# marict/nnue-vision

Hardware: AMD Instinct MI355X
Metric: NNUE training images/sec (full step: fwd+bwd+clip+SGD) (higher is better)
Workload: dtype f32; 1 GPU; c2: NNUE 32x32 grid 10x10x8 F=800 -> 1024/128/32 -> 10, batch 512/GPU, SGD m0.9 wd2e-4 clip1.0; global_batch=512, parallelism=dp1, launch=hipGraph, steps_per_graph=26, max_active_features=453

## Files before the change

### include/nnue_hip.h

```cpp
#ifndef NNUE_HIP_H
#define NNUE_HIP_H

#include <stdint.h>

#ifdef __cplusplus
extern "C" {
#endif

#define NNUE_HIP_ABI_VERSION 39

#define NNUE_OK 0
#define NNUE_E_ARG (-1)
#define NNUE_E_SHAPE (-2)
#define NNUE_E_LAUNCH (-3)
#define NNUE_E_SCRATCH (-4)

typedef void* nnue_stream_t;
typedef struct nnue_cls_rider { unsigned char opaque[256]; } nnue_cls_rider;

int nnue_hip_abi_version(void);
const char* nnue_hip_last_error(void);


int nnue_conv3x3_forward(const float* images, const float* weight, float* conv_out,
// ... 37 lines not shown
int nnue_ft_backward_weight(const float* d_out, const float* coefT, int ldb,
                            int B, int F, int L1, float* d_weight, float* d_bias,
                            nnue_stream_t stream);

int nnue_ft_backward_values(const float* d_out, const float* weight,
                            const int32_t* rows, const int32_t* pos, const int32_t* n, int cap,
                            int B, int F, int L1, float* dst, int dst_ld, nnue_stream_t stream);

int nnue_ftb_supported(int L1);
int nnue_ftb_list_tiles(int B, int F, int P, int* tiles_fwd, int* tiles_bwd);
int64_t nnue_ftb_scratch(int B, int F, int P, int L1);

int nnue_binarize_bits(const float* conv_out, const float* thr, int B, int fps, int Gh, int Gw, int F,
                       uint64_t* maskW, int pw64, uint64_t* maskT, int bw64, float* sink, int32_t* n,
                       uint8_t* tlW, uint8_t* tcW, uint8_t* tlT, uint8_t* tcT, int stages, nnue_stream_t stream);

int nnue_ftb_forward(const float* weight, const float* bias, const uint8_t* tlW, const uint8_t* tcW,
                     const float* sink, int B, int F, int P, int L1, float* out,
                     void* scratch, int64_t scratch_bytes, nnue_stream_t stream);

int nnue_ftb_backward_weight(const float* d_out, const uint8_t* tlT, const uint8_t* tcT, const float* sink,
                             int B, int F, int P, int L1, float* d_weight, float* d_bias,
                             void* scratch, int64_t scratch_bytes, nnue_stream_t stream);

int nnue_ftb_backward_values(const float* d_out, const float* weight, const uint64_t* maskW, int pw64,
                             int B, int F, int P, int L1, float* d_conv_out, nnue_stream_t stream);

int nnue_ftm_supported(int F, int P, int L1);
int64_t nnue_ftm_scratch(int B, int F, int P, int L1);

int nnue_ftm_binarize(const float* conv_out, const float* thr, int B, int fps, int Gh, int Gw, int F,
                      uint8_t* bits, int32_t* n, float* sink, nnue_stream_t stream);

int nnue_ftm_conv_binarize(const float* images, const float* weight, const float* thr, int B, int H, int W,
                           int fps, int stride, int F, float* conv_out, uint8_t* bits, int32_t* n, float* sink,
                           nnue_stream_t stream);
int nnue_ftm_conv_binarize_patches(const float* images, const float* weight, const float* thr, int B, int H, int W,
                                   int fps, int stride, int F, float* patches, float* conv_out, uint8_t* bits,
                                   int32_t* n, float* sink, nnue_stream_t stream);

int nnue_ftm_forward(const uint8_t* bits, const float* sink, const float* weight, const float* bias,
                     int B, int F, int P, int L1, float* out,
                     void* scratch, int64_t scratch_bytes, nnue_stream_t stream);

int nnue_ftm_forward_l1_supported(int B, int F, int P, int L1, int L2);

int nnue_ftm_forward_l1(const uint8_t* bits, const float* sink, const float* weight, const float* bias,
                        const float* w1, int B, int F, int P, int L1, int L2, float* out, float* part,
                        nnue_stream_t stream);

int nnue_ftm_forward_l1_planes_supported(int B, int F, int P, int L1, int L2);
int64_t nnue_ftm_forward_planes_bytes(int B, int F, int P, int L1);

int nnue_ftm_conv_binarize_planes(const float* images, const float* weight, const float* thr, int B, int H, int W,
                                  int fps, int stride, int F, const float* table, int L1, int L2, void* planes,
                                  int64_t planes_bytes, float* conv_out, uint8_t* bits, int32_t* n, float* sink,
                                  nnue_stream_t stream);

int nnue_ftm_forward_l1_planes(const uint8_t* bits, const float* sink, const void* planes, int64_t planes_bytes,
                               const float* weight, const float* bias, const float* w1, int B, int F, int P, int L1,
                               int L2, float* out, float* part, nnue_stream_t stream);

int nnue_ftm_backward_weight(const uint8_t* bits, const float* sink, const float* d_out,
                             int B, int F, int P, int L1, float* d_weight, float* d_bias,
                             nnue_stream_t stream);

int nnue_ftm_backward_values(const uint8_t* bits, const float* d_out, const float* weight,
                             int B, int F, int P, int L1, float* d_conv_out, nnue_stream_t stream);
int64_t nnue_ftm_backward_values_scratch(int B, int F, int P, int L1);
int nnue_ftm_backward_values_ws(const uint8_t* bits, const float* d_out, const float* weight, int B, int F, int P, int L1,
                                float* d_conv_out, void* scratch, int64_t scratch_bytes, nnue_stream_t stream);

int nnue_ftm_backward_cw_supported(int B, int F, int P, int L1, int L2);
int64_t nnue_ftm_backward_sq_count(int B, int F, int P, int L1);
int64_t nnue_ftm_backward_ste_chunks(int B, int F, int P, int L1, int H, int W, int stride);
int nnue_ftm_backward_ste_supported(int B, int F, int P, int L1, int H, int W, int stride);

int nnue_ftm_backward(const uint8_t* bits, const float* sink, const float* d_out, const float* weight,
                      int B, int F, int P, int L1, float* d_weight, float* d_bias, float* d_conv_out,
                      const float* ft, const float* d_z1, int L2, float* d_w1, float* sq_partial,
                      const nnue_cls_rider* small, const float* ste_images, const float* ste_patches, const float* ste_conv_out,
                      const float* ste_thr, int H, int W, int stride, float* ste_partial, int64_t ste_partial_bytes,
                      nnue_stream_t stream);


int64_t nnue_classifier_scratch(int B, int L1, int L2, int L3);
int nnue_classifier_forward(const float* x, int pairwise,
                            const float* w1, const float* b1, const float* w2, const float* b2,
                            const float* w3, const float* b3, float clip,
                            int B, int L1, int L2, int L3, int C,
                            float* h1, float* h2, float* logits,
                            void* scratch, int64_t scratch_bytes, nnue_stream_t stream);

int nnue_classifier_backward(const float* x, int pairwise,
                             const float* w1, const float* w2, const float* w3, float clip,
                             const float* h1, const float* h2, const float* d_logits,
                             int B, int L1, int L2, int L3, int C,
                             float* d_x, float* d_w1, float* d_b1, float* d_w2, float* d_b2,
                             float* d_w3, float* d_b3,
                             void* scratch, int64_t scratch_bytes, nnue_stream_t stream);

int64_t nnue_classifier_train_scratch(int B, int L1, int L2, int L3, int C);
int64_t nnue_classifier_train_dz1_offset(int B, int L1, int L2, int L3, int C, int pairwise);
int nnue_classifier_train_step(const float* x, int pairwise,
                               const float* w1, const float* b1, const float* w2, const float* b2,
                               const float* w3, const float* b3, float clip,
                               const int64_t* labels, float grad_scale,
                               int B, int L1, int L2, int L3, int C,
                               float* h1, float* h2, float* logits, float* sample_loss, float* loss,
                               float* d_x, float* d_w1, float* d_b1, float* d_w2, float* d_b2,
                               float* d_w3, float* d_b3,
                               void* scratch, int64_t scratch_bytes, int phases, nnue_stream_t stream);
int nnue_classifier_train_fused_tail_supported(int B, int L1, int L2, int L3, int C, int K, int pairwise);
int nnue_classifier_train_rider(int pairwise, int B, int L1, int L2, int L3, int C, const float* h1, const float* h2,
                                const float* sample_loss, float* loss, float* d_b1, float* d_w2, float* d_b2,
                                float* d_w3, float* d_b3, void* scratch, int64_t scratch_bytes,
                                const struct nnue_buckets* buckets, nnue_cls_rider* out);

typedef struct nnue_buckets {
  int32_t K;
  const int32_t* bucket;
  const int32_t* rows;
  const int32_t* tile_bucket;
  const int32_t* seg;
  int32_t tiles;
} nnue_buckets;

int nnue_bucket_tile_count(int B, int K);
int nnue_bucket_group(const int32_t* n, int B, int P, int K, int32_t* bucket, int32_t* rows,
                      int32_t* tile_bucket, int32_t* seg, nnue_stream_t stream);

int nnue_ftm_forward_grouping(const uint8_t* bits, const float* sink, const float* weight, const float* bias,
                              int B, int F, int P, int L1, float* out, void* scratch, int64_t scratch_bytes,
                              const int32_t* n, int K, int32_t* bucket, int32_t* rows, int32_t* tile_bucket,
                              int32_t* seg, nnue_stream_t stream);

int64_t nnue_classifier_scratch_bucketed(int B, int L1, int L2, int L3, int K);
int64_t nnue_classifier_train_scratch_bucketed(int B, int L1, int L2, int L3, int C, int K);
int nnue_classifier_forward_bucketed(const float* x, int pairwise,
                                     const float* w1, const float* b1, const float* w2, const float* b2,
                                     const float* w3, const float* b3, float clip,
                                     int B, int L1, int L2, int L3, int C,
                                     float* h1, float* h2, float* logits,
                                     void* scratch, int64_t scratch_bytes, const nnue_buckets* buckets,
                                     nnue_stream_t stream);
int nnue_classifier_backward_bucketed(const float* x, int pairwise,
                                      const float* w1, const float* w2, const float* w3, float clip,
                                      const float* h1, const float* h2, const float* d_logits,
                                      int B, int L1, int L2, int L3, int C,
                                      float* d_x, float* d_w1, float* d_b1, float* d_w2, float* d_b2,
                                      float* d_w3, float* d_b3,
                                      void* scratch, int64_t scratch_bytes, const nnue_buckets* buckets,
                                      nnue_stream_t stream);
int64_t nnue_classifier_train_dz1_grouped_offset(int B, int L1, int L2, int L3, int C, int K);
int64_t nnue_classifier_train_x_grouped_offset(int B, int L1, int L2, int L3, int C, int K);
int nnue_classifier_train_step_bucketed(const float* x, int pairwise,
                                        const float* w1, const float* b1, const float* w2, const float* b2,
                                        const float* w3, const float* b3, float clip,
                                        const int64_t* labels, float grad_scale,
                                        int B, int L1, int L2, int L3, int C,
                                        float* h1, float* h2, float* logits, float* sample_loss, float* loss,
                                        float* d_x, float* d_w1, float* d_b1, float* d_w2, float* d_b2,
                                        float* d_w3, float* d_b3,
                                        void* scratch, int64_t scratch_bytes, int phases,
                                        const nnue_buckets* buckets, nnue_stream_t stream);

// ... 196 lines not shown
```

### nnue-vision_amd/csrc/feature_kernels.hip

```cpp
#include "common.h"

#include <cstdlib>

namespace {

constexpr float kSteSharpness = 10.0f;
constexpr int kConvChunk = 8;

__global__ __launch_bounds__(256) void conv3x3_forward_kernel(const float* __restrict__ img,
                                                              const float* __restrict__ w,
                                                              float* __restrict__ out, int B, int H, int W,
                                                              int fps, int stride, int Gh, int Gw) {
  extern __shared__ float w_lds[];
  for (int i = threadIdx.x; i < fps * 27; i += blockDim.x) w_lds[i] = w[i];
  __syncthreads();
  const int G = Gh * Gw;
  const long long t = (long long)blockIdx.x * blockDim.x + threadIdx.x;
  if (t >= (long long)B * G) return;
  const int b = (int)(t / G);
  const int hw = (int)(t - (long long)b * G);
  const int h = hw / Gw, x = hw - h * Gw;
  float patch[27];
#pragma unroll
  for (int ci = 0; ci < 3; ++ci)
#pragma unroll
    for (int kh = 0; kh < 3; ++kh)
#pragma unroll
      for (int kw = 0; kw < 3; ++kw) {
        const int iy = h * stride + kh - 1, ix = x * stride + kw - 1;
        const bool in = iy >= 0 && iy < H && ix >= 0 && ix < W;
        patch[ci * 9 + kh * 3 + kw] = in ? img[(((size_t)b * 3 + ci) * H + iy) * W + ix] : 0.0f;
      }
  for (int c0 = 0; c0 < fps; c0 += kConvChunk) {
    float acc[kConvChunk];
#pragma unroll
    for (int u = 0; u < kConvChunk; ++u) acc[u] = 0.0f;
#pragma unroll
    for (int q = 0; q < 27; ++q)
#pragma unroll
      for (int u = 0; u < kConvChunk; ++u) {
        const int c = (c0 + u < fps) ? c0 + u : fps - 1;
        acc[u] = fmaf(patch[q], w_lds[c * 27 + q], acc[u]);
      }
#pragma unroll
    for (int u = 0; u < kConvChunk; ++u)
      if (c0 + u < fps) out[((size_t)b * fps + c0 + u) * G + hw] = acc[u];
  }
}

#include "conv_binarize.h"

template <bool kFullUnroll, bool kPatch = false>
__global__ __launch_bounds__(256) void conv_binarize_kernel(const float* __restrict__ img, const float* __restrict__ w,
                                                            const float* __restrict__ thr, float* __restrict__ out,
                                                            uint8_t* __restrict__ bits, int* __restrict__ n,
                                                            float* __restrict__ sink, int H, int W, int fps, int stride,
                                                            int Gh, int Gw, int F, int slices, float* __restrict__ patches) {
  extern __shared__ __attribute__((aligned(16))) float w_lds[];
  ConvParamsPlain prm{w, thr};
  conv_binarize_body<kFullUnroll, kPatch>(img, prm, out, bits, n, sink, H, W, fps, stride, Gh, Gw, F, slices, (int)blockIdx.x, (int)blockIdx.y,
                                          w_lds, [] {}, patches, (size_t)gridDim.x * Gh * Gw);
}

#include "forward_planes.h"

template <bool kFullUnroll>
__global__ __launch_bounds__(256) void conv_binarize_planes_kernel(const float* __restrict__ img, const float* __restrict__ w,
                                                                   const float* __restrict__ thr, float* __restrict__ out,
                                                                   uint8_t* __restrict__ bits, int* __restrict__ n,
                                                                   float* __restrict__ sink, int B, int H, int W, int fps, int stride,
                                                                   int Gh, int Gw, int F, int slices, FwdPlaneArgs pa) {
  extern __shared__ __attribute__((aligned(16))) float w_lds[];
  const int id = (int)blockIdx.x;
  if (id >= B * slices) {
    forward_planes_write(pa, id - B * slices);
    return;
  }
  ConvParamsPlain prm{w, thr};
  conv_binarize_body<kFullUnroll, false>(img, prm, out, bits, n, sink, H, W, fps, stride, Gh, Gw, F, slices, id % B, id / B, w_lds, [] {});
}

__global__ __launch_bounds__(256) void binarize_compact_kernel(const float* __restrict__ conv_out,
                                                               const float* __restrict__ thr, int G, int P, int F,
                                                               int* __restrict__ rows, int* __restrict__ pos,
                                                               float* __restrict__ coef, int* __restrict__ n,
                                                               float* __restrict__ coefT, int ldb) {
  __shared__ int wave_count[4];
  __shared__ int sink_count[4];
  const int b = blockIdx.x;
  const int tid = threadIdx.x, lane = tid & 63, wave = tid >> 6;
  const float* __restrict__ x = conv_out + (size_t)b * P;
  const size_t base = (size_t)b * P;
  int written = 0, sink = 0;
  for (int p0 = 0; p0 < P; p0 += 256) {
    const int p = p0 + tid;
    const bool on = (p < P) && (x[p] > thr[p / G]);
    const unsigned long long m = __ballot(on);
    const unsigned long long ms = __ballot(on && p >= F - 1);
    if (lane == 0) {
      wave_count[wave] = __popcll(m);
      sink_count[wave] = __popcll(ms);
    }
    __syncthreads();
    int offset = written, total = 0;
#pragma unroll
    for (int w = 0; w < 4; ++w) {
      const int c = wave_count[w];
      if (w < wave) offset += c;
      total += c;
      sink += sink_count[w];
    }
    if (on) {
      const int k = offset + __popcll(m & ((1ull << lane) - 1ull));
      rows[base + k] = p < F - 1 ? p : F - 1;
      pos[base + k] = p;
      coef[base + k] = 1.0f;
    }
    written += total;
    __syncthreads();
  }
  if (tid == 0) {
    n[b] = written;
    coefT[(size_t)(F - 1) * ldb + b] = (float)sink;
  }
}

__global__ __launch_bounds__(256) void binarize_transpose_kernel(const float* __restrict__ conv_out,
                                                                 const float* __restrict__ thr, int B, int G, int P,
                                                                 int F, float* __restrict__ coefT, int ldb) {
  __shared__ float tile[64][65];
  const int p0 = blockIdx.x * 64, b0 = blockIdx.y * 64;
  const int tx = threadIdx.x & 63, ty = threadIdx.x >> 6;
  const int p = p0 + tx;
  const float t = (p < P) ? thr[p / G] : 0.0f;
  for (int j = ty; j < 64; j += 4) {
    const int b = b0 + j;
    const bool on = (b < B) && (p < P) && (conv_out[(size_t)b * P + p] > t);
    tile[j][tx] = on ? 1.0f : 0.0f;
  }
  __syncthreads();
  for (int j = ty; j < 64; j += 4) {
    const int f = p0 + j;
    if (f < F - 1 && b0 + tx < ldb) coefT[(size_t)f * ldb + b0 + tx] = tile[tx][j];
  }
}

__global__ __launch_bounds__(256) void ste_conv_backward_stage1(const float* __restrict__ img,
                                                                const float* __restrict__ conv_out,
                                                                const float* __restrict__ thr,
                                                                const float* __restrict__ d_conv_out, int B, int H,
                                                                int W, int fps, int stride, int Gh, int Gw,
                                                                int samples_per_chunk, float* __restrict__ partial) {
  __shared__ float red[4][28];
  const int c = blockIdx.x;
  const int chunk = blockIdx.y;
  const int G = Gh * Gw;
  const int b_lo = chunk * samples_per_chunk;
  const int b_hi = min(B, b_lo + samples_per_chunk);
// ... 212 lines not shown
  return blocks > 0 ? blocks : 1;
}

__global__ __launch_bounds__(256) void conv3x3_backward_input_kernel(const float* __restrict__ d_out, const float* __restrict__ w,
                                                                     float* __restrict__ d_img, int B, int H, int W, int fps,
                                                                     int stride, int Gh, int Gw) {
  extern __shared__ float w_lds[];
  for (int i = threadIdx.x; i < fps * 27; i += blockDim.x) w_lds[i] = w[i];
  __syncthreads();
  const long long t = (long long)blockIdx.x * blockDim.x + threadIdx.x;
  if (t >= (long long)B * H * W) return;
  const int b = (int)(t / ((long long)H * W));
  const int yx = (int)(t - (long long)b * H * W);
  const int y = yx / W, x = yx - y * W;
  const int G = Gh * Gw;
  float a0 = 0.f, a1 = 0.f, a2 = 0.f;
#pragma unroll
  for (int kh = 0; kh < 3; ++kh) {
    const int ny = y + 1 - kh;
    if (ny < 0 || ny % stride) continue;
    const int oh = ny / stride;
    if (oh >= Gh) continue;
#pragma unroll
    for (int kw = 0; kw < 3; ++kw) {
      const int nx = x + 1 - kw;
      if (nx < 0 || nx % stride) continue;
      const int ow = nx / stride;
      if (ow >= Gw) continue;
      const float* __restrict__ d = d_out + (size_t)b * fps * G + oh * Gw + ow;
      const int q = kh * 3 + kw;
      for (int c = 0; c < fps; ++c) {
        const float g = d[(size_t)c * G];
        a0 = fmaf(g, w_lds[c * 27 + q], a0);
        a1 = fmaf(g, w_lds[c * 27 + 9 + q], a1);
        a2 = fmaf(g, w_lds[c * 27 + 18 + q], a2);
      }
    }
  }
  float* __restrict__ o = d_img + (size_t)b * 3 * H * W + yx;
  o[0] = a0;
  o[(size_t)H * W] = a1;
  o[(size_t)2 * H * W] = a2;
}

__global__ __launch_bounds__(256) void sparse_values_gather_kernel(const float* __restrict__ map, const int64_t* __restrict__ idx,
                                                                   long long total, int P, int M, float* __restrict__ val) {
  const long long t = (long long)blockIdx.x * 256 + threadIdx.x;
  if (t >= total) return;
  const long long b = t / M;
  const int64_t p = idx[t];
  val[t] = (p >= 0 && p < P) ? map[b * P + p] : 0.0f;
}
__global__ __launch_bounds__(256) void sparse_values_scatter_kernel(const float* __restrict__ d_val, const int64_t* __restrict__ idx,
                                                                    long long total, int P, int M, float* __restrict__ d_map) {
  const long long t = (long long)blockIdx.x * 256 + threadIdx.x;
  if (t >= total) return;
  const long long b = t / M;
  const int64_t p = idx[t];
  if (p >= 0 && p < P) d_map[b * P + p] = d_val[t];
}

}

extern "C" int nnue_conv3x3_forward(const float* images, const float* weight, float* conv_out, int B, int H, int W,
                                    int fps, int stride, nnue_stream_t stream) {
  NNUE_REQUIRE(images && weight && conv_out, NNUE_E_ARG, "nnue_conv3x3_forward: null pointer");
  NNUE_REQUIRE(B > 0 && H > 0 && W > 0 && fps > 0 && stride > 0, NNUE_E_ARG,
               "nnue_conv3x3_forward: B=%d H=%d W=%d fps=%d stride=%d must be positive", B, H, W, fps, stride);
  NNUE_REQUIRE(fps * 27 * 4 <= 64 * 1024, NNUE_E_SHAPE, "nnue_conv3x3_forward: fps=%d too large for the LDS weight tile", fps);
  const int Gh = (H - 1) / stride + 1, Gw = (W - 1) / stride + 1;
  const long long total = (long long)B * Gh * Gw;
  NNUE_REQUIRE(total < (1ll << 31) * 256, NNUE_E_SHAPE, "nnue_conv3x3_forward: too many outputs");
  hipLaunchKernelGGL(conv3x3_forward_kernel, dim3((unsigned)((total + 255) / 256)), dim3(256), fps * 27 * sizeof(float),
                     static_cast<hipStream_t>(stream), images, weight, conv_out, B, H, W, fps, stride, Gh, Gw);
  return nnue_launch_status("nnue_conv3x3_forward");
}

namespace {
struct PlaneRide {
  const float* table;
  int L1, L2;
  void* planes;
  int64_t planes_bytes;
};

int conv_binarize_impl(const char* who, const float* images, const float* weight, const float* thr, int B, int H, int W, int fps, int stride, int F,
                       float* conv_out, float* patches, uint8_t* bits, int32_t* n, float* sink, nnue_stream_t stream,
                       const PlaneRide& ride = PlaneRide{}) {
  NNUE_REQUIRE(images && weight && thr && conv_out && bits && n && sink, NNUE_E_ARG, "%s: null pointer", who);
  NNUE_REQUIRE(B > 0 && H > 0 && W > 0 && fps > 0 && stride > 0 && F > 0, NNUE_E_ARG, "%s: B=%d H=%d W=%d fps=%d stride=%d F=%d must be positive", who,
               B, H, W, fps, stride, F);
  NNUE_REQUIRE(((fps + 7) & ~7) * 28 * 4 <= 64 * 1024, NNUE_E_SHAPE, "%s: fps=%d too large for the LDS weight tile", who, fps);
  const int Gh = (H - 1) / stride + 1, Gw = (W - 1) / stride + 1;
  const long long G = (long long)Gh * Gw;
  NNUE_REQUIRE(G * fps < (1ll << 30) && (long long)B * G * fps < (1ll << 40), NNUE_E_SHAPE, "%s: map too large", who);
  NNUE_REQUIRE(!patches || 27ll * B * G * 4 < (1ll << 31), NNUE_E_SHAPE, "%s: the im2col buffer must stay below 2 GiB", who);
  const int P = (int)(G * fps);
  if (ride.table) {
    NNUE_REQUIRE(ride.planes, NNUE_E_ARG, "%s: null pointer", who);
    NNUE_REQUIRE(nnue_ftm_forward_l1_planes_supported(B, F, P, ride.L1, ride.L2), NNUE_E_SHAPE,
                 "%s: B=%d F=%d P=%d L1=%d L2=%d is not a planes-fed forward shape (nnue_ftm_forward_l1_planes_supported)", who, B, F, P, ride.L1,
                 ride.L2);
    NNUE_REQUIRE(nnue_aligned16(ride.table) && nnue_aligned16(ride.planes), NNUE_E_ARG, "%s: pointers must be 16-byte aligned", who);
    NNUE_REQUIRE(ride.planes_bytes >= nnue_ftm_forward_planes_bytes(B, F, P, ride.L1), NNUE_E_SCRATCH, "%s: plane buffer of %lld bytes, needs %lld", who,
                 (long long)ride.planes_bytes, (long long)nnue_ftm_forward_planes_bytes(B, F, P, ride.L1));
  }
  hipStream_t s = static_cast<hipStream_t>(stream);
  const int threads = G <= 64 ? 64 : (G <= 128 ? 128 : 256);
  int slices = (512 + B - 1) / B;
  if (slices > (int)(G / threads)) slices = (int)(G / threads);
  slices = slices < 1 ? 1 : (slices > 16 ? 16 : slices);
  if (slices > 1) nnue_zero_counters(n, sink, B, s);
  const size_t lds = (size_t)(((fps + 7) & ~7) * 28) * sizeof(float);
  if (ride.table) {
    const int direct = (F - 1 < P) ? F - 1 : P, ktiles = (direct + kBfK - 1) / kBfK, parts = 256 / threads;
    const FwdPlaneArgs pa{ride.table, static_cast<unsigned char*>(ride.planes), (unsigned)((size_t)direct * ride.L1 * 4), ride.L1, ktiles, parts};
    const int riders = (ride.L1 / 64) * ktiles * parts;
    const dim3 grid((unsigned)(B * slices + riders));
    if (fps <= 16)
      hipLaunchKernelGGL((conv_binarize_planes_kernel<true>), grid, dim3(threads), lds, s, images, weight, thr, conv_out, bits, n, sink, B, H, W, fps,
                         stride, Gh, Gw, F, slices, pa);
    else
      hipLaunchKernelGGL((conv_binarize_planes_kernel<false>), grid, dim3(threads), lds, s, images, weight, thr, conv_out, bits, n, sink, B, H, W, fps,
                         stride, Gh, Gw, F, slices, pa);
    return nnue_launch_status(who);
  }
#define NNUE_CONV_LAUNCH(FULL, PATCH)                                                                                                           \
  hipLaunchKernelGGL((conv_binarize_kernel<FULL, PATCH>), dim3(B, slices), dim3(threads), lds, s, images, weight, thr, conv_out, bits, n, sink, H, \
                     W, fps, stride, Gh, Gw, F, slices, patches)
  if (fps <= 16) {
    if (!patches) NNUE_CONV_LAUNCH(true, false);
    else NNUE_CONV_LAUNCH(true, true);
  } else {
    if (!patches) NNUE_CONV_LAUNCH(false, false);
    else NNUE_CONV_LAUNCH(false, true);
  }
#undef NNUE_CONV_LAUNCH
  return nnue_launch_status(who);
}
}

extern "C" int nnue_ftm_conv_binarize(const float* images, const float* weight, const float* thr, int B, int H, int W, int fps,
                                      int stride, int F, float* conv_out, uint8_t* bits, int32_t* n, float* sink,
                                      nnue_stream_t stream) {
  return conv_binarize_impl("nnue_ftm_conv_binarize", images, weight, thr, B, H, W, fps, stride, F, conv_out, nullptr, bits, n, sink, stream);
}

extern "C" int nnue_ftm_conv_binarize_patches(const float* images, const float* weight, const float* thr, int B, int H, int W, int fps,
                                              int stride, int F, float* patches, float* conv_out, uint8_t* bits, int32_t* n, float* sink,
                                              nnue_stream_t stream) {
  NNUE_REQUIRE(patches, NNUE_E_ARG, "nnue_ftm_conv_binarize_patches: null pointer");
  return conv_binarize_impl("nnue_ftm_conv_binarize_patches", images, weight, thr, B, H, W, fps, stride, F, conv_out, patches, bits, n, sink, stream);
}

extern "C" int nnue_ftm_conv_binarize_planes(const float* images, const float* weight, const float* thr, int B, int H, int W, int fps,
                                             int stride, int F, const float* table, int L1, int L2, void* planes, int64_t planes_bytes,
                                             float* conv_out, uint8_t* bits, int32_t* n, float* sink, nnue_stream_t stream) {
  NNUE_REQUIRE(table && planes, NNUE_E_ARG, "nnue_ftm_conv_binarize_planes: null pointer");
  return conv_binarize_impl("nnue_ftm_conv_binarize_planes", images, weight, thr, B, H, W, fps, stride, F, conv_out, nullptr, bits, n, sink, stream,
                            PlaneRide{table, L1, L2, planes, planes_bytes});
}

extern "C" int nnue_binarize_features(const float* conv_out, const float* thr, int B, int fps, int Gh, int Gw, int F,
                                      int32_t* rows, int32_t* pos, float* coef, int32_t* n, float* coefT, int ldb,
                                      nnue_stream_t stream) {
  NNUE_REQUIRE(conv_out && thr && rows && pos && coef && n && coefT, NNUE_E_ARG, "nnue_binarize_features: null pointer");
  NNUE_REQUIRE(B > 0 && fps > 0 && Gh > 0 && Gw > 0 && F > 0, NNUE_E_ARG,
               "nnue_binarize_features: B=%d fps=%d Gh=%d Gw=%d F=%d must be positive", B, fps, Gh, Gw, F);
  NNUE_REQUIRE(ldb >= B && ldb % 64 == 0, NNUE_E_SHAPE, "nnue_binarize_features: ldb=%d must be a multiple of 64 and >= B=%d", ldb, B);
  const long long P64 = (long long)fps * Gh * Gw;
  NNUE_REQUIRE(P64 < (1ll << 30), NNUE_E_SHAPE, "nnue_binarize_features: fps*Gh*Gw too large");
  const int P = (int)P64, G = Gh * Gw;
  hipStream_t s = static_cast<hipStream_t>(stream);
  if (F > 1)
    hipLaunchKernelGGL(binarize_transpose_kernel, dim3((F - 1 + 63) / 64, ldb / 64), dim3(256), 0, s, conv_out, thr, B, G,
                       P, F, coefT, ldb);
  hipLaunchKernelGGL(binarize_compact_kernel, dim3(B), dim3(256), 0, s, conv_out, thr, G, P, F, rows, pos, coef, n, coefT,
                     ldb);
  return nnue_launch_status("nnue_binarize_features");
}

extern "C" int64_t nnue_ste_conv_backward_scratch(int B, int fps, int Gh, int Gw) {
  if (B <= 0 || fps <= 0) return 0;
  int64_t blocks = ste_chunks(B, fps);
  if (fps <= 64 && Gh > 0 && Gw > 0) blocks = ste_mfma_blocks((int64_t)B * Gh * Gw);
  return blocks * fps * 28 * (int64_t)sizeof(float);
}

extern "C" int64_t nnue_ste_conv_backward_chunks(int B, int fps, int Gh, int Gw) {
  if (B <= 0 || fps <= 0 || Gh <= 0 || Gw <= 0) return 0;
  return fps <= 64 ? ste_mfma_blocks((int64_t)B * Gh * Gw) : ste_chunks(B, fps);
}

namespace {
int ste_impl(const char* who, const float* images, const float* conv_out, const float* patches, const float* thr,
             const float* d_conv_out, int B, int H, int W, int fps, int stride, int Gh, int Gw, float* d_thr, float* d_weight, void* scratch,
             int64_t scratch_bytes, int stages, nnue_stream_t stream) {
  NNUE_REQUIRE(d_thr || d_weight, NNUE_E_ARG, "%s: both outputs are null", who);
  NNUE_REQUIRE(stages >= 1 && stages <= 3, NNUE_E_ARG, "%s: stages = 1 (partials) | 2 (final sums)", who);
  NNUE_REQUIRE(scratch_bytes >= nnue_ste_conv_backward_scratch(B, fps, Gh, Gw), NNUE_E_SCRATCH, "%s: scratch %lld < %lld bytes", who,
               (long long)scratch_bytes, (long long)nnue_ste_conv_backward_scratch(B, fps, Gh, Gw));
  hipStream_t s = static_cast<hipStream_t>(stream);
  float* partial = static_cast<float*>(scratch);
  int chunks;
  if (fps <= 64) {
    const long long NP = (long long)B * Gh * Gw;
    NNUE_REQUIRE(NP < (1ll << 31) - 64 && (long long)B * fps * Gh * Gw < (1ll << 40), NNUE_E_SHAPE, "%s: too many positions", who);
    const int tiles = (int)((NP + kStePos - 1) / kStePos);
    chunks = (int)ste_mfma_blocks(NP);
    const char* abl_env = std::getenv("NNUE_STE_ABL");
    const int abl = abl_env ? std::atoi(abl_env) : 0;
    if (stages & 1) {
#define NNUE_STE_LAUNCH(MT)                                                                                                          \
  do {                                                                                                                               \
    if (patches)                                                                                                                     \
      hipLaunchKernelGGL((ste_conv_backward_mfma<MT, true>), dim3(chunks), dim3(256), 0, s, patches, conv_out, thr, d_conv_out, B, H, W,  \
                         fps, stride, Gh, Gw, tiles, partial, abl);                                                                  \
    else                                                                                                                             \
      hipLaunchKernelGGL((ste_conv_backward_mfma<MT, false>), dim3(chunks), dim3(256), 0, s, images, conv_out, thr, d_conv_out, B, H, W, \
                         fps, stride, Gh, Gw, tiles, partial, abl);                                                                  \
  } while (0)
    switch ((fps + 15) / 16) {
      case 1: NNUE_STE_LAUNCH(1); break;
      case 2: NNUE_STE_LAUNCH(2); break;
      case 3: NNUE_STE_LAUNCH(3); break;
      default: NNUE_STE_LAUNCH(4); break;
    }
#undef NNUE_STE_LAUNCH
    }
  } else {
    NNUE_REQUIRE(!patches, NNUE_E_SHAPE, "%s: the im2col form needs fps <= 64 (fps = %d)", who, fps);
    chunks = ste_chunks(B, fps);
    const int spc = (B + chunks - 1) / chunks;
    NNUE_REQUIRE((long long)spc * Gh * Gw < (1ll << 31), NNUE_E_SHAPE, "%s: chunk too large", who);
    if (stages & 1)
      hipLaunchKernelGGL(ste_conv_backward_stage1, dim3(fps, chunks), dim3(256), 0, s, images, conv_out, thr, d_conv_out, B, H,
                         W, fps, stride, Gh, Gw, spc, partial);
  }
  if (stages & 2)
    hipLaunchKernelGGL(ste_conv_backward_stage2, dim3((fps * 28 + 3) / 4), dim3(256), 0, s, partial, chunks, fps, d_thr, d_weight);
  return nnue_launch_status(who);
}
}
// ... 56 lines not shown
```

### nnue-vision_amd/csrc/ftm_kernels.hip

```cpp
#include "common.h"
#include "small_wgrad.h"

#include <cstdlib>
#include <cstring>
#include <type_traits>

namespace {

using f32x4 = __attribute__((ext_vector_type(4))) float;

#include "bucket_group.h"
#include "optim_update.h"

struct Mat {
  const void* p;
  unsigned bytes;
  int ld, clamp, inner_k;
};
using u32x4 = __attribute__((__vector_size__(4 * sizeof(unsigned)))) unsigned;
#include "forward_planes.h"

template <bool U8>
__device__ __forceinline__ u32x4 mat_load(__amdgpu_buffer_rsrc_t rsrc, const Mat& m, int outer, int inner) {
  const int row = outer < m.clamp ? outer : m.clamp;
  const int elem = row * m.ld + inner;
  if (U8) {
    u32x4 raw = {0u, 0u, 0u, 0u};
    raw[0] = __builtin_amdgcn_raw_buffer_load_b32(rsrc, inner < m.inner_k ? elem : 0x7ffffff0, 0, 0);
    return raw;
  }
  return __builtin_amdgcn_raw_buffer_load_b128(rsrc, inner < m.inner_k ? elem * 4 : 0x7ffffff0, 0, 0);
}

template <bool U8>
__device__ __forceinline__ float4 widen(const u32x4& raw) {
  if (U8) {
    const unsigned w = raw[0];
    return make_float4((float)(w & 0xffu), (float)((w >> 8) & 0xffu), (float)((w >> 16) & 0xffu), (float)(w >> 24));
  }
  return make_float4(__uint_as_float(raw[0]), __uint_as_float(raw[1]), __uint_as_float(raw[2]), __uint_as_float(raw[3]));
}

__device__ __forceinline__ int xcd_contiguous_tile(int tile, int nwg) {
  const int xcd = tile & 7, q8 = nwg >> 3, r8 = nwg & 7;
  return (xcd < r8 ? xcd * (q8 + 1) : r8 * (q8 + 1) + (xcd - r8) * q8) + (tile >> 3);
}

struct FwdEpi {
  static constexpr bool kAU8 = true;
  static constexpr bool kFusedL1 = false;
  static constexpr bool kBPair = false;
  static constexpr bool kSq = false;
  const float* __restrict__ bias;
  const float* __restrict__ w_last;
  const float* __restrict__ sink;
  float* __restrict__ out;
  int B, L1, ksplit;
  __device__ __forceinline__ float2 col(int n) const { return ksplit == 1 ? make_float2(bias[n], w_last[n]) : make_float2(0.f, 0.f); }
  __device__ __forceinline__ float pre(int m, int) const { return ksplit == 1 ? sink[m] : 0.0f; }
  __device__ __forceinline__ void store(int m, int n, float v, float2 c, float s, int ks) const {
    if (ksplit == 1) v += fmaf(s, c.y, c.x);
    out[((size_t)ks * B + m) * L1 + n] = v;
  }
};

struct BwwEpi {
  static constexpr bool kAU8 = true;
  static constexpr bool kFusedL1 = false;
  static constexpr bool kBPair = false;
  static constexpr bool kSq = true;
  float* __restrict__ d_weight;
  int L1;
  float* __restrict__ sq;
  __device__ __forceinline__ float2 col(int) const { return make_float2(0.f, 0.f); }
  __device__ __forceinline__ float pre(int, int) const { return 0.0f; }
  __device__ __forceinline__ void store(int m, int n, float v, float2, float, int) const { d_weight[(size_t)m * L1 + n] = v; }
};

struct BwwSgdEpi {
  static constexpr bool kAU8 = true;
  static constexpr bool kFusedL1 = false;
  static constexpr bool kBPair = false;
  static constexpr bool kSq = false;
  static constexpr bool kRmw = true;
  float* __restrict__ weight;
  float* __restrict__ momentum;
  const float* __restrict__ coef;
  int L1;
  float lr, mom, wd, scale;
  int first_step;
  int xcd_remap;
  const float* __restrict__ lr_dev;
  __device__ __forceinline__ float2 col(int) const { return make_float2(coef[0] * scale, 0.f); }
  __device__ __forceinline__ float pre(int m, int n) const { return weight[(size_t)m * L1 + n]; }
  __device__ __forceinline__ void store(int m, int n, float v, float2 c, float w, int) const {
    const size_t i = (size_t)m * L1 + n;
    float gi = fmaf(wd, w, v * c.x);
    if (momentum) {
      gi = first_step ? gi : fmaf(mom, momentum[i], gi);
      momentum[i] = gi;
    }
    weight[i] = w - (lr_dev ? lr_dev[0] : lr) * gi;
  }
};

struct BwwAdamEpi {
  static constexpr bool kAU8 = true;
  static constexpr bool kFusedL1 = false;
  static constexpr bool kRmw = true;
  static constexpr bool kAdam = true;
  float* __restrict__ weight;
  float* __restrict__ exp_avg;
  float* __restrict__ exp_avg_sq;
  const float* __restrict__ coef;
  const int* __restrict__ step_counter;
  int L1;
  float lr, beta1, beta2, eps, wd, scale;
  int xcd_remap;
  const float* __restrict__ lr_dev;
};

struct ValEpi {
  static constexpr bool kAU8 = false;
  static constexpr bool kFusedL1 = false;
  static constexpr bool kBPair = false;
  static constexpr bool kSq = false;
  const uint8_t* __restrict__ bits;
  float* __restrict__ d_conv_out;
  int P;
  __device__ __forceinline__ float2 col(int) const { return make_float2(0.f, 0.f); }
  __device__ __forceinline__ float pre(int m, int p) const { return (float)bits[(size_t)m * P + p]; }
  __device__ __forceinline__ void store(int m, int p, float v, float2, float bit, int) const {
    d_conv_out[(size_t)m * P + p] = bit != 0.0f ? v : 0.0f;
  }
};

struct ValSteEpi {
  static constexpr bool kAU8 = false;
  static constexpr bool kFusedL1 = false;
  static constexpr bool kBPair = false;
  static constexpr bool kSte = true;
  const uint8_t* __restrict__ bits;
  float* __restrict__ d_conv_out;
  int P;
  const float* __restrict__ img;
  const float* __restrict__ patches;
  const float* __restrict__ conv_out;
  const float* __restrict__ thr;
  int H, W, stride, Gw, G;
  float* __restrict__ partial;
  int n_tiles;
  __device__ __forceinline__ int prow(int tile_n, int j) const {
    const int hw = tile_n * 8 + (j & 7);
    return (j >> 3) * G + (hw < G ? hw : G - 1);
  }
};
constexpr float kFtmSteSharpness = 10.0f;

template <class Epi, class = void>
struct is_ste { static constexpr bool value = false; };
template <class Epi>
struct is_ste<Epi, decltype((void)Epi::kSte)> { static constexpr bool value = Epi::kSte; };

template <int BM>
struct SteFrag {
  float pv[BM / 8][4][2];
  unsigned in[(BM + 31) / 32];
};
template <int BM>
__device__ __forceinline__ void ste_pixels(const ValSteEpi& e, SteFrag<BM>& f, int M, int m_base, int tile_n, int wave, int r, int q) {
#pragma unroll
  for (int w = 0; w < (BM + 31) / 32; ++w) f.in[w] = 0u;
#pragma unroll
  for (int g = 0; g < BM / 8; ++g)
#pragma unroll
    for (int t4 = 0; t4 < 4; ++t4) {
      const int k = wave * 2 * BM + 16 * g + 4 * q + t4;
      const int m = m_base + (k >> 3), hw = tile_n * 8 + (k & 7);
      const bool ok = m < M && hw < e.G;
      const int h = hw / e.Gw, x = hw - h * e.Gw;
#pragma unroll
      for (int s = 0; s < 2; ++s) {
        const int qq = r + 16 * s;
        const int qc = qq < 27 ? qq : 26;
        bool in;
        float v;
        if (e.patches) {
          in = ok && qq < 27;
          v = e.patches[in ? ((size_t)qc * M + m) * e.G + hw : 0];
        } else {
          const int ci = qc / 9, kh = (qc - ci * 9) / 3, kw = qc - ci * 9 - kh * 3;
          const int iy = h * e.stride + kh - 1, ix = x * e.stride + kw - 1;
          in = ok && qq < 27 && iy >= 0 && iy < e.H && ix >= 0 && ix < e.W;
          v = e.img[in ? (((size_t)m * 3 + ci) * e.H + iy) * e.W + ix : 0];
        }
        f.pv[g][t4][s] = v;
        f.in[g >> 2] |= (in ? 1u : 0u) << (8 * (g & 3) + 2 * t4 + s);
      }
    }
}
template <int BM>
__device__ __forceinline__ void ste_pixels_select(SteFrag<BM>& f, int r) {
#pragma unroll
  for (int g = 0; g < BM / 8; ++g)
#pragma unroll
    for (int t4 = 0; t4 < 4; ++t4)
#pragma unroll
      for (int s = 0; s < 2; ++s) {
        const bool in = (f.in[g >> 2] >> (8 * (g & 3) + 2 * t4 + s)) & 1u;
        f.pv[g][t4][s] = in ? f.pv[g][t4][s] : (r + 16 * s == 27 ? 1.0f : 0.0f);
      }
}

template <int BM>
struct StePre {
  uint8_t bit[BM / 32][2][4];
  float cv[BM / 32][2][4], th[2];
};
template <int BM>
__device__ __forceinline__ void ste_prefetch(const ValSteEpi& e, StePre<BM>& p, int M, int m_base, int tile_n, int m0, int n0, int r, int q) {
#pragma unroll
  for (int t = 0; t < 2; ++t) {
    const int j = n0 + 16 * t + r, c = j >> 3, hw = tile_n * 8 + (j & 7);
    const int pp = c * e.G + (hw < e.G ? hw : 0);
    p.th[t] = e.thr[c];
#pragma unroll
    for (int i = 0; i < BM / 32; ++i)
#pragma unroll
      for (int ee = 0; ee < 4; ++ee) {
        const int m = min(m_base + m0 + 16 * i + 4 * q + ee, M - 1);
        p.bit[i][t][ee] = e.bits[(size_t)m * e.P + pp];
        p.cv[i][t][ee] = e.conv_out[(size_t)m * e.P + pp];
      }
  }
}

template <int BM, int BN>
__device__ __forceinline__ void ste_tile(float* __restrict__ smem, const ValSteEpi& e, const f32x4 (&acc)[BM / 32][BN / 32], const SteFrag<BM>& f,
                                         const StePre<BM>& pre, int M, int m_base, int tile_n, int m0, int n0, int tile) {
  static_assert(BN == 64, "a tile holds the 8 channels of 8 positions");
  constexpr int TM = BM / 32, TN = BN / 32, LDA = 8 * BM + 4;
  const int tid = threadIdx.x, lane = tid & 63;
  const int wave = __builtin_amdgcn_readfirstlane(tid >> 6);
  const int r = lane & 15, q = lane >> 4;
  float bit[TM][TN][4], slope[TM][TN][4];
#pragma unroll
  for (int t = 0; t < TN; ++t) {
    const int hw = tile_n * 8 + ((n0 + 16 * t + r) & 7);
#pragma unroll
    for (int i = 0; i < TM; ++i)
#pragma unroll
      for (int ee = 0; ee < 4; ++ee) {
        const int m = m_base + m0 + 16 * i + 4 * q + ee;
        const bool ok = m < M && hw < e.G;
        bit[i][t][ee] = ok ? (float)pre.bit[i][t][ee] : 0.0f;
        const float cv = ok ? pre.cv[i][t][ee] : 0.0f;
        const float s = 1.0f / (1.0f + __expf(-kFtmSteSharpness * (cv - pre.th[t])));
        slope[i][t][ee] = (kFtmSteSharpness * s) * (1.0f - s);
      }
  }
  float* __restrict__ A = smem;
  float* __restrict__ red = smem + 16 * LDA;
#pragma unroll
  for (int t = 0; t < TN; ++t) {
    const int j = n0 + 16 * t + r, c = j >> 3, hw = tile_n * 8 + (j & 7);
    const int p = c * e.G + (hw < e.G ? hw : 0);
#pragma unroll
    for (int i = 0; i < TM; ++i)
#pragma unroll
      for (int ee = 0; ee < 4; ++ee) {
        const int m_loc = m0 + 16 * i + 4 * q + ee, m = m_base + m_loc;
        const float d = bit[i][t][ee] != 0.0f ? acc[i][t][ee] : 0.0f;
        if (e.d_conv_out && m < M && hw < e.G) e.d_conv_out[(size_t)m * e.P + p] = d;
        const int k = m_loc * 8 + (j & 7);
        A[c * LDA + k] = d;
        A[(8 + c) * LDA + k] = d * slope[i][t][ee];
      }
  }
  __syncthreads();
  f32x4 c0 = {0.f, 0.f, 0.f, 0.f}, c1 = {0.f, 0.f, 0.f, 0.f};
#pragma unroll
  for (int g = 0; g < BM / 8; ++g) {
    const float4 a = *reinterpret_cast<const float4*>(&A[r * LDA + wave * 2 * BM + 16 * g + 4 * q]);
    c0 = __builtin_amdgcn_mfma_f32_16x16x4f32(a.x, f.pv[g][0][0], c0, 0, 0, 0);
    c1 = __builtin_amdgcn_mfma_f32_16x16x4f32(a.x, f.pv[g][0][1], c1, 0, 0, 0);
    c0 = __builtin_amdgcn_mfma_f32_16x16x4f32(a.y, f.pv[g][1][0], c0, 0, 0, 0);
    c1 = __builtin_amdgcn_mfma_f32_16x16x4f32(a.y, f.pv[g][1][1], c1, 0, 0, 0);
    c0 = __builtin_amdgcn_mfma_f32_16x16x4f32(a.z, f.pv[g][2][0], c0, 0, 0, 0);
    c1 = __builtin_amdgcn_mfma_f32_16x16x4f32(a.z, f.pv[g][2][1], c1, 0, 0, 0);
    c0 = __builtin_amdgcn_mfma_f32_16x16x4f32(a.w, f.pv[g][3][0], c0, 0, 0, 0);
    c1 = __builtin_amdgcn_mfma_f32_16x16x4f32(a.w, f.pv[g][3][1], c1, 0, 0, 0);
  }
#pragma unroll
  for (int ee = 0; ee < 4; ++ee) {
    red[(wave * 8 + ee) * 64 + lane] = c0[ee];
    red[(wave * 8 + 4 + ee) * 64 + lane] = c1[ee];
  }
  __syncthreads();
  const int slot = xcd_contiguous_tile(tile, e.n_tiles);
  for (int o = tid; o < 8 * 28; o += 256) {
    const int c = o / 28, qq = o - c * 28;
    const int row = qq < 27 ? c : 8 + c, col = qq;
    const int s = (col >> 4) * 4 + (row & 3), ln = (row >> 2) * 16 + (col & 15);
    e.partial[(size_t)o * e.n_tiles + slot] =
        (red[(0 * 8 + s) * 64 + ln] + red[(1 * 8 + s) * 64 + ln]) + (red[(2 * 8 + s) * 64 + ln] + red[(3 * 8 + s) * 64 + ln]);
  }
}

struct CwEpi {
  static constexpr bool kAU8 = false;
  static constexpr bool kFusedL1 = false;
  static constexpr bool kBPair = true;
  static constexpr bool kSq = false;
  float* __restrict__ d_w1;
  int L1, half;
  __device__ __forceinline__ float2 col(int) const { return make_float2(0.f, 0.f); }
  __device__ __forceinline__ float pre(int, int) const { return 0.0f; }
  __device__ __forceinline__ void store(int m, int n, float v, float2, float, int) const { d_w1[(size_t)m * L1 + n] = v; }
};

struct FwdL1Epi {
  static constexpr bool kAU8 = true;
  static constexpr bool kFusedL1 = true;
  static constexpr bool kBPair = false;
// ... 840 lines not shown
    if constexpr (ABL == 4) return;
#pragma unroll
    for (int i = 0; i < GA; ++i) {
      const int g = tid + 256 * i, row = g / RUNS, c = g % RUNS;
      u32x4 hi, mid, lo;
      if constexpr (ABL == 1 || ABL == 2) { hi = ra[i][0]; mid = ra[i][1]; lo = ra[i][0] ^ ra[i][1]; }
      else split8(ra[i][0], ra[i][1], hi, mid, lo);
      *reinterpret_cast<u32x4*>(As + bf6_img<KT>(row, c)) = hi;
      *reinterpret_cast<u32x4*>(As + PA + bf6_img<KT>(row, c)) = mid;
      *reinterpret_cast<u32x4*>(As + 2 * PA + bf6_img<KT>(row, c)) = lo;
    }
#pragma unroll
    for (int i = 0; i < GB; ++i) {
      const int g = tid + 256 * i, row = g / RUNS, c = g % RUNS;
      u32x4 hi, mid, lo;
      if constexpr (ABL == 2) { hi = rb[i][0]; mid = rb[i][1]; lo = rb[i][0] ^ rb[i][1]; }
      else split8(rb[i][0], rb[i][1], hi, mid, lo);
      *reinterpret_cast<u32x4*>(Bs + bf6_img<KT>(row, c)) = hi;
      *reinterpret_cast<u32x4*>(Bs + PB + bf6_img<KT>(row, c)) = mid;
      *reinterpret_cast<u32x4*>(Bs + 2 * PB + bf6_img<KT>(row, c)) = lo;
    }
  };
  f32x4 acc[TM][TN];
#pragma unroll
  for (int i = 0; i < TM; ++i)
#pragma unroll
    for (int t = 0; t < TN; ++t) acc[i][t] = (f32x4){0.f, 0.f, 0.f, 0.f};
  auto contract = [&]() {
#pragma unroll
    for (int kb = 0; kb < KT / 32; ++kb) {
      const int c = kb * 4 + q;
      bf16x8 a[3][TM], b[3][TN];
#pragma unroll
      for (int pl = 0; pl < 3; ++pl) {
#pragma unroll
        for (int i = 0; i < TM; ++i) a[pl][i] = *reinterpret_cast<const bf16x8*>(As + pl * PA + bf6_img<KT>(m0 + 16 * i + r, c));
#pragma unroll
        for (int t = 0; t < TN; ++t) b[pl][t] = *reinterpret_cast<const bf16x8*>(Bs + pl * PB + bf6_img<KT>(n0 + 16 * t + r, c));
      }
      constexpr int pa[6] = {2, 0, 1, 1, 0, 0}, pb[6] = {0, 2, 1, 0, 1, 0};
      if constexpr (ABL == 3) {
#pragma unroll
        for (int s6 = 0; s6 < 6; ++s6)
#pragma unroll
          for (int i = 0; i < TM; ++i)
#pragma unroll
            for (int t = 0; t < TN; ++t) acc[i][t][0] += (float)a[pa[s6]][i][0] + (float)b[pb[s6]][t][0];
      } else {
#pragma unroll
      for (int s6 = 0; s6 < 6; ++s6)
#pragma unroll
        for (int i = 0; i < TM; ++i)
#pragma unroll
          for (int t = 0; t < TN; ++t) acc[i][t] = __builtin_amdgcn_mfma_f32_16x16x32_bf16(a[pa[s6]][i], b[pb[s6]][t], acc[i][t], 0, 0, 0);
      }
    }
  };
  fetch(k_lo);
  for (int k0 = k_lo; k0 < k_hi; k0 += KT) {
    stage();
    __syncthreads();
    if (k0 + KT < k_hi) fetch(k0 + KT);
    contract();
    __syncthreads();
  }
  if constexpr (is_ste<Epi>::value) {
    SteFrag<BM> stef;
    StePre<BM> stepre;
    ste_prefetch<BM>(epi, stepre, M, m_base, tile_n, m0, n0, r, q);
    ste_pixels<BM>(epi, stef, M, m_base, tile_n, wave, r, q);
    ste_pixels_select<BM>(stef, r);
    ste_tile<BM, BN>(reinterpret_cast<float*>(smem), epi, acc, stef, stepre, M, m_base, tile_n, m0, n0, tile);
  } else {
    store_tile<BM, BN, Epi>(reinterpret_cast<float*>(smem), epi, acc, M, N, m_base, n_base, m0, n0, tile, ks);
  }
}

template <int BM, int BN, class Epi, int KT, int ABL = 0>
__global__ __launch_bounds__(256) void ftm_gemm_bf6_kernel(Mat ma, Mat mb, Epi epi, int M, int N, int K, int tiles_n) {
  __shared__ __attribute__((aligned(16))) unsigned char smem[gemm_bf6_lds_bytes<BM, BN, KT>()];
  gemm_tile_bf6<BM, BN, Epi, KT, ABL>(smem, ma, mb, epi, M, N, 0, K, tiles_n, blockIdx.x, 0);
}

template <int BM, int BN, bool AKC, class Epi>
__global__ __launch_bounds__(256) void ftm_gemm_bf_kernel(Mat ma, Mat mb, Epi epi, int M, int N, int K, int klen, int tiles_n, GroupArgs ga) {
  __shared__ __attribute__((aligned(16))) unsigned char smem[gemm_bf_lds_bytes<BM, BN, kBfK>()];
  if (ga.n && blockIdx.x == gridDim.x - 1) {
    if (blockIdx.y == 0) bucket_group_body<256>(ga, reinterpret_cast<int*>(smem));
    return;
  }
  const int ks = blockIdx.y, k_lo = ks * klen;
  int tile = blockIdx.x;
  if constexpr (is_rmw<Epi>::value) {
    if (epi.xcd_remap) tile = xcd_contiguous_tile(tile, gridDim.x);
  }
  gemm_tile_bf<BM, BN, AKC, Epi>(smem, ma, mb, epi, M, N, k_lo, (k_lo + klen < K) ? k_lo + klen : K, tiles_n, tile, ks);
}

template <int BM>
__global__ __launch_bounds__(256) void ftm_forward_l1_bf_kernel(Mat ma, Mat mb, FwdL1Epi epi, int M, int N, int K, int tiles_n) {
  constexpr int kGemm = gemm_bf_lds_bytes<BM, 64, kBfK>(), kEpi = 2 * BM * kL1Ld * 4;
  __shared__ __attribute__((aligned(16))) unsigned char smem[kGemm > kEpi ? kGemm : kEpi];
  gemm_tile_bf<BM, 64, true, FwdL1Epi>(smem, ma, mb, epi, M, N, 0, K, tiles_n, blockIdx.x, 0);
}

__global__ __launch_bounds__(256) void ftm_forward_l1_planes_kernel(Mat ma, Mat mp, FwdL1Epi epi, int M, int N, int K, int tiles_n) {
  constexpr int kGemm = gemm_bf_lds_bytes<32, 64, kBfK>(), kEpi = 2 * 32 * kL1Ld * 4;
  __shared__ __attribute__((aligned(16))) unsigned char smem[kGemm > kEpi ? kGemm : kEpi];
  gemm_tile_bf<32, 64, true, FwdL1Epi, true>(smem, ma, mp, epi, M, N, 0, K, tiles_n, blockIdx.x, 0);
}

constexpr int kStreamKTiles = 7, kStreamDepth = 3;
__global__ __launch_bounds__(256) __attribute__((amdgpu_waves_per_eu(1, 1))) void ftm_forward_l1_stream_kernel(Mat ma, Mat mp, FwdL1Epi epi,
                                                                                                            int K, int tiles_n) {
  constexpr int D = kStreamDepth;
  static_assert(D >= 1 && D <= kStreamKTiles, "K tiles of plane loads requested ahead");
  constexpr int kA = 32 * kBfK * 2, kEpi = 2 * 32 * kL1Ld * 4;
  static_assert(kStreamKTiles * kA >= kEpi, "the epilogue's LDS aliases the A images");
  __shared__ __attribute__((aligned(16))) unsigned char smem[kStreamKTiles * kA];
  const __amdgpu_buffer_rsrc_t rsa = __builtin_amdgcn_make_buffer_rsrc(const_cast<void*>(ma.p), 0, ma.bytes, 0x00020000);
  const __amdgpu_buffer_rsrc_t rsb = __builtin_amdgcn_make_buffer_rsrc(const_cast<void*>(mp.p), 0, mp.bytes, 0x00020000);
  const int tid = threadIdx.x, lane = tid & 63;
  const int wave = __builtin_amdgcn_readfirstlane(tid >> 6);
  const int r = lane & 15, q = lane >> 4;
  const int tile = blockIdx.x, tile_n = tile % tiles_n, tile_m = tile / tiles_n;
  const int m_base = tile_m * 32, n0 = 16 * wave;
  const int ktiles = (K + kBfK - 1) / kBfK;
  const int a_row = ((tid >> 4) << 1) | (tid & 1), a_grp = (tid >> 1) & 7;
  u32x4 ra[kStreamKTiles];
#pragma unroll
  for (int kt = 0; kt < kStreamKTiles; ++kt)
    ra[kt] = __builtin_amdgcn_raw_buffer_load_b128(rsa, (m_base + a_row) * ma.ld + kt * kBfK + a_grp * 16, 0, 0);
  FusedL1Pre<32, true> l1pre;
  fused_l1_prefetch<32, true>(epi, l1pre, m_base, tile_n, 0, n0, r, q, wave);
  __builtin_amdgcn_sched_barrier(0);
  int b_off[kBfK / 32];
#pragma unroll
  for (int kb = 0; kb < kBfK / 32; ++kb) b_off[kb] = bf_img(n0 + r, 4 * kb + q);
  u32x4 rb[D][kBfK / 32][3];
  auto fetch = [&](int kt, u32x4 (&R)[kBfK / 32][3]) {
    const int blk = (tile_n * ktiles + (kt < ktiles ? kt : ktiles - 1)) * kFwdPlaneBlock;
#pragma unroll
    for (int kb = 0; kb < kBfK / 32; ++kb)
#pragma unroll
      for (int pnum = 2; pnum >= 0; --pnum) R[kb][pnum] = __builtin_amdgcn_raw_buffer_load_b128(rsb, b_off[kb], blk + pnum * (64 * kBfK * 2), 0);
  };
#pragma unroll
  for (int kt = 0; kt < D; ++kt) fetch(kt, rb[kt]);
  __builtin_amdgcn_sched_barrier(0);
#pragma unroll
  for (int kt = 0; kt < kStreamKTiles; ++kt) stage_map_k(smem + kt * kA, BfImg<kBfK>{}, a_row, a_grp * 2, ra[kt]);
  __syncthreads();
  f32x4 acc[2][1];
#pragma unroll
  for (int i = 0; i < 2; ++i) acc[i][0] = (f32x4){0.f, 0.f, 0.f, 0.f};
#pragma unroll
  for (int kt = 0; kt < kStreamKTiles; ++kt) {
    u32x4 (&R)[kBfK / 32][3] = rb[kt % D];
    if (kt < ktiles) {
      const unsigned char* __restrict__ As = smem + kt * kA;
#pragma unroll
      for (int kb = 0; kb < kBfK / 32; ++kb) {
        const int c = kb * 4 + q;
        bf16x8 a[2];
#pragma unroll
        for (int i = 0; i < 2; ++i) a[i] = *reinterpret_cast<const bf16x8*>(As + bf_img(16 * i + r, c));
// ... 87 lines not shown
#pragma unroll
      for (int u = 0; u < 8; ++u) {
        d[u] = d_out[(size_t)(b + u) * L1 + col];
        s[u] = sink[b + u];
      }
#pragma unroll
      for (int u = 0; u < 8; ++u) {
        sb += d[u];
        sw = fmaf(s[u], d[u], sw);
      }
    }
    for (; b < hi; ++b) {
      const float d = d_out[(size_t)b * L1 + col];
      sb += d;
      sw = fmaf(sink[b], d, sw);
    }
  }
  red[0][part][c] = sb;
  red[1][part][c] = sw;
  __syncthreads();
  if (part < 2 && col < L1) {
    float s = 0.f;
#pragma unroll
    for (int i = 0; i < 16; ++i) s += red[part][i][c];
    if (part == 0) {
      if (d_bias) d_bias[col] = s;
    } else if (d_weight) {
      d_weight[(size_t)(F - 1) * L1 + col] = s;
    }
  }
}

__global__ __launch_bounds__(256) void ftm_tail_rows_kernel(TailRows t) {
  __shared__ float red[512];
  tail_rows_block(t, blockIdx.x, blockIdx.y, red);
}

struct CwArgs {
  Mat a, b;
  CwEpi e;
  int M, N, K, tiles_n, n_c;
  const int* seg;
  int per_bucket;
};

template <int WM, int WN, int WK, int VM, int VN, int VK>
__global__ __launch_bounds__(256) void ftm_backward_kernel(Mat wa, Mat wb, BwwEpi we, int wM, int wN, int wK, int w_tiles_n, int n_w,
                                                           Mat va, Mat vb, ValEpi ve, int vM, int vN, int vK, int v_tiles_n, int n_v,
                                                           CwArgs c, TailRows t, SmallWgrad sw) {
  constexpr int kW = gemm_lds_floats<WM, WN, WK, false, false>(), kV = gemm_lds_floats<VM, VN, VK, true, true>();
  constexpr int kC = gemm_lds_floats<WM, WN, WK, false, false>();
  constexpr int kWV = kW > kV ? kW : kV;
  __shared__ __attribute__((aligned(16))) float smem[kWV > kC ? kWV : kC];
  const int blk = blockIdx.x;
  if (blk < n_v) {
    gemm_tile<VM, VN, VK, true, true, ValEpi>(smem, va, vb, ve, vM, vN, 0, vK, v_tiles_n, blk, 0);
  } else if (blk < n_v + n_w) {
    gemm_tile<WM, WN, WK, false, false, BwwEpi>(smem, wa, wb, we, wM, wN, 0, wK, w_tiles_n, blk - n_v, 0);
  } else if (blk < n_v + n_w + c.n_c) {
    const int t = blk - n_v - n_w;
    if (c.seg) {
      const int kb = t / c.per_bucket;
      const int k_lo = c.seg[kb], k_hi = c.seg[kb + 1];
      Mat a = c.a, b = c.b;
      a.bytes = (unsigned)k_hi * (unsigned)a.ld * 4u;
      b.bytes = (unsigned)k_hi * (unsigned)b.ld * 4u;
      CwEpi e = c.e;
      e.d_w1 += (size_t)kb * c.M * c.N;
      gemm_tile<WM, WN, WK, false, false, CwEpi>(smem, a, b, e, c.M, c.N, k_lo, k_hi, c.tiles_n, t - kb * c.per_bucket, 0);
    } else {
      gemm_tile<WM, WN, WK, false, false, CwEpi>(smem, c.a, c.b, c.e, c.M, c.N, 0, c.K, c.tiles_n, t, 0);
    }
  } else {
    const int i = blk - n_w - n_v - c.n_c, n_t = t.col_blocks * (1 + t.zero_slices);
    if (i < n_t) tail_rows_block(t, i % t.col_blocks, i / t.col_blocks, smem);
    else small_wgrad_body(sw, i - n_t, smem);
  }
}

template <int WM, int VM, int VN, int VK, bool V6 = false, bool W64 = false, class VE = ValEpi>
__global__ __launch_bounds__(256) void ftm_backward_bf_kernel(Mat wa, Mat wb, BwwEpi we, int wM, int wN, int wK, int w_tiles_n, int n_w,
                                                              Mat va, Mat vb, VE ve, int vM, int vN, int vK, int v_tiles_n, int n_v,
                                                              CwArgs c, TailRows t, SmallWgrad sw) {
  constexpr int kW = gemm_bf_lds_bytes<WM, 64, W64 ? kBf64K : kBfK>(), kV = V6 ? gemm_bf6_lds_bytes<VM, VN>() : gemm_lds_floats<VM, VN, VK, true, true>() * 4;
  constexpr int kC = gemm_lds_floats<32, 64, 128, false, false>() * 4;
  constexpr int kWV = kW > kV ? kW : kV;
  constexpr int kLds = kWV > kC ? kWV : kC;
  static_assert(!is_ste<VE>::value || (16 * (8 * VM + 4) + 2048) * 4 <= kLds, "the STE epilogue borrows the tile's LDS");
  __shared__ __attribute__((aligned(16))) unsigned char smem_b[kLds];
  float* smem = reinterpret_cast<float*>(smem_b);
  const int blk = blockIdx.x;
  if (blk < n_v) {
    if constexpr (V6) gemm_tile_bf6<VM, VN, VE>(smem_b, va, vb, ve, vM, vN, 0, vK, v_tiles_n, blk, 0);
    else gemm_tile<VM, VN, VK, true, true, VE>(smem, va, vb, ve, vM, vN, 0, vK, v_tiles_n, blk, 0);
  } else if (blk < n_v + n_w) {
    if constexpr (W64) gemm_tile_bf64<WM, false, BwwEpi>(smem_b, wa, wb, we, wM, wN, 0, wK, w_tiles_n, blk - n_v, 0);
    else gemm_tile_bf<WM, 64, false, BwwEpi>(smem_b, wa, wb, we, wM, wN, 0, wK, w_tiles_n, blk - n_v, 0);
  } else if (blk < n_v + n_w + c.n_c) {
    const int t2 = blk - n_v - n_w;
    if (c.seg) {
      const int kb = t2 / c.per_bucket;
      const int k_lo = c.seg[kb], k_hi = c.seg[kb + 1];
      Mat a = c.a, b = c.b;
      a.bytes = (unsigned)k_hi * (unsigned)a.ld * 4u;
      b.bytes = (unsigned)k_hi * (unsigned)b.ld * 4u;
      CwEpi e = c.e;
      e.d_w1 += (size_t)kb * c.M * c.N;
      gemm_tile<32, 64, 128, false, false, CwEpi>(smem, a, b, e, c.M, c.N, k_lo, k_hi, c.tiles_n, t2 - kb * c.per_bucket, 0);
    } else {
      gemm_tile<32, 64, 128, false, false, CwEpi>(smem, c.a, c.b, c.e, c.M, c.N, 0, c.K, c.tiles_n, t2, 0);
    }
  } else {
    const int i = blk - n_w - n_v - c.n_c, n_t = t.col_blocks * (1 + t.zero_slices);
    if (i < n_t) tail_rows_block(t, i % t.col_blocks, i / t.col_blocks, smem);
    else small_wgrad_body(sw, i - n_t, smem);
  }
}

__global__ __launch_bounds__(256) void ftm_binarize_kernel(const float* __restrict__ conv_out, const float* __restrict__ thr,
                                                           int P, int G, int F, int slices, uint8_t* __restrict__ bits,
                                                           int* __restrict__ n, float* __restrict__ sink) {
  __shared__ int cnt_s[4], sink_s[4];
  const int b = blockIdx.x;
  const float4* __restrict__ x4 = reinterpret_cast<const float4*>(conv_out + (size_t)b * P);
  unsigned* __restrict__ o4 = reinterpret_cast<unsigned*>(bits + (size_t)b * P);
  int cnt = 0, snk = 0;
  for (int g = blockIdx.y * 256 + threadIdx.x; g < P / 4; g += 256 * slices) {
    const float4 x = x4[g];
    const int p = g * 4;
    int c = p / G, rem = p - c * G;
    float4 v;
    v.x = x.x > thr[c] ? 1.0f : 0.0f;
    if (++rem == G) { rem = 0; ++c; }
    v.y = x.y > thr[c] ? 1.0f : 0.0f;
    if (++rem == G) { rem = 0; ++c; }
    v.z = x.z > thr[c] ? 1.0f : 0.0f;
    if (++rem == G) { rem = 0; ++c; }
    v.w = x.w > thr[c] ? 1.0f : 0.0f;
    o4[g] = (unsigned)v.x | ((unsigned)v.y << 8) | ((unsigned)v.z << 16) | ((unsigned)v.w << 24);
    cnt += (int)(v.x + v.y + v.z + v.w);
    snk += (p >= F - 1 ? (int)v.x : 0) + (p + 1 >= F - 1 ? (int)v.y : 0) + (p + 2 >= F - 1 ? (int)v.z : 0) + (p + 3 >= F - 1 ? (int)v.w : 0);
  }
#pragma unroll
  for (int s = 32; s >= 1; s >>= 1) {
    cnt += __shfl_xor(cnt, s);
    snk += __shfl_xor(snk, s);
  }
  if ((threadIdx.x & 63) == 0) {
    cnt_s[threadIdx.x >> 6] = cnt;
    sink_s[threadIdx.x >> 6] = snk;
  }
  __syncthreads();
  if (threadIdx.x == 0) {
    const int total = cnt_s[0] + cnt_s[1] + cnt_s[2] + cnt_s[3], st = sink_s[0] + sink_s[1] + sink_s[2] + sink_s[3];
    if (slices == 1) {
      n[b] = total;
      sink[b] = (float)st;
    } else {
      atomicAdd(&n[b], total);
      if (st) atomicAdd(&sink[b], (float)st);
    }
  }
}

using i32x4 = __attribute__((ext_vector_type(4))) int;
constexpr int kGramU = 4;

__device__ __forceinline__ void gram_pair(int x, int& tm, int& tn) {
  tm = 0;
  while ((tm + 1) * (tm + 2) / 2 <= x) ++tm;
  tn = x - tm * (tm + 1) / 2;
}

__global__ __launch_bounds__(256) void gram_i8_kernel(const uint8_t* __restrict__ bits, unsigned bytes, int B, int P, int direct, int wave_steps,
                                                      int* __restrict__ slabs, int slices, TailRows tr, int n_tail) {
  __shared__ int red[4][4][256];
// ... 329 lines not shown
}
}

namespace {
bool values_bf6(int B, int P, int L1) {
  static const int bf6 = env_int("NNUE_FTM_VAL_BF6", 1);
  const Shape s = plan(B, P, L1, true, false);
  return bf6 && use_bf16() && s.cfg == 2 && s.ksplit == 1 && L1 % 8 == 0;
}
}

extern "C" int nnue_ftm_backward_values(const uint8_t* bits, const float* d_out, const float* weight, int B, int F, int P, int L1,
                                        float* d_conv_out, nnue_stream_t stream) {
  NNUE_REQUIRE(bits && d_out && weight && d_conv_out, NNUE_E_ARG, "nnue_ftm_backward_values: null pointer");
  NNUE_REQUIRE(shape_ok(B, F, P, L1), NNUE_E_ARG, "nnue_ftm_backward_values: B=%d F=%d P=%d L1=%d out of range", B, F, P, L1);
  NNUE_REQUIRE(nnue_ftm_supported(F, P, L1), NNUE_E_SHAPE, "nnue_ftm_backward_values: P=%d and L1=%d must be multiples of 4", P, L1);
  NNUE_REQUIRE(nnue_aligned16(d_out) && nnue_aligned16(weight), NNUE_E_ARG, "nnue_ftm_backward_values: pointers must be 16-byte aligned");
  hipStream_t st = static_cast<hipStream_t>(stream);
  const Shape s = plan(B, P, L1, true, false);
  const Mat ma{d_out, (unsigned)((size_t)B * L1 * 4), L1, kIntMax, L1}, mb{weight, (unsigned)((size_t)F * L1 * 4), L1, F - 1, kIntMax};
  const ValEpi epi{bits, d_conv_out, P};
  if (values_bf6(B, P, L1)) {
    const dim3 grid((unsigned)(s.tiles_m * s.tiles_n));
#ifdef NNUE_ABLATIONS
    static const int abl = env_int("NNUE_FTM_BF6_ABL", 0);
#define NNUE_ABL(N) if (abl == N) { hipLaunchKernelGGL((ftm_gemm_bf6_kernel<128, 64, ValEpi, 32, N>), grid, dim3(256), 0, st, ma, mb, epi, B, P, L1, s.tiles_n); return nnue_launch_status("nnue_ftm_backward_values"); }
    NNUE_ABL(1) NNUE_ABL(2) NNUE_ABL(3) NNUE_ABL(4) NNUE_ABL(5)
#undef NNUE_ABL
#endif
    hipLaunchKernelGGL((ftm_gemm_bf6_kernel<128, 64, ValEpi, 32>), grid, dim3(256), 0, st, ma, mb, epi, B, P, L1, s.tiles_n);
    return nnue_launch_status("nnue_ftm_backward_values");
  }
  launch<true, true>(st, s, ma, mb, epi, B, P, L1);
  return nnue_launch_status("nnue_ftm_backward_values");
}

extern "C" int64_t nnue_ftm_backward_values_scratch(int , int , int , int ) { return 0; }

extern "C" int nnue_ftm_backward_values_ws(const uint8_t* bits, const float* d_out, const float* weight, int B, int F, int P, int L1,
                                           float* d_conv_out, void* , int64_t , nnue_stream_t stream) {
  return nnue_ftm_backward_values(bits, d_out, weight, B, F, P, L1, d_conv_out, stream);
}

namespace {
int merged_bf_wm() {
  const int wm = env_int("NNUE_FTM_BF_WM", 64);
  return use_bf16() ? (wm == 32 ? 32 : 64) : 0;
}

bool merged_backward_shape(int B, int F, int P, int L1, bool* big) {
  const int direct = (F - 1 < P) ? F - 1 : P;
  if (direct <= 0) return false;
  static const int split_launch = env_int("NNUE_FTM_SPLIT_BACKWARD", 0);
  static const int force_pair = env_int("NNUE_FTM_BWD_PAIR", 0);
  const Shape sw = plan(direct, L1, B, false, false), sv = plan(B, P, L1, true, false);
  const long long tiles64 = (long long)((direct + 63) / 64) * ((L1 + 63) / 64) + (long long)((B + 63) / 64) * ((P + 63) / 64);
  const bool small_pair = sw.cfg == 0 && (sv.cfg == 0 || sv.cfg == 1);
  *big = force_pair == 11 || (force_pair != 1 && small_pair && tiles64 >= 448);
  return !split_launch && (small_pair || *big);
}
bool merged_w64() {
  static const int w64 = env_int("NNUE_FTM_BWD_W64", 1);
  return w64 != 0;
}
bool merged_values_bf6(int B, int F, int P, int L1) {
  static const int bf6 = env_int("NNUE_FTM_BWD_BF6", 1);
  bool big = false;
  if (!merged_backward_shape(B, F, P, L1, &big) || !merged_bf_wm()) return false;
  const bool v_small = !big && plan(B, P, L1, true, false).cfg == 0;
  return bf6 && !v_small && L1 % 8 == 0;
}
}

namespace {
struct SteArgs {
  const float* img;
  const float* patches;
  const float* conv_out;
  const float* thr;
  int H, W, stride;
  float* partial;
  int64_t partial_bytes;
};

int64_t ste_ride_tiles(int B, int F, int P, int L1, int H, int W, int stride) {
  if (!nnue_ftm_supported(F, P, L1) || !shape_ok(B, F, P, L1) || H <= 0 || W <= 0 || stride <= 0) return 0;
  const long long Gh = (H - 1) / stride + 1, Gw = (W - 1) / stride + 1;
  if (8 * Gh * Gw != P || (long long)B * 3 * H * W >= (1ll << 40)) return 0;
  bool big = false;
  if (!merged_backward_shape(B, F, P, L1, &big) || merged_bf_wm() != 64 || !merged_w64()) return 0;
  static const int wide = env_int("NNUE_FTM_RIDE_STE_V64", 0);
  const int vm = (!big && plan(B, P, L1, true, false).cfg == 0) ? 32 : 64;
  if (vm != 32 && !wide) return 0;
  return (int64_t)((B + vm - 1) / vm) * ((Gh * Gw + 7) / 8);
}
}

extern "C" int64_t nnue_ftm_backward_ste_chunks(int B, int F, int P, int L1, int H, int W, int stride) {
  return ste_ride_tiles(B, F, P, L1, H, W, stride);
}
extern "C" int nnue_ftm_backward_ste_supported(int B, int F, int P, int L1, int H, int W, int stride) {
  return ste_ride_tiles(B, F, P, L1, H, W, stride) > 0;
}

extern "C" int64_t nnue_ftm_backward_sq_count(int B, int F, int P, int L1) {
  if (!nnue_ftm_supported(F, P, L1) || !shape_ok(B, F, P, L1)) return 0;
  const int direct = (F - 1 < P) ? F - 1 : P;
  if (direct <= 0) return 0;
  bool big = false;
  if (merged_backward_shape(B, F, P, L1, &big)) {
    if (const int wm = merged_bf_wm()) return (int64_t)((direct + wm - 1) / wm) * ((L1 + 63) / 64);
    if (big) return (int64_t)((direct + 63) / 64) * ((L1 + 63) / 64);
    const Shape s = plan(direct, L1, B, false, false);
    return (int64_t)s.tiles_m * s.tiles_n;
  }
  const Shape s = plan(direct, L1, B, false, false, true);
  return s.ksplit == 1 ? (int64_t)s.tiles_m * s.tiles_n : 0;
}

extern "C" int nnue_ftm_backward_cw_supported(int B, int F, int P, int L1, int L2) {
  bool big = false;
  return nnue_ftm_supported(F, P, L1) && shape_ok(B, F, P, L1) && merged_backward_shape(B, F, P, L1, &big) && L1 % 128 == 0 && L2 > 0 &&
         L2 % 4 == 0 && ((long long)B + 256) * L2 * 4 < (1ll << 31);
}

namespace {
int ftm_backward_impl(const uint8_t* bits, const float* sink, const float* d_out, const float* weight, int B, int F, int P, int L1,
                      float* d_weight, float* d_bias, float* d_conv_out, const float* ft, const float* d_z1, int L2, float* d_w1,
                      float* sq_partial, int K, const int32_t* seg, int grouped_rows, const nnue_cls_rider* small, const SteArgs* ste,
                      nnue_stream_t stream);
}
extern "C" int nnue_ftm_backward(const uint8_t* bits, const float* sink, const float* d_out, const float* weight, int B, int F, int P,
                                 int L1, float* d_weight, float* d_bias, float* d_conv_out, const float* ft, const float* d_z1, int L2,
                                 float* d_w1, float* sq_partial, const nnue_cls_rider* small, const float* ste_images, const float* ste_patches, const float* ste_conv_out,
                                 const float* ste_thr, int H, int W, int stride, float* ste_partial, int64_t ste_partial_bytes, nnue_stream_t stream) {
  const SteArgs sa{ste_images, ste_patches, ste_conv_out, ste_thr, H, W, stride, ste_partial, ste_partial_bytes};
  return ftm_backward_impl(bits, sink, d_out, weight, B, F, P, L1, d_weight, d_bias, d_conv_out, ft, d_z1, L2, d_w1, sq_partial, 1, nullptr, 0,
                           small, ste_partial ? &sa : nullptr, stream);
}
extern "C" int nnue_ftm_backward_bucketed(const uint8_t* bits, const float* sink, const float* d_out, const float* weight, int B, int F,
                                          int P, int L1, float* d_weight, float* d_bias, float* d_conv_out, const float* ft_grouped,
                                          const float* d_z1_grouped, int L2, float* d_w1, float* sq_partial, int K, const int32_t* seg,
                                          int grouped_rows, const nnue_cls_rider* small, const float* ste_images, const float* ste_patches, const float* ste_conv_out,
                                          const float* ste_thr, int H, int W, int stride, float* ste_partial, int64_t ste_partial_bytes,
                                          nnue_stream_t stream) {
  NNUE_REQUIRE(K >= 1 && K <= 64, NNUE_E_ARG, "nnue_ftm_backward_bucketed: K=%d out of range", K);
  NNUE_REQUIRE(K == 1 || !d_w1 || (seg && grouped_rows >= B && grouped_rows % 16 == 0), NNUE_E_ARG,
               "nnue_ftm_backward_bucketed: d_w1 for K > 1 needs seg and the grouped row count (a multiple of 16, >= B)");
  const SteArgs sa{ste_images, ste_patches, ste_conv_out, ste_thr, H, W, stride, ste_partial, ste_partial_bytes};
  return ftm_backward_impl(bits, sink, d_out, weight, B, F, P, L1, d_weight, d_bias, d_conv_out, ft_grouped, d_z1_grouped, L2, d_w1, sq_partial,
                           K, K > 1 ? seg : nullptr, K > 1 ? grouped_rows : 0, small, ste_partial ? &sa : nullptr, stream);
}
namespace {
int ftm_backward_impl(const uint8_t* bits, const float* sink, const float* d_out, const float* weight, int B, int F, int P, int L1,
                      float* d_weight, float* d_bias, float* d_conv_out, const float* ft, const float* d_z1, int L2, float* d_w1,
                      float* sq_partial, int K, const int32_t* seg, int grouped_rows, const nnue_cls_rider* small, const SteArgs* ste,
                      nnue_stream_t stream) {
  NNUE_REQUIRE(bits && sink && d_out && weight && d_weight && d_bias && (d_conv_out || ste), NNUE_E_ARG, "nnue_ftm_backward: null pointer");
  const int64_t ste_tiles = ste ? ste_ride_tiles(B, F, P, L1, ste->H, ste->W, ste->stride) : 0;
  NNUE_REQUIRE(!ste || ((ste->img || ste->patches) && ste->conv_out && ste->thr && ste->partial), NNUE_E_ARG,
               "nnue_ftm_backward: null STE pointer");
  NNUE_REQUIRE(!ste || ste_tiles > 0, NNUE_E_SHAPE, "nnue_ftm_backward: STE partials requested for a shape the merged launch does not take "
               "(nnue_ftm_backward_ste_chunks)");
  NNUE_REQUIRE(!ste || ste->partial_bytes >= ste_tiles * 8 * 28 * (int64_t)sizeof(float), NNUE_E_SCRATCH, "nnue_ftm_backward: STE partials %lld < %lld bytes",
               ste ? (long long)ste->partial_bytes : 0ll, (long long)ste_tiles * 8 * 28 * 4);
  const bool want_cw = d_w1 != nullptr;
  NNUE_REQUIRE(!want_cw || (ft && d_z1 && nnue_ftm_backward_cw_supported(B, F, P, L1, L2) && nnue_aligned16(ft) && nnue_aligned16(d_z1)),
               NNUE_E_SHAPE, "nnue_ftm_backward: d_w1 requested for a shape / pointers the merged launch does not take (nnue_ftm_backward_cw_supported)");
  NNUE_REQUIRE(shape_ok(B, F, P, L1), NNUE_E_ARG, "nnue_ftm_backward: B=%d F=%d P=%d L1=%d out of range", B, F, P, L1);
  NNUE_REQUIRE(nnue_ftm_supported(F, P, L1), NNUE_E_SHAPE, "nnue_ftm_backward: P=%d and L1=%d must be multiples of 4", P, L1);
  NNUE_REQUIRE(nnue_aligned16(bits) && nnue_aligned16(d_out) && nnue_aligned16(weight), NNUE_E_ARG,
               "nnue_ftm_backward: pointers must be 16-byte aligned");
  hipStream_t st = static_cast<hipStream_t>(stream);
  const int direct = (F - 1 < P) ? F - 1 : P;
  const Shape sw = plan(direct > 0 ? direct : 1, L1, B, false, false), sv = plan(B, P, L1, true, false);
  bool big_pair = false;
  const bool pair_ok = merged_backward_shape(B, F, P, L1, &big_pair);
  Shape sw2 = sw, sv2 = sv;
  for (Shape* q : {&sw2, &sv2}) { q->cfg = 1; q->bm = 64; q->bn = 64; q->bk = 64; }
  sw2.tiles_m = (direct + 63) / 64; sw2.tiles_n = (L1 + 63) / 64; sv2.tiles_m = (B + 63) / 64; sv2.tiles_n = (P + 63) / 64;
  NNUE_REQUIRE(!small || pair_ok, NNUE_E_SHAPE, "nnue_ftm_backward: the classifier's small gradients can ride only in the merged launch");
  if (!pair_ok) {
    const int rc = backward_weight_impl(bits, sink, d_out, B, F, P, L1, d_weight, d_bias, sq_partial, stream);
    return rc != NNUE_OK ? rc : nnue_ftm_backward_values(bits, d_out, weight, B, F, P, L1, d_conv_out, stream);
  }
  const Mat wa{bits, (unsigned)((size_t)B * P), P, kIntMax, kIntMax}, wb{d_out, (unsigned)((size_t)B * L1 * 4), L1, kIntMax, kIntMax};
  const Mat va{d_out, (unsigned)((size_t)B * L1 * 4), L1, kIntMax, L1}, vb{weight, (unsigned)((size_t)F * L1 * 4), L1, F - 1, kIntMax};
  const BwwEpi we{d_weight, L1, sq_partial};
  const ValEpi ve{bits, d_conv_out, P};
  const TailRows t = tail_rows(d_out, sink, B, L1, direct, F, d_weight, d_bias);
  const int bf_wm = merged_bf_wm();
  Shape sw3 = sw;
  if (bf_wm) { sw3.bm = bf_wm; sw3.bn = 64; sw3.bk = 128; sw3.tiles_m = (direct + bf_wm - 1) / bf_wm; sw3.tiles_n = (L1 + 63) / 64; }
  const Shape& swr = bf_wm ? sw3 : big_pair ? sw2 : sw;
  const Shape& svr = big_pair ? sv2 : sv;
  const int G = P / 8, v_tiles_n = ste ? (G + 7) / 8 : svr.tiles_n;
  const int n_w = swr.tiles_m * swr.tiles_n, n_v = svr.tiles_m * v_tiles_n, n_t = t.col_blocks * (1 + t.zero_slices);
  ValSteEpi vs{};
  if (ste) {
    const int Gw = (ste->W - 1) / ste->stride + 1;
    vs = ValSteEpi{bits, d_conv_out, P, ste->img, ste->patches, ste->conv_out, ste->thr, ste->H, ste->W, ste->stride, Gw, G, ste->partial, n_v};
  }
  CwArgs cw{};
  if (want_cw) {
    const int rows = seg ? grouped_rows : B;
    cw.a = Mat{d_z1, (unsigned)((size_t)rows * L2 * 4), L2, kIntMax, kIntMax};
    cw.b = Mat{ft, (unsigned)((size_t)rows * L1 * 4), L1, kIntMax, kIntMax};
    cw.e = CwEpi{d_w1, L1, L1 / 2};
    cw.M = L2; cw.N = L1; cw.K = B; cw.tiles_n = (L1 + 63) / 64;
    const int cw_bm = bf_wm ? 32 : swr.bm;
    cw.per_bucket = ((L2 + cw_bm - 1) / cw_bm) * cw.tiles_n;
    cw.seg = seg;
    cw.n_c = cw.per_bucket * (seg ? K : 1);
  }
  SmallWgrad sgw{};
  static_assert(sizeof(SmallWgrad) <= sizeof(nnue_cls_rider), "nnue_cls_rider is too small for the tile family's arguments");
  if (small) memcpy(&sgw, small, sizeof(SmallWgrad));
  const int n_s = small ? sgw.wgrad_blocks : 0;
  const dim3 grid((unsigned)(n_w + n_v + cw.n_c + n_t + n_s));
#define NNUE_FTM_BWD(WM, WN, WK, VM, VN, VK)                                                                                          \
  hipLaunchKernelGGL((ftm_backward_kernel<WM, WN, WK, VM, VN, VK>), grid, dim3(256), 0, st, wa, wb, we, direct, L1, B, swr.tiles_n, n_w, va, \
                     vb, ve, B, P, L1, svr.tiles_n, n_v, cw, t, sgw)
#define NNUE_FTM_BWD_BF(WM, VM, VN, VK)                                                                                                  \
  do {                                                                                                                                   \
    if (w64 && WM == 64 && !v6) hipLaunchKernelGGL((ftm_backward_bf_kernel<64, VM, VN, VK, false, true>), grid, dim3(256), 0, st, wa, wb, we, direct, L1, B, \
                               swr.tiles_n, n_w, va, vb, ve, B, P, L1, svr.tiles_n, n_v, cw, t, sgw);                                    \
    else if (w64 && WM == 64) hipLaunchKernelGGL((ftm_backward_bf_kernel<64, VM, VN, VK, true, true>), grid, dim3(256), 0, st, wa, wb, we, direct, L1, B, \
                               swr.tiles_n, n_w, va, vb, ve, B, P, L1, svr.tiles_n, n_v, cw, t, sgw);                                    \
    else if (v6) hipLaunchKernelGGL((ftm_backward_bf_kernel<WM, VM, VN, VK, true>), grid, dim3(256), 0, st, wa, wb, we, direct, L1, B, swr.tiles_n, n_w, va, \
                               vb, ve, B, P, L1, svr.tiles_n, n_v, cw, t, sgw);                                                           \
    else hipLaunchKernelGGL((ftm_backward_bf_kernel<WM, VM, VN, VK>), grid, dim3(256), 0, st, wa, wb, we, direct, L1, B, swr.tiles_n, n_w, va, vb, \
                            ve, B, P, L1, svr.tiles_n, n_v, cw, t, sgw);                                                                  \
  } while (0)
  const bool v_small = !big_pair && sv.cfg == 0;
  const bool v6 = merged_values_bf6(B, F, P, L1);
  const bool w64 = merged_w64();
  if (ste) {
    if (v_small)
      hipLaunchKernelGGL((ftm_backward_bf_kernel<64, 32, 64, 128, false, true, ValSteEpi>), grid, dim3(256), 0, st, wa, wb, we, direct, L1, B,
                         swr.tiles_n, n_w, va, vb, vs, B, P, L1, v_tiles_n, n_v, cw, t, sgw);
    else if (v6)
      hipLaunchKernelGGL((ftm_backward_bf_kernel<64, 64, 64, 64, true, true, ValSteEpi>), grid, dim3(256), 0, st, wa, wb, we, direct, L1, B,
                         swr.tiles_n, n_w, va, vb, vs, B, P, L1, v_tiles_n, n_v, cw, t, sgw);
    else
      hipLaunchKernelGGL((ftm_backward_bf_kernel<64, 64, 64, 64, false, true, ValSteEpi>), grid, dim3(256), 0, st, wa, wb, we, direct, L1, B,
                         swr.tiles_n, n_w, va, vb, vs, B, P, L1, v_tiles_n, n_v, cw, t, sgw);
    return nnue_launch_status("nnue_ftm_backward");
  }
  if (bf_wm == 64) { if (v_small) NNUE_FTM_BWD_BF(64, 32, 64, 128); else NNUE_FTM_BWD_BF(64, 64, 64, 64); }
  else if (bf_wm == 32) { if (v_small) NNUE_FTM_BWD_BF(32, 32, 64, 128); else NNUE_FTM_BWD_BF(32, 64, 64, 64); }
  else if (big_pair) NNUE_FTM_BWD(64, 64, 64, 64, 64, 64);
  else if (sv.cfg == 0) NNUE_FTM_BWD(32, 64, 128, 32, 64, 128);
  else NNUE_FTM_BWD(32, 64, 128, 64, 64, 64);
#undef NNUE_FTM_BWD_BF
#undef NNUE_FTM_BWD
  return nnue_launch_status("nnue_ftm_backward");
}
}

extern "C" int nnue_ftm_forward_l1_supported(int B, int F, int P, int L1, int L2) {
  if (!nnue_ftm_supported(F, P, L1) || !shape_ok(B, F, P, L1) || L1 % 64 != 0 || L2 <= 0) return 0;
  const int direct = (F - 1 < P) ? F - 1 : P;
  if (direct <= 0) return 0;
  const Shape s = plan(B, L1, direct, true, true, true);
  return (s.cfg == 0 || s.cfg == 1 || s.cfg == 6 || s.cfg == 7) && s.ksplit == 1;
}

extern "C" int nnue_ftm_forward_l1(const uint8_t* bits, const float* sink, const float* weight, const float* bias, const float* w1, int B,
                                   int F, int P, int L1, int L2, float* out, float* part, nnue_stream_t stream) {
  NNUE_REQUIRE(bits && sink && weight && bias && w1 && out && part, NNUE_E_ARG, "nnue_ftm_forward_l1: null pointer");
  NNUE_REQUIRE(nnue_ftm_forward_l1_supported(B, F, P, L1, L2), NNUE_E_SHAPE,
               "nnue_ftm_forward_l1: B=%d F=%d P=%d L1=%d L2=%d is not a fused-forward shape (nnue_ftm_forward_l1_supported)", B, F, P, L1, L2);
  NNUE_REQUIRE(nnue_aligned16(bits) && nnue_aligned16(weight) && nnue_aligned16(bias) && nnue_aligned16(out) && nnue_aligned16(w1), NNUE_E_ARG,
               "nnue_ftm_forward_l1: pointers must be 16-byte aligned");
  hipStream_t st = static_cast<hipStream_t>(stream);
  const int direct = (F - 1 < P) ? F - 1 : P;
  const Shape s = plan(B, L1, direct, true, true, true);
  const Mat ma{bits, (unsigned)((size_t)B * P), P, kIntMax, kIntMax}, mb{weight, (unsigned)((size_t)direct * L1 * 4), L1, kIntMax, kIntMax};
  const FwdL1Epi epi{bias, weight + (size_t)(F - 1) * L1, sink, out, w1, part, B, L1, L2, L1 / 2};
  const dim3 grid((unsigned)(s.tiles_m * s.tiles_n));
  if (s.cfg == 0) hipLaunchKernelGGL((ftm_forward_l1_kernel<32, 128>), grid, dim3(256), 0, st, ma, mb, epi, B, L1, direct, s.tiles_n);
  else if (s.cfg == 1) hipLaunchKernelGGL((ftm_forward_l1_kernel<64, 64>), grid, dim3(256), 0, st, ma, mb, epi, B, L1, direct, s.tiles_n);
  else if (s.cfg == 6) hipLaunchKernelGGL((ftm_forward_l1_bf_kernel<32>), grid, dim3(256), 0, st, ma, mb, epi, B, L1, direct, s.tiles_n);
  else hipLaunchKernelGGL((ftm_forward_l1_bf_kernel<64>), grid, dim3(256), 0, st, ma, mb, epi, B, L1, direct, s.tiles_n);
  return nnue_launch_status("nnue_ftm_forward_l1");
}

extern "C" int nnue_ftm_forward_l1_planes_supported(int B, int F, int P, int L1, int L2) {
  if (!nnue_ftm_forward_l1_supported(B, F, P, L1, L2)) return 0;
  const int direct = (F - 1 < P) ? F - 1 : P;
  if ((long long)direct * L1 * 4 > (long long)kStreamTableBytes) return 0;
  const long long t32 = (long long)((B + 31) / 32) * (L1 / 64), t64 = (long long)((B + 63) / 64) * (L1 / 64);
  return t32 >= env_int("NNUE_FTM_FWD_PLANES_MIN_WG", 256) && t64 < 256;
}

extern "C" int64_t nnue_ftm_forward_planes_bytes(int B, int F, int P, int L1) {
  if (B <= 0 || F <= 1 || P <= 0 || L1 <= 0 || L1 % 64 != 0) return 0;
  const int direct = (F - 1 < P) ? F - 1 : P;
  return (int64_t)(L1 / 64) * ((direct + kBfK - 1) / kBfK) * kFwdPlaneBlock;
}

extern "C" int nnue_ftm_forward_l1_planes(const uint8_t* bits, const float* sink, const void* planes, int64_t planes_bytes, const float* weight,
                                          const float* bias, const float* w1, int B, int F, int P, int L1, int L2, float* out, float* part,
                                          nnue_stream_t stream) {
  NNUE_REQUIRE(bits && sink && planes && weight && bias && w1 && out && part, NNUE_E_ARG, "nnue_ftm_forward_l1_planes: null pointer");
  NNUE_REQUIRE(nnue_ftm_forward_l1_planes_supported(B, F, P, L1, L2), NNUE_E_SHAPE,
               "nnue_ftm_forward_l1_planes: B=%d F=%d P=%d L1=%d L2=%d is not a planes-fed forward shape (nnue_ftm_forward_l1_planes_supported)", B, F,
               P, L1, L2);
  NNUE_REQUIRE(nnue_aligned16(bits) && nnue_aligned16(planes) && nnue_aligned16(weight) && nnue_aligned16(bias) && nnue_aligned16(out) &&
                   nnue_aligned16(w1),
               NNUE_E_ARG, "nnue_ftm_forward_l1_planes: pointers must be 16-byte aligned");
  const int64_t need = nnue_ftm_forward_planes_bytes(B, F, P, L1);
  NNUE_REQUIRE(planes_bytes >= need && need < (1ll << 31), NNUE_E_SCRATCH, "nnue_ftm_forward_l1_planes: plane buffer of %lld bytes, needs %lld",
               (long long)planes_bytes, (long long)need);
  hipStream_t st = static_cast<hipStream_t>(stream);
  const int direct = (F - 1 < P) ? F - 1 : P, tiles_n = L1 / 64;
  const Mat ma{bits, (unsigned)((size_t)B * P), P, kIntMax, kIntMax}, mp{planes, (unsigned)need, L1, kIntMax, kIntMax};
  const FwdL1Epi epi{bias, weight + (size_t)(F - 1) * L1, sink, out, w1, part, B, L1, L2, L1 / 2};
  const dim3 grid((unsigned)(((B + 31) / 32) * tiles_n));
  const int streamed = env_int("NNUE_FTM_FWD_STREAM", 1) != 0 && direct <= kStreamKTiles * kBfK;
  if (streamed) hipLaunchKernelGGL(ftm_forward_l1_stream_kernel, grid, dim3(256), 0, st, ma, mp, epi, direct, tiles_n);
// ... 204 lines not shown
  const Shape s = plan(B_next, L1, direct, true, true, true);
  static const int kt64 = env_int("NNUE_FTM_BF_KT64", 1);
  return s.cfg == 8 && kt64 && s.ksplit > 1 && s.klen % 128 == 0 && plan(direct, L1, B, false, false, true).cfg == 8;
}

extern "C" int nnue_ftm_backward_weight_update_forward(const uint8_t* bits, const float* d_out, int B, int F, int P, int L1, float* weight,
                                                       float* momentum_rows, const float* coef, float lr, float momentum, float weight_decay,
                                                       float grad_scale, int first_step, const float* lr_dev, const uint8_t* bits_next,
                                                       const float* sink_next, int B_next, const float* bias, float* out_next, void* scratch,
                                                       int64_t scratch_bytes, nnue_stream_t stream) {
  const char* who = "nnue_ftm_backward_weight_update_forward";
  const NextFwd nx{bits_next, sink_next, bias, out_next, scratch, scratch_bytes};
  if (const int rc = update_ptrs_nonnull(who, bits, d_out, weight, coef, &nx)) return rc;
  NNUE_REQUIRE(momentum == 0.0f || momentum_rows, NNUE_E_ARG, "%s: momentum %g needs the momentum rows", who, momentum);
  NNUE_REQUIRE(nnue_ftm_update_forward_supported(B, B_next, F, P, L1), NNUE_E_SHAPE,
               "%s: B=%d B_next=%d F=%d P=%d L1=%d is not a split-K forward over a big table (use the two separate calls)", who, B, B_next, F, P, L1);
  if (const int rc = update_ptrs_aligned(who, bits, d_out, weight, momentum_rows, &nx)) return rc;
  const UpdFwd a = make_upd_fwd<UpdFwd>(bits, d_out, B, F, P, L1, weight, momentum == 0.0f ? nullptr : momentum_rows, coef, lr_dev, lr, momentum,
                                        weight_decay, grad_scale, bits_next, B_next);
  return update_forward_launch<false>(who, a, F, a.momentum && first_step, nx, stream);
}

namespace {
int adam_table_args_ok(const char* who, const void* exp_avg_rows, const void* exp_avg_sq_rows, const void* step_counter, int B, int F, int P,
                       int L1, float beta1, float beta2, float eps) {
  NNUE_REQUIRE(exp_avg_rows && exp_avg_sq_rows && step_counter, NNUE_E_ARG, "%s: null pointer", who);
  NNUE_REQUIRE(nnue_aligned16(exp_avg_rows) && nnue_aligned16(exp_avg_sq_rows), NNUE_E_ARG, "%s: the moment rows must be 16-byte aligned", who);
  NNUE_REQUIRE(beta1 >= 0.f && beta1 < 1.f && beta2 >= 0.f && beta2 < 1.f && eps > 0.f, NNUE_E_ARG, "%s: betas must be in [0,1) and eps > 0", who);
  NNUE_REQUIRE(shape_ok(B, F, P, L1), NNUE_E_ARG, "%s: B=%d F=%d P=%d L1=%d out of range", who, B, F, P, L1);
  NNUE_REQUIRE(nnue_ftm_supported(F, P, L1), NNUE_E_SHAPE, "%s: P=%d and L1=%d must be multiples of 4", who, P, L1);
  NNUE_REQUIRE((int64_t)B * L1 <= (1 << 24), NNUE_E_SHAPE, "%s: B=%d x L1=%d exceeds 2^24 (the Gram form of the clip norm)", who, B, L1);
  NNUE_REQUIRE((int64_t)F * L1 * 4 <= 0x7ff00000ll, NNUE_E_SHAPE, "%s: table of %d x %d floats is too large", who, F, L1);
  return NNUE_OK;
}
}

extern "C" int nnue_ftm_backward_weight_update_adam(const uint8_t* bits, const float* d_out, int B, int F, int P, int L1, float* weight,
                                                    float* exp_avg_rows, float* exp_avg_sq_rows, const float* coef,
                                                    const int32_t* step_counter, float lr, float beta1, float beta2, float eps,
                                                    float weight_decay, float grad_scale, const float* lr_dev, nnue_stream_t stream) {
  const char* who = "nnue_ftm_backward_weight_update_adam";
  if (const int rc = update_ptrs_nonnull(who, bits, d_out, weight, coef, nullptr)) return rc;
  if (const int rc = adam_table_args_ok(who, exp_avg_rows, exp_avg_sq_rows, step_counter, B, F, P, L1, beta1, beta2, eps)) return rc;
  if (const int rc = update_ptrs_aligned(who, bits, d_out, weight, nullptr, nullptr)) return rc;
  const int direct = (F - 1 < P) ? F - 1 : P;
  if (direct <= 0) return NNUE_OK;
  static const int xcd = env_int("NNUE_FTM_XCD_REMAP", 1);
  return update_launch(who, bits, d_out, B, P, L1, direct,
                       BwwAdamEpi{weight, exp_avg_rows, exp_avg_sq_rows, coef, step_counter, L1, lr, beta1, beta2, eps, weight_decay, grad_scale, xcd, lr_dev},
                       stream);
}

extern "C" int nnue_ftm_backward_weight_update_forward_adam(const uint8_t* bits, const float* d_out, int B, int F, int P, int L1, float* weight,
                                                            float* exp_avg_rows, float* exp_avg_sq_rows, const float* coef,
                                                            const int32_t* step_counter, float lr, float beta1, float beta2, float eps,
                                                            float weight_decay, float grad_scale, const float* lr_dev,
                                                            const uint8_t* bits_next, const float* sink_next, int B_next, const float* bias,
                                                            float* out_next, void* scratch, int64_t scratch_bytes, nnue_stream_t stream) {
  const char* who = "nnue_ftm_backward_weight_update_forward_adam";
  const NextFwd nx{bits_next, sink_next, bias, out_next, scratch, scratch_bytes};
  if (const int rc = update_ptrs_nonnull(who, bits, d_out, weight, coef, &nx)) return rc;
  if (const int rc = adam_table_args_ok(who, exp_avg_rows, exp_avg_sq_rows, step_counter, B, F, P, L1, beta1, beta2, eps)) return rc;
  NNUE_REQUIRE(nnue_ftm_update_forward_supported(B, B_next, F, P, L1), NNUE_E_SHAPE,
               "%s: B=%d B_next=%d F=%d P=%d L1=%d is not a split-K forward over a big table (use the two separate calls)", who, B, B_next, F, P, L1);
  if (const int rc = update_ptrs_aligned(who, bits, d_out, weight, nullptr, &nx)) return rc;
  UpdFwdAdam a = make_upd_fwd<UpdFwdAdam>(bits, d_out, B, F, P, L1, weight, exp_avg_rows, coef, lr_dev, lr, 0.0f, weight_decay, grad_scale,
                                          bits_next, B_next);
  a.exp_avg_sq = exp_avg_sq_rows;
  a.step_counter = step_counter;
  a.beta1 = beta1;
  a.beta2 = beta2;
  a.eps = eps;
  return update_forward_launch<true>(who, a, F, false, nx, stream);
}

extern "C" int nnue_ftm_uses_bf16(int which, int B, int F, int P, int L1) {
  if (!nnue_ftm_supported(F, P, L1) || !shape_ok(B, F, P, L1)) return 0;
  const int direct = (F - 1 < P) ? F - 1 : P;
  if (direct <= 0) return 0;
  if (which == 0) return plan(B, L1, direct, true, true, true).cfg >= 6;
  if (which == 1) return plan(direct, L1, B, false, false, true).cfg >= 6;
  if (which == 2) { bool big = false; return merged_backward_shape(B, F, P, L1, &big) ? merged_bf_wm() != 0 : plan(direct, L1, B, false, false, true).cfg >= 6; }
  if (which == 4) return values_bf6(B, P, L1);
  if (which == 5) return merged_values_bf6(B, F, P, L1);
  return 1;
}
```

### nnue-vision_amd/nnue_hip/lib.py

```python
from __future__ import annotations

import ctypes
import os
from dataclasses import dataclass
from pathlib import Path
from typing import Optional, Tuple

import torch

_HERE = Path(__file__).resolve().parent
LIB_PATH = _HERE / "libnnue_hip.so"
ABI_VERSION = 39

_c_int, _c_i64, _c_f, _c_p = ctypes.c_int, ctypes.c_int64, ctypes.c_float, ctypes.c_void_p


class NnueBuckets(ctypes.Structure):
    _fields_ = [("K", ctypes.c_int32), ("bucket", _c_p), ("rows", _c_p), ("tile_bucket", _c_p), ("seg", _c_p),
                ("tiles", ctypes.c_int32)]


_c_bk = ctypes.POINTER(NnueBuckets)


class NnueClsRider(ctypes.Structure):
    _fields_ = [("opaque", ctypes.c_ubyte * 256)]


_c_rider = ctypes.POINTER(NnueClsRider)

SIGNATURES = {
    "nnue_hip_abi_version": (_c_int, []),
    "nnue_hip_last_error": (ctypes.c_char_p, []),
    "nnue_conv3x3_forward": (_c_int, [_c_p, _c_p, _c_p, _c_int, _c_int, _c_int, _c_int, _c_int, _c_p]),
    "nnue_conv3x3_backward_input": (_c_int, [_c_p, _c_p, _c_int, _c_int, _c_int, _c_int, _c_int, _c_p, _c_p]),
    "nnue_sparse_values": (_c_int, [_c_p, _c_p, _c_int, _c_int, _c_int, _c_p, _c_p]),
    "nnue_sparse_values_backward": (_c_int, [_c_p, _c_p, _c_int, _c_int, _c_int, _c_p, _c_p]),
    "nnue_binarize_features": (_c_int, [_c_p, _c_p, _c_int, _c_int, _c_int, _c_int, _c_int,
                                        _c_p, _c_p, _c_p, _c_p, _c_p, _c_int, _c_p]),
    "nnue_act_to_padded": (_c_int, [_c_p, _c_p, _c_p, _c_int, _c_int, _c_int, _c_p, _c_p, _c_p]),
    "nnue_ste_conv_backward_scratch": (_c_i64, [_c_int, _c_int, _c_int, _c_int]),
    "nnue_ste_conv_backward_chunks": (_c_i64, [_c_int, _c_int, _c_int, _c_int]),
    "nnue_ste_conv_backward": (_c_int, [_c_p, _c_p, _c_p, _c_p, _c_int, _c_int, _c_int, _c_int, _c_int,
                                        _c_p, _c_p, _c_p, _c_i64, _c_int, _c_p]),
    "nnue_ft_prepare": (_c_int, [_c_p, _c_p, _c_int, _c_int, _c_int, _c_p, _c_p, _c_p, _c_p, _c_p, _c_int, _c_p]),
    "nnue_ft_forward": (_c_int, [_c_p, _c_p, _c_p, _c_p, _c_p, _c_int, _c_int, _c_int, _c_int, _c_p, _c_p]),
    "nnue_ft_backward_weight": (_c_int, [_c_p, _c_p, _c_int, _c_int, _c_int, _c_int, _c_p, _c_p, _c_p]),
    "nnue_ft_backward_values": (_c_int, [_c_p, _c_p, _c_p, _c_p, _c_p, _c_int, _c_int, _c_int, _c_int,
                                         _c_p, _c_int, _c_p]),
    "nnue_ftb_supported": (_c_int, [_c_int]),
    "nnue_ftb_list_tiles": (_c_int, [_c_int, _c_int, _c_int, _c_p, _c_p]),
    "nnue_ftb_scratch": (_c_i64, [_c_int, _c_int, _c_int, _c_int]),
    "nnue_binarize_bits": (_c_int, [_c_p, _c_p, _c_int, _c_int, _c_int, _c_int, _c_int, _c_p, _c_int, _c_p, _c_int,
                                    _c_p, _c_p, _c_p, _c_p, _c_p, _c_p, _c_int, _c_p]),
    "nnue_ftb_forward": (_c_int, [_c_p, _c_p, _c_p, _c_p, _c_p, _c_int, _c_int, _c_int, _c_int, _c_p, _c_p, _c_i64, _c_p]),
    "nnue_ftb_backward_weight": (_c_int, [_c_p, _c_p, _c_p, _c_p, _c_int, _c_int, _c_int, _c_int, _c_p, _c_p,
                                          _c_p, _c_i64, _c_p]),
    "nnue_ftb_backward_values": (_c_int, [_c_p, _c_p, _c_p, _c_int, _c_int, _c_int, _c_int, _c_int, _c_p, _c_p]),
    "nnue_ftm_supported": (_c_int, [_c_int, _c_int, _c_int]),
    "nnue_ftm_scratch": (_c_i64, [_c_int, _c_int, _c_int, _c_int]),
    "nnue_ftm_binarize": (_c_int, [_c_p, _c_p, _c_int, _c_int, _c_int, _c_int, _c_int, _c_p, _c_p, _c_p, _c_p]),
    "nnue_ftm_conv_binarize": (_c_int, [_c_p, _c_p, _c_p, _c_int, _c_int, _c_int, _c_int, _c_int, _c_int, _c_p, _c_p, _c_p, _c_p, _c_p]),
    "nnue_ftm_conv_binarize_patches": (_c_int, [_c_p, _c_p, _c_p, _c_int, _c_int, _c_int, _c_int, _c_int, _c_int, _c_p, _c_p, _c_p, _c_p, _c_p,
                                                _c_p]),
    "nnue_ste_conv_backward_patches": (_c_int, [_c_p, _c_p, _c_p, _c_p, _c_int, _c_int, _c_int, _c_int, _c_p, _c_p, _c_p, _c_i64, _c_int, _c_p]),
    "nnue_ftm_forward": (_c_int, [_c_p, _c_p, _c_p, _c_p, _c_int, _c_int, _c_int, _c_int, _c_p, _c_p, _c_i64, _c_p]),
    "nnue_ftm_forward_grouping": (_c_int, [_c_p, _c_p, _c_p, _c_p, _c_int, _c_int, _c_int, _c_int, _c_p, _c_p, _c_i64, _c_p, _c_int,
                                           _c_p, _c_p, _c_p, _c_p, _c_p]),
    "nnue_ftm_forward_l1_supported": (_c_int, [_c_int, _c_int, _c_int, _c_int, _c_int]),
    "nnue_ftm_forward_l1": (_c_int, [_c_p, _c_p, _c_p, _c_p, _c_p, _c_int, _c_int, _c_int, _c_int, _c_int, _c_p, _c_p, _c_p]),
    "nnue_ftm_forward_l1_planes_supported": (_c_int, [_c_int, _c_int, _c_int, _c_int, _c_int]),
    "nnue_ftm_forward_planes_bytes": (_c_i64, [_c_int, _c_int, _c_int, _c_int]),
    "nnue_ftm_conv_binarize_planes": (_c_int, [_c_p, _c_p, _c_p, _c_int, _c_int, _c_int, _c_int, _c_int, _c_int, _c_p, _c_int, _c_int, _c_p, _c_i64,
                                               _c_p, _c_p, _c_p, _c_p, _c_p]),
    "nnue_ftm_forward_l1_planes": (_c_int, [_c_p, _c_p, _c_p, _c_i64, _c_p, _c_p, _c_p, _c_int, _c_int, _c_int, _c_int, _c_int, _c_p, _c_p, _c_p]),
    "nnue_ftm_backward_weight": (_c_int, [_c_p, _c_p, _c_p, _c_int, _c_int, _c_int, _c_int, _c_p, _c_p, _c_p]),
    "nnue_ftm_backward_values": (_c_int, [_c_p, _c_p, _c_p, _c_int, _c_int, _c_int, _c_int, _c_p, _c_p]),
    "nnue_ftm_backward_values_scratch": (_c_i64, [_c_int, _c_int, _c_int, _c_int]),
    "nnue_ftm_backward_values_ws": (_c_int, [_c_p, _c_p, _c_p, _c_int, _c_int, _c_int, _c_int, _c_p, _c_p, _c_i64, _c_p]),
    "nnue_ftm_backward_cw_supported": (_c_int, [_c_int, _c_int, _c_int, _c_int, _c_int]),
    "nnue_ftm_backward_sq_count": (_c_i64, [_c_int, _c_int, _c_int, _c_int]),
    "nnue_ftm_backward_ste_chunks": (_c_i64, [_c_int, _c_int, _c_int, _c_int, _c_int, _c_int, _c_int]),
    "nnue_ftm_backward_ste_supported": (_c_int, [_c_int, _c_int, _c_int, _c_int, _c_int, _c_int, _c_int]),
    "nnue_ftm_backward": (_c_int, [_c_p, _c_p, _c_p, _c_p, _c_int, _c_int, _c_int, _c_int, _c_p, _c_p, _c_p,
                                   _c_p, _c_p, _c_int, _c_p, _c_p, _c_rider, _c_p, _c_p, _c_p, _c_p, _c_int, _c_int, _c_int,
                                   _c_p, _c_i64, _c_p]),
    "nnue_ftm_backward_bucketed": (_c_int, [_c_p, _c_p, _c_p, _c_p, _c_int, _c_int, _c_int, _c_int, _c_p, _c_p, _c_p,
                                            _c_p, _c_p, _c_int, _c_p, _c_p, _c_int, _c_p, _c_int, _c_rider, _c_p, _c_p, _c_p,
                                            _c_p, _c_int, _c_int, _c_int, _c_p, _c_i64, _c_p]),
    "nnue_classifier_train_rider": (_c_int, [_c_int, _c_int, _c_int, _c_int, _c_int, _c_int, _c_p, _c_p, _c_p, _c_p, _c_p, _c_p, _c_p,
                                             _c_p, _c_p, _c_p, _c_i64, _c_bk, _c_rider]),
    "nnue_classifier_train_dz1_grouped_offset": (_c_i64, [_c_int, _c_int, _c_int, _c_int, _c_int, _c_int]),
    "nnue_classifier_train_x_grouped_offset": (_c_i64, [_c_int, _c_int, _c_int, _c_int, _c_int, _c_int]),
    "nnue_classifier_scratch": (_c_i64, [_c_int, _c_int, _c_int, _c_int]),
    "nnue_classifier_forward": (_c_int, [_c_p, _c_int, _c_p, _c_p, _c_p, _c_p, _c_p, _c_p, _c_f,
                                         _c_int, _c_int, _c_int, _c_int, _c_int, _c_p, _c_p, _c_p,
                                         _c_p, _c_i64, _c_p]),
    "nnue_classifier_backward": (_c_int, [_c_p, _c_int, _c_p, _c_p, _c_p, _c_f, _c_p, _c_p, _c_p,
                                          _c_int, _c_int, _c_int, _c_int, _c_int,
                                          _c_p, _c_p, _c_p, _c_p, _c_p, _c_p, _c_p, _c_p, _c_i64, _c_p]),
    "nnue_classifier_train_scratch": (_c_i64, [_c_int, _c_int, _c_int, _c_int, _c_int]),
    "nnue_classifier_train_dz1_offset": (_c_i64, [_c_int, _c_int, _c_int, _c_int, _c_int, _c_int]),
    "nnue_classifier_train_fused_tail_supported": (_c_int, [_c_int, _c_int, _c_int, _c_int, _c_int, _c_int, _c_int]),
    "nnue_classifier_train_step": (_c_int, [_c_p, _c_int, _c_p, _c_p, _c_p, _c_p, _c_p, _c_p, _c_f, _c_p, _c_f,
                                            _c_int, _c_int, _c_int, _c_int, _c_int,
                                            _c_p, _c_p, _c_p, _c_p, _c_p,
                                            _c_p, _c_p, _c_p, _c_p, _c_p, _c_p, _c_p, _c_p, _c_i64, _c_int, _c_p]),
    "nnue_bucket_tile_count": (_c_int, [_c_int, _c_int]),
    "nnue_bucket_group": (_c_int, [_c_p, _c_int, _c_int, _c_int, _c_p, _c_p, _c_p, _c_p, _c_p]),
    "nnue_classifier_scratch_bucketed": (_c_i64, [_c_int, _c_int, _c_int, _c_int, _c_int]),
    "nnue_classifier_train_scratch_bucketed": (_c_i64, [_c_int, _c_int, _c_int, _c_int, _c_int, _c_int]),
    "nnue_classifier_forward_bucketed": (_c_int, [_c_p, _c_int, _c_p, _c_p, _c_p, _c_p, _c_p, _c_p, _c_f,
                                                  _c_int, _c_int, _c_int, _c_int, _c_int, _c_p, _c_p, _c_p,
                                                  _c_p, _c_i64, _c_bk, _c_p]),
    "nnue_classifier_backward_bucketed": (_c_int, [_c_p, _c_int, _c_p, _c_p, _c_p, _c_f, _c_p, _c_p, _c_p,
                                                   _c_int, _c_int, _c_int, _c_int, _c_int,
                                                   _c_p, _c_p, _c_p, _c_p, _c_p, _c_p, _c_p, _c_p, _c_i64, _c_bk, _c_p]),
    "nnue_classifier_train_step_bucketed": (_c_int, [_c_p, _c_int, _c_p, _c_p, _c_p, _c_p, _c_p, _c_p, _c_f, _c_p, _c_f,
                                                     _c_int, _c_int, _c_int, _c_int, _c_int,
                                                     _c_p, _c_p, _c_p, _c_p, _c_p,
                                                     _c_p, _c_p, _c_p, _c_p, _c_p, _c_p, _c_p, _c_p, _c_i64, _c_int, _c_bk, _c_p]),
    "nnue_cross_entropy": (_c_int, [_c_p, _c_p, _c_int, _c_int, _c_f, _c_p, _c_p, _c_p, _c_p]),
    "nnue_confusion_accumulate": (_c_int, [_c_p, _c_p, _c_int, _c_int, _c_p, _c_p]),
    "nnue_load_batch": (_c_int, [_c_p, _c_p, _c_p, _c_int, _c_int, _c_int, _c_i64, _c_int, ctypes.c_uint64, ctypes.c_uint64,
                                 _c_p, _c_p, _c_p]),
    "nnue_load_batch_policy": (_c_int, [_c_p, _c_p, _c_p, _c_int, _c_int, _c_int, _c_i64, _c_int, _c_int, _c_int, ctypes.c_uint64,
                                        ctypes.c_uint64, _c_p, _c_p, _c_p, _c_p]),
    "nnue_load_batch_params_count": (_c_int, []),
    "nnue_engine_scratch": (_c_i64, [_c_p, _c_int]),
    "nnue_engine_evaluate_logits": (_c_int, [_c_p, _c_p, _c_int, _c_int, _c_int, _c_p, _c_p, _c_p, _c_i64, _c_p]),
    "nnue_engine_stream_state_bytes": (_c_i64, [_c_p, _c_int]),
    "nnue_engine_stream_step": (_c_int, [_c_p, _c_p, _c_p, _c_int, _c_int, _c_int, _c_p, _c_i64, _c_p, _c_p, _c_p, _c_p, _c_i64, _c_p]),
    "nnue_engine_evaluate_logits_stacks": (_c_int, [_c_p, _c_p, _c_p, _c_int, _c_int, _c_int, _c_p, _c_p, _c_p, _c_p, _c_p, _c_i64,
                                                    _c_p]),
    "nnue_engine_stream_step_stacks": (_c_int, [_c_p, _c_p, _c_p, _c_p, _c_int, _c_int, _c_int, _c_p, _c_p, _c_i64, _c_p, _c_p, _c_p,
                                                _c_p, _c_p, _c_i64, _c_p]),
    "nnue_engine_stream_update": (_c_int, [_c_p, _c_p, _c_p, _c_p, _c_i64, _c_p, _c_p, _c_i64, _c_int, _c_int, _c_p, _c_p, _c_i64, _c_p,
                                           _c_p, _c_p, _c_p, _c_p]),
    "nnue_engine_matrix_supported": (_c_int, [_c_p, _c_int, _c_int]),
    "nnue_engine_table_planes_bytes": (_c_i64, [_c_p, _c_int]),
    "nnue_engine_matrix_scratch": (_c_i64, [_c_p, _c_int, _c_int]),
    "nnue_engine_pack_table": (_c_int, [_c_p, _c_int, _c_p, _c_i64, _c_p, _c_p]),
    "nnue_engine_evaluate_logits_matrix": (_c_int, [_c_p, _c_p, _c_p, _c_int, _c_p, _c_p, _c_int, _c_int, _c_int, _c_p, _c_p, _c_p,
                                                    _c_p, _c_p, _c_i64, _c_p]),
    "nnue_engine_evaluate_logits_u8": (_c_int, [_c_p, _c_p, _c_p, _c_int, _c_int, _c_int, _c_p, _c_p, _c_p, _c_p, _c_p, _c_i64, _c_p]),
    "nnue_engine_evaluate_logits_matrix_u8": (_c_int, [_c_p, _c_p, _c_p, _c_int, _c_p, _c_int, _c_int, _c_int, _c_p, _c_p, _c_p, _c_p,
                                                       _c_p, _c_i64, _c_p]),
    "nnue_engine_stream_step_u8": (_c_int, [_c_p, _c_p, _c_p, _c_int, _c_int, _c_int, _c_p, _c_p, _c_i64, _c_p, _c_p, _c_p, _c_p, _c_p,
                                            _c_i64, _c_p]),
    "nnue_engine_quantize_model": (_c_int, [_c_p, _c_p, _c_p, _c_p, _c_p, _c_p, _c_p, _c_p, _c_p, _c_int, _c_int, _c_int, _c_int,
                                            _c_int, _c_int, _c_int, _c_int, _c_p, _c_p, _c_p, _c_p]),
    "nnue_sgd_scratch": (_c_i64, [_c_i64]),
    "nnue_multi_optim_scratch": (_c_i64, [_c_p, _c_int]),
    "nnue_multi_sgd_step": (_c_int, [_c_p, _c_p, _c_p, _c_p, _c_int, _c_p, _c_p, _c_p, _c_p, _c_f, _c_p, _c_p, _c_i64, _c_p, _c_p]),
    "nnue_multi_adam_step": (_c_int, [_c_p, _c_p, _c_p, _c_p, _c_p, _c_p, _c_int, _c_p, _c_p, _c_p, _c_p, _c_p, _c_f, _c_p, _c_p,
                                      _c_i64, _c_p, _c_p]),
    "nnue_adam_step": (_c_int, [_c_p, _c_p, _c_p, _c_p, _c_p, _c_i64, _c_f, _c_f, _c_f, _c_f, _c_f, _c_f, _c_f,
                                _c_p, _c_p, _c_i64, _c_p, _c_p]),
    "nnue_sgd_step": (_c_int, [_c_p, _c_p, _c_p, _c_i64, _c_f, _c_f, _c_f, _c_f, _c_f, _c_int,
                               _c_p, _c_p, _c_i64, _c_p, _c_int, _c_int, _c_p, _c_p, _c_p, _c_int, _c_i64, _c_i64, _c_p, _c_int, _c_p, _c_p]),
    "nnue_ftm_uses_bf16": (_c_int, [_c_int, _c_int, _c_int, _c_int, _c_int]),
    "nnue_sqnorm_partials": (_c_int, [_c_p, _c_i64, _c_p, _c_int, _c_p]),
    "nnue_dp_factor_chunk_bytes": (_c_i64, [_c_int, _c_int, _c_int, _c_i64]),
    "nnue_dp_factor_offset": (_c_i64, [_c_int, _c_int, _c_int, _c_int, _c_i64]),
    "nnue_dp_factor_pack": (_c_int, [_c_p, _c_p, _c_i64, _c_i64, _c_i64, _c_int, _c_int, _c_int, _c_p, _c_p]),
    "nnue_dp_factor_unpack": (_c_int, [_c_p, _c_int, _c_int, _c_int, _c_int, _c_i64, _c_i64, _c_i64, _c_p, _c_p, _c_p, _c_p, _c_p]),
    "nnue_ftm_gram_sq_count": (_c_i64, [_c_int, _c_int]),
    "nnue_ftm_gram_scratch": (_c_i64, [_c_int, _c_int, _c_int]),
    "nnue_ftm_gram_sqnorm": (_c_int, [_c_p, _c_p, _c_int, _c_int, _c_int, _c_int, _c_p, _c_p, _c_p]),
    "nnue_ftm_gram_sqnorm_tail": (_c_int, [_c_p, _c_p, _c_p, _c_int, _c_int, _c_int, _c_int, _c_p, _c_p, _c_p, _c_p, _c_p]),
    "nnue_ftm_backward_tail_rows": (_c_int, [_c_p, _c_p, _c_int, _c_int, _c_int, _c_int, _c_p, _c_p, _c_p]),
    "nnue_ftm_backward_weight_update": (_c_int, [_c_p, _c_p, _c_int, _c_int, _c_int, _c_int, _c_p, _c_p, _c_p, _c_f, _c_f, _c_f, _c_f,
                                                 _c_int, _c_p, _c_p]),
    "nnue_ftm_update_forward_supported": (_c_int, [_c_int, _c_int, _c_int, _c_int, _c_int]),
    "nnue_ftm_backward_weight_update_forward": (_c_int, [_c_p, _c_p, _c_int, _c_int, _c_int, _c_int, _c_p, _c_p, _c_p, _c_f, _c_f, _c_f, _c_f,
                                                         _c_int, _c_p, _c_p, _c_p, _c_int, _c_p, _c_p, _c_p, _c_i64, _c_p]),
    "nnue_adam_step_ext": (_c_int, [_c_p, _c_p, _c_p, _c_p, _c_p, _c_i64, _c_f, _c_f, _c_f, _c_f, _c_f, _c_f, _c_f,
                                    _c_p, _c_p, _c_i64, _c_p, _c_int, _c_i64, _c_i64, _c_p, _c_int, _c_p, _c_p]),
    "nnue_ftm_backward_weight_update_adam": (_c_int, [_c_p, _c_p, _c_int, _c_int, _c_int, _c_int, _c_p, _c_p, _c_p, _c_p, _c_p,
                                                      _c_f, _c_f, _c_f, _c_f, _c_f, _c_f, _c_p, _c_p]),
    "nnue_ftm_backward_weight_update_forward_adam": (_c_int, [_c_p, _c_p, _c_int, _c_int, _c_int, _c_int, _c_p, _c_p, _c_p, _c_p, _c_p,
                                                              _c_f, _c_f, _c_f, _c_f, _c_f, _c_f, _c_p,
                                                              _c_p, _c_p, _c_int, _c_p, _c_p, _c_p, _c_i64, _c_p]),
}

_lib: Optional[ctypes.CDLL] = None


class NnueHipError(RuntimeError):
    pass


def load() -> ctypes.CDLL:
    global _lib
    if _lib is not None:
        return _lib
    if not LIB_PATH.exists():
        raise NnueHipError(
            f"{LIB_PATH} is missing: build it with `python nnue-vision_amd/csrc/build.py` "
            "(or __graft_entry__.build()).  There is no CPU or eager fallback.")
    lib = ctypes.CDLL(str(LIB_PATH))
    for name, (res, args) in SIGNATURES.items():
        fn = getattr(lib, name)
        fn.restype, fn.argtypes = res, args
    got = lib.nnue_hip_abi_version()
    if got != ABI_VERSION:
        raise NnueHipError(f"libnnue_hip.so ABI {got} != binding ABI {ABI_VERSION}: rebuild")
    _lib = lib
    return lib


_recording: Optional[list] = None


class record_calls:

    def __enter__(self):
        global _recording
        self.prev, _recording = _recording, []
        self.calls = _recording
        return self.calls

    def __exit__(self, *exc):
        global _recording
        _recording = self.prev
        return False


_timing: Optional[dict] = None


class time_calls:

    def __init__(self, timers):
        self.timers = timers

    def __enter__(self):
        global _timing
        self.prev, _timing = _timing, self.timers
        return self.timers

    def __exit__(self, *exc):
        global _timing
        _timing = self.prev
        return False


_TIMED_AS = {"nnue_ftm_conv_binarize_planes": "nnue_ftm_conv_binarize", "nnue_ftm_forward_l1_planes": "nnue_ftm_forward_l1"}


def _call(name: str, *args) -> None:
    lib = load()
    fn = getattr(lib, name)
    key = _TIMED_AS.get(name, name)
    if _timing is not None and key in _timing:
        t0, t1 = torch.cuda.Event(enable_timing=True), torch.cuda.Event(enable_timing=True)
        t0.record()
        rc = fn(*args)
        t1.record()
        _timing[key].append((t0, t1))
    else:
        rc = fn(*args)
    if rc != 0:
        raise NnueHipError(f"{name} failed (code {rc}): {lib.nnue_hip_last_error().decode()}")
    if _recording is not None:
        _recording.append((name, fn, args[:-1]))


def run_plan(plan, stream_ptr: int, timers=None) -> None:
    for name, fn, args in plan:
        key = _TIMED_AS.get(name, name)
        if timers is not None and key in timers:
            t0, t1 = torch.cuda.Event(enable_timing=True), torch.cuda.Event(enable_timing=True)
            t0.record()
            rc = fn(*args, stream_ptr)
            t1.record()
            timers[key].append((t0, t1))
        else:
            rc = fn(*args, stream_ptr)
        if rc != 0:
            raise NnueHipError(f"{name} failed (code {rc}): {load().nnue_hip_last_error().decode()}")


def _stream(t: torch.Tensor) -> int:
    return torch.cuda.current_stream(t.device).cuda_stream


def _need(t: torch.Tensor, dtype, what: str, shape: Optional[Tuple[int, ...]] = None) -> torch.Tensor:
    if not isinstance(t, torch.Tensor):
        raise TypeError(f"{what}: expected a tensor, got {type(t).__name__}")
    if not t.is_cuda:
        raise NnueHipError(f"{what}: tensor is on {t.device}; the NNUE hot path runs on the GPU only "
                           "(no CPU fallback in this build)")
    if t.dtype != dtype:
        raise TypeError(f"{what}: expected {dtype}, got {t.dtype}")
    if shape is not None and tuple(t.shape) != tuple(shape):
        raise ValueError(f"{what}: expected shape {tuple(shape)}, got {tuple(t.shape)}")
    return t if t.is_contiguous() else t.contiguous()


def _ptr(t: Optional[torch.Tensor]) -> int:
    return 0 if t is None else t.data_ptr()


def round_up(v: int, m: int) -> int:
    return (v + m - 1) // m * m


@dataclass
class ActList:
    rows: torch.Tensor
    pos: torch.Tensor
    coef: torch.Tensor
    n: torch.Tensor
    coefT: torch.Tensor
    cap: int
    ldb: int

    @property
    def batch(self) -> int:
        return self.n.shape[0]

    @staticmethod
    def empty(batch: int, cap: int, num_rows: int, device) -> "ActList":
        ldb = round_up(batch, 64)
        i32 = dict(dtype=torch.int32, device=device)
        return ActList(torch.empty((batch, cap), **i32), torch.empty((batch, cap), **i32),
                       torch.empty((batch, cap), dtype=torch.float32, device=device),
                       torch.empty((batch,), **i32),
                       torch.empty((num_rows, ldb), dtype=torch.float32, device=device), cap, ldb)

# ... 356 lines not shown
def ftm_conv_binarize(images: torch.Tensor, weight: torch.Tensor, thr: torch.Tensor, stride: int, num_rows: int, l1: int,
                      conv_out: Optional[torch.Tensor] = None, fm: Optional[FeatureMatrix] = None,
                      patches: Optional[torch.Tensor] = None):
    images = _need(images, torch.float32, "images")
    if images.dim() != 4 or images.shape[1] != 3:
        raise ValueError(f"images: expected [B,3,H,W], got {tuple(images.shape)}")
    b, _, h, w = images.shape
    weight = _need(weight, torch.float32, "conv.weight")
    fps = weight.shape[0]
    if tuple(weight.shape) != (fps, 3, 3, 3):
        raise ValueError("conv.weight: expected [fps,3,3,3]")
    thr = _need(thr.reshape(-1), torch.float32, "threshold", (fps,))
    gh, gw = conv_out_hw(h, w, stride)
    if conv_out is None:
        conv_out = torch.empty((b, fps, gh, gw), dtype=torch.float32, device=images.device)
    elif tuple(conv_out.shape) != (b, fps, gh, gw):
        raise ValueError("ftm_conv_binarize: conv_out has the wrong shape")
    if fm is None:
        fm = FeatureMatrix.empty(b, fps * gh * gw, num_rows, l1, images.device)
    elif fm.batch != b or fm.positions != fps * gh * gw or fm.num_rows != num_rows:
        raise ValueError("ftm_conv_binarize: buffers do not match the map")
    if patches is not None:
        patches = _need(patches, torch.float32, "patches", (27, b * gh * gw))
        _call("nnue_ftm_conv_binarize_patches", images.data_ptr(), weight.data_ptr(), thr.data_ptr(), b, h, w, fps, int(stride), int(num_rows),
              patches.data_ptr(), conv_out.data_ptr(), fm.bits.data_ptr(), fm.n.data_ptr(), fm.sink.data_ptr(), _stream(images))
        return conv_out, fm
    _call("nnue_ftm_conv_binarize", images.data_ptr(), weight.data_ptr(), thr.data_ptr(), b, h, w, fps, int(stride), int(num_rows),
          conv_out.data_ptr(), fm.bits.data_ptr(), fm.n.data_ptr(), fm.sink.data_ptr(), _stream(images))
    return conv_out, fm


def ftm_forward(weight: torch.Tensor, bias: torch.Tensor, fm: FeatureMatrix, out: Optional[torch.Tensor] = None,
                group=None) -> torch.Tensor:
    weight = _need(weight, torch.float32, "input.weight")
    f, l1 = weight.shape
    bias = _need(bias, torch.float32, "input.bias", (l1,))
    if f != fm.num_rows:
        raise ValueError("ftm_forward: the map was built for a different table")
    if out is None:
        out = torch.empty((fm.batch, l1), dtype=torch.float32, device=weight.device)
    args = (fm.bits.data_ptr(), fm.sink.data_ptr(), weight.data_ptr(), bias.data_ptr(), fm.batch, f,
            fm.positions, l1, out.data_ptr(), fm.scratch.data_ptr(), fm.scratch.numel())
    if group is None:
        _call("nnue_ftm_forward", *args, _stream(weight))
    else:
        if group.batch != fm.batch:
            raise ValueError("ftm_forward: the bucket plan was built for another batch size")
        _call("nnue_ftm_forward_grouping", *args, fm.n.data_ptr(), group.K, group.bucket.data_ptr(), group.rows.data_ptr(),
              group.tile_bucket.data_ptr(), group.seg.data_ptr(), _stream(weight))
    return out


def ftm_forward_l1_supported(batch: int, num_rows: int, positions: int, l1: int, l2: int) -> bool:
    return bool(load().nnue_ftm_forward_l1_supported(int(batch), int(num_rows), int(positions), int(l1), int(l2)))


def ftm_forward_l1(weight: torch.Tensor, bias: torch.Tensor, fm: FeatureMatrix, w1: torch.Tensor, part: torch.Tensor,
                   out: Optional[torch.Tensor] = None) -> torch.Tensor:
    weight = _need(weight, torch.float32, "input.weight")
    f, l1 = weight.shape
    bias = _need(bias, torch.float32, "input.bias", (l1,))
    l2 = w1.shape[0]
    w1 = _need(w1, torch.float32, "classifier.0.weight", (l2, l1))
    if f != fm.num_rows:
        raise ValueError("ftm_forward_l1: the map was built for a different table")
    if not part.is_cuda or part.numel() * part.element_size() < (l1 // 64) * fm.batch * l2 * 4:
        raise ValueError("ftm_forward_l1: part buffer too small for [L1/64][B][L2] floats")
    if out is None:
        out = torch.empty((fm.batch, l1), dtype=torch.float32, device=weight.device)
    _call("nnue_ftm_forward_l1", fm.bits.data_ptr(), fm.sink.data_ptr(), weight.data_ptr(), bias.data_ptr(), w1.data_ptr(),
          fm.batch, f, fm.positions, l1, l2, out.data_ptr(), part.data_ptr(), _stream(weight))
    return out


def ftm_forward_l1_planes_supported(batch: int, num_rows: int, positions: int, l1: int, l2: int) -> bool:
    return bool(load().nnue_ftm_forward_l1_planes_supported(int(batch), int(num_rows), int(positions), int(l1), int(l2)))


def ftm_forward_planes_bytes(batch: int, num_rows: int, positions: int, l1: int) -> int:
    return int(load().nnue_ftm_forward_planes_bytes(int(batch), int(num_rows), int(positions), int(l1)))


def ftm_conv_binarize_planes(images: torch.Tensor, weight: torch.Tensor, thr: torch.Tensor, stride: int, table: torch.Tensor, l2: int,
                             planes: torch.Tensor, conv_out: Optional[torch.Tensor] = None, fm: Optional[FeatureMatrix] = None):
    images = _need(images, torch.float32, "images")
    if images.dim() != 4 or images.shape[1] != 3:
        raise ValueError(f"images: expected [B,3,H,W], got {tuple(images.shape)}")
    b, _, h, w = images.shape
    weight = _need(weight, torch.float32, "conv.weight")
    fps = weight.shape[0]
    if tuple(weight.shape) != (fps, 3, 3, 3):
        raise ValueError("conv.weight: expected [fps,3,3,3]")
    thr = _need(thr.reshape(-1), torch.float32, "threshold", (fps,))
    table = _need(table, torch.float32, "input.weight")
    f, l1 = table.shape
    planes = _need(planes, torch.uint8, "planes")
    gh, gw = conv_out_hw(h, w, stride)
    if conv_out is None:
        conv_out = torch.empty((b, fps, gh, gw), dtype=torch.float32, device=images.device)
    elif tuple(conv_out.shape) != (b, fps, gh, gw):
        raise ValueError("ftm_conv_binarize_planes: conv_out has the wrong shape")
    if fm is None:
        fm = FeatureMatrix.empty(b, fps * gh * gw, f, l1, images.device)
    elif fm.batch != b or fm.positions != fps * gh * gw or fm.num_rows != f:
        raise ValueError("ftm_conv_binarize_planes: buffers do not match the map")
    _call("nnue_ftm_conv_binarize_planes", images.data_ptr(), weight.data_ptr(), thr.data_ptr(), b, h, w, fps, int(stride), f,
          table.data_ptr(), l1, int(l2), planes.data_ptr(), planes.numel(), conv_out.data_ptr(), fm.bits.data_ptr(), fm.n.data_ptr(),
          fm.sink.data_ptr(), _stream(images))
    return conv_out, fm


def ftm_forward_l1_planes(weight: torch.Tensor, bias: torch.Tensor, fm: FeatureMatrix, planes: torch.Tensor, w1: torch.Tensor,
                          part: torch.Tensor, out: Optional[torch.Tensor] = None) -> torch.Tensor:
    weight = _need(weight, torch.float32, "input.weight")
    f, l1 = weight.shape
    bias = _need(bias, torch.float32, "input.bias", (l1,))
    l2 = w1.shape[0]
    w1 = _need(w1, torch.float32, "classifier.0.weight", (l2, l1))
    planes = _need(planes, torch.uint8, "planes")
    if f != fm.num_rows:
        raise ValueError("ftm_forward_l1_planes: the map was built for a different table")
    if not part.is_cuda or part.numel() * part.element_size() < (l1 // 64) * fm.batch * l2 * 4:
        raise ValueError("ftm_forward_l1_planes: part buffer too small for [L1/64][B][L2] floats")
    if out is None:
        out = torch.empty((fm.batch, l1), dtype=torch.float32, device=weight.device)
    _call("nnue_ftm_forward_l1_planes", fm.bits.data_ptr(), fm.sink.data_ptr(), planes.data_ptr(), planes.numel(), weight.data_ptr(),
          bias.data_ptr(), w1.data_ptr(), fm.batch, f, fm.positions, l1, l2, out.data_ptr(), part.data_ptr(), _stream(weight))
    return out


def ftm_backward_weight(d_out: torch.Tensor, fm: FeatureMatrix, d_weight: Optional[torch.Tensor] = None,
                        d_bias: Optional[torch.Tensor] = None, want_weight: bool = True, want_bias: bool = True):
    d_out = _need(d_out, torch.float32, "d_out")
    if d_out.dim() != 2 or d_out.shape[0] != fm.batch:
        raise ValueError("ftm_backward_weight: d_out does not match the map")
    l1 = d_out.shape[1]
    if want_weight and d_weight is None:
        d_weight = torch.empty((fm.num_rows, l1), dtype=torch.float32, device=d_out.device)
    if want_bias and d_bias is None:
        d_bias = torch.empty((l1,), dtype=torch.float32, device=d_out.device)
    _call("nnue_ftm_backward_weight", fm.bits.data_ptr(), fm.sink.data_ptr(), d_out.data_ptr(), fm.batch, fm.num_rows,
          fm.positions, l1, _ptr(d_weight if want_weight else None), _ptr(d_bias if want_bias else None), _stream(d_out))
    return d_weight, d_bias


def ftm_backward_values(d_out: torch.Tensor, weight: torch.Tensor, fm: FeatureMatrix,
                        dst: Optional[torch.Tensor] = None) -> torch.Tensor:
    d_out = _need(d_out, torch.float32, "d_out")
    weight = _need(weight, torch.float32, "input.weight")
    b, l1 = d_out.shape
    if tuple(weight.shape) != (fm.num_rows, l1) or b != fm.batch:
        raise ValueError("ftm_backward_values: shape mismatch")
    if dst is None:
        dst = torch.empty((b, fm.positions), dtype=torch.float32, device=d_out.device)
    elif dst.numel() != b * fm.positions:
        raise ValueError("ftm_backward_values: dst has the wrong size")
    _call("nnue_ftm_backward_values_ws", fm.bits.data_ptr(), d_out.data_ptr(), weight.data_ptr(), b, fm.num_rows, fm.positions,
          l1, dst.data_ptr(), None, 0, _stream(d_out))
    return dst


def ftm_backward_sq_count(b: int, f: int, p: int, l1: int) -> int:
    return int(load().nnue_ftm_backward_sq_count(b, f, p, l1))


def ftm_backward_cw_supported(b: int, f: int, p: int, l1: int, l2: int) -> bool:
    return bool(load().nnue_ftm_backward_cw_supported(b, f, p, l1, l2))


def ftm_backward_ste_chunks(b: int, f: int, p: int, l1: int, h: int, w: int, stride: int) -> int:
    return int(load().nnue_ftm_backward_ste_chunks(b, f, p, l1, h, w, stride))


def ftm_backward(d_out: torch.Tensor, weight: torch.Tensor, fm: FeatureMatrix, d_weight: Optional[torch.Tensor] = None,
                 d_bias: Optional[torch.Tensor] = None, dst: Optional[torch.Tensor] = None, ft: Optional[torch.Tensor] = None,
                 d_z1: Optional[torch.Tensor] = None, d_w1: Optional[torch.Tensor] = None,
                 sq_partial: Optional[torch.Tensor] = None, buckets=None, small: Optional["NnueClsRider"] = None, ste=None):
    d_out = _need(d_out, torch.float32, "d_out")
    weight = _need(weight, torch.float32, "input.weight")
    b, l1 = d_out.shape
    if weight.shape != (fm.num_rows, l1) or b != fm.batch:
        raise ValueError("ftm_backward: shape mismatch")
    if d_weight is None:
        d_weight = torch.empty((fm.num_rows, l1), dtype=torch.float32, device=d_out.device)
    if d_bias is None:
        d_bias = torch.empty((l1,), dtype=torch.float32, device=d_out.device)
    if dst is None and ste is None:
        dst = torch.empty((b, fm.positions), dtype=torch.float32, device=d_out.device)
    elif dst is not None and dst.numel() != b * fm.positions:
        raise ValueError("ftm_backward: dst has the wrong size")
    ste_args = (None, None, None, None, 0, 0, 0, None, 0)
    if ste is not None:
        images, conv_out, thr, stride, part = ste[:5]
        patches = ste[5] if len(ste) > 5 else None
        images = _need(images, torch.float32, "images")
        conv_out = _need(conv_out, torch.float32, "conv_out")
        thr = _need(thr, torch.float32, "visual_threshold")
        if images.dim() != 4 or images.shape[:2] != (b, 3) or conv_out.numel() != b * fm.positions or part.device != d_out.device:
            raise ValueError("ftm_backward: STE operands have the wrong shape")
        h, w = images.shape[2], images.shape[3]
        if patches is not None:
            gh, gw = conv_out_hw(h, w, stride)
            patches = _need(patches, torch.float32, "patches", (27, b * gh * gw))
        ste_args = (images.data_ptr(), _ptr(patches), conv_out.data_ptr(), thr.data_ptr(), h, w, int(stride), part.data_ptr(),
                    part.numel() * part.element_size())
    l2 = 0
    rows = b if buckets is None else buckets.tiles * 16
    if d_w1 is not None:
        ft = _need(ft, torch.float32, "ft")
        d_z1 = _need(d_z1, torch.float32, "d_z1")
        l2 = d_w1.shape[-2]
        want = (l2, l1) if buckets is None else (buckets.K, l2, l1)
        if ft.shape != (rows, l1) or d_z1.numel() != rows * l2 or tuple(d_w1.shape) != want or not d_w1.is_contiguous():
            raise ValueError("ftm_backward: ft / d_z1 / d_w1 shape mismatch")
    args = (fm.bits.data_ptr(), fm.sink.data_ptr(), d_out.data_ptr(), weight.data_ptr(), b, fm.num_rows,
            fm.positions, l1, d_weight.data_ptr(), d_bias.data_ptr(), _ptr(dst),
            _ptr(ft if d_w1 is not None else None), _ptr(d_z1 if d_w1 is not None else None), l2, _ptr(d_w1), _ptr(sq_partial))
    rider = ctypes.pointer(small) if small is not None else None
    if buckets is None:
        _call("nnue_ftm_backward", *args, rider, *ste_args, _stream(d_out))
    else:
        _call("nnue_ftm_backward_bucketed", *args, buckets.K, buckets.seg.data_ptr(), rows, rider, *ste_args, _stream(d_out))
    return d_weight, d_bias, dst


def classifier_train_rider(pairwise: bool, b: int, l1: int, l2: int, l3: int, c: int, h1, h2, sample_loss, loss, grads, scratch,
                           buckets: Optional["BucketPlan"] = None) -> "NnueClsRider":
    out = NnueClsRider()
    _, d_b1, d_w2, d_b2, d_w3, d_b3 = grads
    rc = load().nnue_classifier_train_rider(int(bool(pairwise)), b, l1, l2, l3, c, h1.data_ptr(), h2.data_ptr(), sample_loss.data_ptr(),
                                            loss.data_ptr(), d_b1.data_ptr(), d_w2.data_ptr(), d_b2.data_ptr(), d_w3.data_ptr(),
                                            d_b3.data_ptr(), scratch.data_ptr(), scratch.numel(),
                                            buckets.ref if buckets is not None else None, ctypes.byref(out))
    if rc != 0:
        raise NnueHipError(f"nnue_classifier_train_rider failed (code {rc}): {load().nnue_hip_last_error().decode()}")
    return out


class BucketPlan:

    def __init__(self, batch: int, buckets: int, device):
        self.batch, self.K = int(batch), int(buckets)
        self.tiles = int(load().nnue_bucket_tile_count(self.batch, self.K))
        i32 = dict(dtype=torch.int32, device=device)
        self.bucket = torch.zeros((self.batch,), **i32)
        self.rows = torch.full((self.tiles * 16,), -1, **i32)
        self.tile_bucket = torch.full((self.tiles,), -1, **i32)
        self.seg = torch.zeros((self.K + 1,), **i32)
        self.cstruct = NnueBuckets(self.K, self.bucket.data_ptr(), self.rows.data_ptr(), self.tile_bucket.data_ptr(),
                                   self.seg.data_ptr(), self.tiles)

    @property
    def ref(self):
        return ctypes.byref(self.cstruct)


def bucket_group(n: torch.Tensor, positions: int, buckets: int, plan: Optional[BucketPlan] = None) -> BucketPlan:
    n = _need(n, torch.int32, "active-feature counts")
    b = n.numel()
    if plan is None:
        plan = BucketPlan(b, buckets, n.device)
    elif plan.batch != b or plan.K != buckets:
        raise ValueError("bucket_group: plan was built for another batch size / bucket count")
    _call("nnue_bucket_group", n.data_ptr(), b, int(positions), int(buckets), plan.bucket.data_ptr(), plan.rows.data_ptr(),
          plan.tile_bucket.data_ptr(), plan.seg.data_ptr(), _stream(n))
    return plan


def classifier_scratch_bytes(b: int, l1: int, l2: int, l3: int, buckets: int = 1) -> int:
    return int(load().nnue_classifier_scratch_bucketed(b, l1, l2, l3, buckets))


def _cls_shapes(w1, b1, w2, b2, w3, b3, l1: int, buckets: Optional[BucketPlan]):
    k = buckets.K if buckets is not None else 1
    lead = (k,) if w1.dim() == 3 else ()
    if (w1.dim() == 3) != (buckets is not None) or (lead and w1.shape[0] != k):
        raise ValueError("stacked [K, out, in] classifier weights need a BucketPlan with the same K (and vice versa)")
    l2, l3, c = w1.shape[-2], w2.shape[-2], w3.shape[-2]
    w1 = _need(w1, torch.float32, "classifier.0.weight", (*lead, l2, l1))
    w2 = _need(w2, torch.float32, "classifier.2.weight", (*lead, l3, l2))
    w3 = _need(w3, torch.float32, "classifier.4.weight", (*lead, c, l3))
    if b1 is not None:
        b1 = _need(b1, torch.float32, "classifier.0.bias", (*lead, l2))
        b2 = _need(b2, torch.float32, "classifier.2.bias", (*lead, l3))
        b3 = _need(b3, torch.float32, "classifier.4.bias", (*lead, c))
    return w1, b1, w2, b2, w3, b3, l2, l3, c, k


def classifier_forward(x, pairwise: bool, w1, b1, w2, b2, w3, b3, clip: float = 0.0,
                       scratch: Optional[torch.Tensor] = None, out=None, buckets: Optional[BucketPlan] = None):
    x = _need(x, torch.float32, "classifier input")
    if x.dim() != 2:
        raise ValueError(f"classifier input: expected [B,L1], got {tuple(x.shape)}")
    b, l1 = x.shape
    w1, b1, w2, b2, w3, b3, l2, l3, c, k = _cls_shapes(w1, b1, w2, b2, w3, b3, l1, buckets)
    dev = x.device
    if scratch is None:
        scratch = torch.empty((classifier_scratch_bytes(b, l1, l2, l3, k),), dtype=torch.uint8, device=dev)
    if out is None:
        h1 = torch.empty((b, l2), dtype=torch.float32, device=dev)
        h2 = torch.empty((b, l3), dtype=torch.float32, device=dev)
        logits = torch.empty((b, c), dtype=torch.float32, device=dev)
# ... 352 lines not shown
```

### nnue-vision_amd/nnue_hip/trainer.py

```python
from __future__ import annotations

import ctypes
from dataclasses import dataclass
from typing import Dict, List, Optional, Tuple

import os

import torch
import torch.distributed as dist

from . import lib

SKIP = ("nnue2score",)


@dataclass
class FlatLayout:
    names: List[str]
    shapes: List[Tuple[int, ...]]
    offsets: List[int]
    count: int

    @staticmethod
    def of(model: torch.nn.Module, align: int = 4, pad_to: int = 1) -> "FlatLayout":
# ... 155 lines not shown
        tbl_ok = tbl_hi > tbl_lo and tbl_lo % 4 == 0 and tbl_hi % 4 == 0
        big_table = self.F * self.L1 * 4 >= (32 << 20)
        gb = B * self.dp.world
        self.factor_exchange = (self.dp.collectives and self.use_mfma and optimizer == "sgd" and self.dp.buckets == 1 and tbl_ok
                                and self.layout.names[:3] == ["visual_threshold", "conv.weight", "input.weight"]
                                and gb * self.L1 <= (1 << 24) and ((gb + 15) // 16) * ((self.L1 + 15) // 16) <= 65536
                                and fx_mode != "0" and (fx_mode == "1" or big_table))
        self.fx = None
        if self.factor_exchange:
            self.fx = lib.FactorExchange(self.dp.world, self.dp.rank, B, self.P, self.F, self.L1, head=tbl_lo, tail_lo=tbl_hi,
                                         tail=self.layout.count - tbl_hi, device=self.dev)
            self.fm.sink = self.fx.sink
        self.bits = lib.FeatureBits.empty(B, self.P, self.F, self.L1, self.dev) if self.use_bits else None
        self.act = lib.ActList.empty(B, self.P, self.F, self.dev) if self.ft_path == "list" else None
        self.ft = torch.empty((B, self.L1), **f32)
        self.h1 = torch.empty((B, self.L2), **f32)
        self.h2 = torch.empty((B, self.L3), **f32)
        self.logits = torch.empty((B, self.C), **f32)
        self.sample_loss = torch.empty((B,), **f32)
        self.loss = torch.zeros((), **f32)
        self.loss_ring = torch.zeros((max(1, input_slots),), **f32)
        self.d_logits = torch.empty((B, self.C), **f32)
        self.d_ft = self.fx.d_ft if self.fx is not None else torch.empty((B, self.L1), **f32)
        self.d_conv_out = torch.empty((B, self.P), **f32)
        self.grad_norm = torch.zeros((), **f32)
        u8 = dict(dtype=torch.uint8, device=self.dev)
        self.cls_scratch = torch.empty((max(lib.classifier_scratch_bytes(B, self.L1, self.L2, self.L3, self.K),
                                            lib.classifier_train_scratch_bytes(B, self.L1, self.L2, self.L3, self.C, self.K)),), **u8)
        self.bucket_plan = lib.BucketPlan(B, self.K, self.dev) if self.K > 1 else None
        self.ste_scratch = torch.empty((max(16, lib.load().nnue_ste_conv_backward_scratch(B, self.fps, self.gh, self.gw)),), **u8)
        self.sgd_scratch = torch.empty((lib.sgd_scratch_bytes(self.layout.count),), **u8)
        self.defer_ste = (not self.dp.collectives and optimizer == "sgd" and os.environ.get("NNUE_DEFER_STE", "1") != "0"
                          and self.fps * 28 <= 4096 and self.layout.names[:2] == ["visual_threshold", "conv.weight"])
        self.ste_chunks = lib.ste_conv_backward_chunks(B, self.fps, self.gh, self.gw)
        self.fuse_l1 = (self.K == 1 and self.use_mfma and os.environ.get("NNUE_FUSE_L1", "1") != "0"
                        and lib.ftm_forward_l1_supported(B, self.F, self.P, self.L1, self.L2))
        self.fwd_planes = (self.fuse_l1 and not self.use_patches and os.environ.get("NNUE_FTM_FWD_PLANES", "1") != "0"
                           and lib.ftm_forward_l1_planes_supported(B, self.F, self.P, self.L1, self.L2))
        self.planes = (torch.empty((lib.ftm_forward_planes_bytes(B, self.F, self.P, self.L1),), **u8) if self.fwd_planes else None)
        mode = os.environ.get("NNUE_DP_SHARDED_UPDATE", "auto")
        self.sharded_update = (self.dp.collectives and optimizer == "sgd" and self.dp.buckets == 1 and mode != "0"
                               and not self.factor_exchange and (mode == "1" or self.layout.count * 4 >= (64 << 20)))
        if self.sharded_update:
            per = self.layout.count // self.dp.world
            self.grad_shard = torch.empty((per,), **f32)
            self.norm_parts = 256
            self.local_partials = torch.empty((self.norm_parts,), **f32)
            self.all_partials = torch.empty((self.norm_parts * self.dp.world,), **f32)
        self.capture_collectives = (self.dp.collectives and use_graph and self.dp.backend == "nccl" and self.dp.buckets == 1
                                    and os.environ.get("NNUE_DP_CAPTURE", "1") != "0")
        self.lr_dev = torch.full((1,), float(lr), **f32)
        self.steps_done = 0
        self.use_graph = use_graph
        self._g_local, self._g_update = {}, None
        self._plan_local = self._plan_seg = self._plan_update_first = self._plan_update = None
        self._plan_slot = 0
        self._side = torch.cuda.Stream(device=self.dev) if use_graph else None
        self.merge_backward = os.environ.get("NNUE_FTM_SPLIT_BACKWARD", "0") != "1"
        self.ride_dw1 = (self.use_mfma and self.merge_backward and os.environ.get("NNUE_FTM_RIDE_DW1", "1") != "0"
                         and lib.ftm_backward_cw_supported(B, self.F, self.P, self.L1, self.L2))
        want = os.environ.get("NNUE_FUSE_TABLE_UPDATE", "auto")
        self.fuse_table_update = (self.use_mfma and not self.dp.collectives and tbl_ok and B * self.L1 <= (1 << 24) and want != "0"
                                  and (big_table or want == "1"))
        self.grads_materialised = not (self.fuse_table_update or self.factor_exchange)
        self.sq_partial = self.sq_range = self.gram = self.clip_coef = None
        n_sq = lib.ftm_backward_sq_count(B, self.F, self.P, self.L1) if (self.use_mfma and self.merge_backward) else 0
        if not self.grads_materialised:
            self.ride_dw1 = False
            self.sq_partial = torch.empty((int(lib.load().nnue_ftm_gram_sq_count(gb, self.L1)),), **f32)
            self.sq_range = (tbl_lo, tbl_hi)
            self.gram = torch.zeros((lib.ftm_gram_scratch(self.fx.g_fm if self.factor_exchange else self.fm),), **f32)
            self.clip_coef = torch.ones((), **f32)
        elif n_sq > 0 and not self.dp.collectives and optimizer == "sgd" and tbl_ok and os.environ.get("NNUE_NORM_PARTIALS", "1") != "0":
            self.sq_partial = torch.empty((n_sq,), **f32)
            self.sq_range = (tbl_lo, tbl_hi)
        ste_chunks = lib.ftm_backward_ste_chunks(B, self.F, self.P, self.L1, self.H, self.W, self.stride) if self.use_mfma else 0
        self.ride_ste = (self.defer_ste and self.merge_backward and not self.fuse_table_update
                         and not self.factor_exchange and ste_chunks > 0 and os.environ.get("NNUE_FTM_RIDE_STE", "1") != "0")
        if self.ride_ste:
            self.ste_chunks = ste_chunks
            need = self.fps * 28 * ste_chunks * 4
            if self.ste_scratch.numel() < need:
                self.ste_scratch = torch.empty((need,), **u8)
        self.fuse_next_forward = ((self.fuse_table_update or self.factor_exchange) and not self.fuse_l1 and self.K == 1
                                  and os.environ.get("NNUE_FUSE_NEXT_FORWARD", "1") != "0"
                                  and lib.ftm_update_forward_supported(gb if self.factor_exchange else B, self.F, self.P, self.L1, B))
        self.fm_alt = lib.FeatureMatrix.empty(B, self.P, self.F, self.L1, self.dev) if self.fuse_next_forward else None
        if self.fm_alt is not None and self.fx is not None:
            self.fm_alt.sink = self.fx.sink
        self._last_alt = False
        self.d_z1 = self.ft_rider = None
        if self.ride_dw1 and self.K == 1:
            off = lib.classifier_train_dz1_offset(B, self.L1, self.L2, self.L3, self.C, True)
            self.d_z1 = self.cls_scratch[off:off + B * self.L2 * 4].view(torch.float32).view(B, self.L2)
            self.ft_rider = self.ft
        elif self.ride_dw1:
            rows = self.bucket_plan.tiles * 16
            o_dz, o_x = lib.classifier_train_grouped_offsets(B, self.L1, self.L2, self.L3, self.C, self.K)
            self.d_z1 = self.cls_scratch[o_dz:o_dz + rows * self.L2 * 4].view(torch.float32).view(rows, self.L2)
            self.ft_rider = self.cls_scratch[o_x:o_x + rows * self.L1 * 4].view(torch.float32).view(rows, self.L1)
        self.ride_small = self.ride_dw1 and os.environ.get("NNUE_CLS_RIDE_SMALL", "1") != "0"
        self.fuse_tail_dx = (self.fuse_l1 and self.ride_small and os.environ.get("NNUE_CLS_FUSE_TAIL_DX", "1") != "0"
                             and lib.classifier_train_fused_tail_supported(B, self.L1, self.L2, self.L3, self.C, self.K))
        self._riders = {}

    def _set_hyper(self, key: str, value: float) -> None:
        if self._hyper[key] == value:
            return
        if key == "lr":
            self._hyper[key] = value
            self.lr_dev.fill_(value)
            return
        if key == "momentum" and self.optimizer == "sgd" and bool(value) != (self.flat_momentum is not None):
            raise ValueError("momentum cannot be switched on or off after construction (the buffer layout is fixed)")
        self._hyper[key] = value
        self._plan_update_first = self._plan_update = None
        self._g_update = None
        for key_ in [k for k in self._g_local if k[1] in ("full", "full_dp", "many")]:
            del self._g_local[key_]

    lr = property(lambda self: self._hyper["lr"], lambda self, v: self._set_hyper("lr", float(v)))
    momentum = property(lambda self: self._hyper["momentum"], lambda self, v: self._set_hyper("momentum", float(v)))
    weight_decay = property(lambda self: self._hyper["weight_decay"], lambda self, v: self._set_hyper("weight_decay", float(v)))
    max_grad_norm = property(lambda self: self._hyper["max_grad_norm"], lambda self, v: self._set_hyper("max_grad_norm", float(v)))

    def set_lr(self, lr: float) -> None:
        self.lr = lr

    def _cls_params(self):
        p = self.p
        return [p[f"classifier.classifier.{i}.{n}"] for i in (0, 2, 4) for n in ("weight", "bias")]

    SEGMENTS = ("front", "transpose", "forward", "ft_wgrad", "cls_wgrad", "tail")

    def _cls_step(self, phases: int) -> None:
        g = self.g
        cls_grads = tuple(g[f"classifier.classifier.{i}.{n}"] for i in (0, 2, 4) for n in ("weight", "bias"))
        lib.classifier_train_step(self.ft, True, *self._cls_params(), self.labels, 1.0, self.clip, scratch=self.cls_scratch,
                                  out=(self.h1, self.h2, self.logits), loss_out=(self.sample_loss, self.loss),
                                  grads=cls_grads, d_x=self.d_ft, phases=phases, buckets=self.bucket_plan)

    def _rider(self, loss: torch.Tensor):
        key = loss.data_ptr()
        if key not in self._riders:
            g = self.g
            grads = tuple(g[f"classifier.classifier.{i}.{n}"] for i in (0, 2, 4) for n in ("weight", "bias"))
            self._riders[key] = lib.classifier_train_rider(True, self.B, self.L1, self.L2, self.L3, self.C, self.h1, self.h2,
                                                           self.sample_loss, loss, grads, self.cls_scratch, self.bucket_plan)
        return self._riders[key]

    def _segment(self, name: str) -> None:
        p, g = self.p, self.g
        if name == "front":
            if self.fwd_planes:
                lib.ftm_conv_binarize_planes(self.images, p["conv.weight"], p["visual_threshold"], self.stride, p["input.weight"], self.L2,
                                             self.planes, conv_out=self.conv_out, fm=self.fm)
                return
            if self.use_mfma:
                lib.ftm_conv_binarize(self.images, p["conv.weight"], p["visual_threshold"], self.stride, self.F, self.L1,
                                      conv_out=self.conv_out, fm=self.fm, patches=self.patches)
                return
            lib.conv3x3_forward(self.images, p["conv.weight"], self.stride, out=self.conv_out)
            if self.use_bits:
                lib.binarize_bits(self.conv_out, p["visual_threshold"], self.F, self.L1, bits=self.bits, stages=1)
            else:
                lib.binarize_features(self.conv_out, p["visual_threshold"], self.F, act=self.act)
        elif name == "transpose":
            if self.use_bits:
                lib.binarize_bits(self.conv_out, p["visual_threshold"], self.F, self.L1, bits=self.bits, stages=2)
        elif name == "forward":
            if self.bucket_plan is not None and not self.use_mfma:
                feats = self.bits if self.use_bits else self.act
                lib.bucket_group(feats.n, self.P, self.K, plan=self.bucket_plan)
            if self.use_mfma and self.fuse_l1:
                if self.fwd_planes:
                    lib.ftm_forward_l1_planes(p["input.weight"], p["input.bias"], self.fm, self.planes, p["classifier.classifier.0.weight"],
                                              self.cls_scratch, out=self.ft)
                else:
                    lib.ftm_forward_l1(p["input.weight"], p["input.bias"], self.fm, p["classifier.classifier.0.weight"], self.cls_scratch,
                                       out=self.ft)
                self._cls_step((123 if self.fuse_tail_dx else 59 if self.ride_small else 27) if self.ride_dw1 else 13)
                return
            if self.use_mfma:
                lib.ftm_forward(p["input.weight"], p["input.bias"], self.fm, out=self.ft, group=self.bucket_plan)
            elif self.use_bits:
                lib.ftb_forward(p["input.weight"], p["input.bias"], self.bits, out=self.ft)
            else:
                lib.ft_forward(p["input.weight"], p["input.bias"], self.act, out=self.ft)
            self._cls_step((51 if self.ride_small else 19) if self.ride_dw1 else 5)
        elif name == "ft_wgrad":
            if self.factor_exchange:
                lib.ftm_backward_tail_rows(self.d_ft, self.fm, g["input.weight"], g["input.bias"])
            elif self.fuse_table_update:
                lib.ftm_gram_sqnorm(self.fm, self.d_ft, self.gram, self.sq_partial, tail=(g["input.weight"], g["input.bias"]))
            elif self.use_mfma and self.merge_backward:
                lib.ftm_backward(self.d_ft, p["input.weight"], self.fm, d_weight=g["input.weight"], d_bias=g["input.bias"],
                                 dst=None if self.ride_ste else self.d_conv_out, ft=self.ft_rider, d_z1=self.d_z1,
                                 d_w1=g["classifier.classifier.0.weight"] if self.ride_dw1 else None, sq_partial=self.sq_partial,
                                 buckets=self.bucket_plan, small=self._rider(self.loss) if self.ride_small else None,
                                 ste=((self.images, self.conv_out, p["visual_threshold"], self.stride, self.ste_scratch, self.patches)
                                      if self.ride_ste else None))
            elif self.use_mfma:
                lib.ftm_backward_weight(self.d_ft, self.fm, d_weight=g["input.weight"], d_bias=g["input.bias"])
            elif self.use_bits:
                lib.ftb_backward_weight(self.d_ft, self.bits, d_weight=g["input.weight"], d_bias=g["input.bias"])
            else:
                lib.ft_backward_weight(self.d_ft, self.act, self.F, d_weight=g["input.weight"], d_bias=g["input.bias"])
        elif name == "cls_wgrad":
            if not self.ride_dw1:
                self._cls_step(6)
        elif name == "tail":
            if self.use_mfma and self.merge_backward and not self.fuse_table_update and not self.factor_exchange:
                pass
            elif self.use_mfma:
                lib.ftm_backward_values(self.d_ft, p["input.weight"], self.fm, dst=self.d_conv_out)
            elif self.use_bits:
                lib.ftb_backward_values(self.d_ft, p["input.weight"], self.bits, dst=self.d_conv_out)
            else:
                lib.ft_backward_values(self.d_ft, p["input.weight"], self.act, self.P, dst=self.d_conv_out)
            if self.ride_ste:
                return
            if self.use_patches:
                lib.ste_conv_backward_patches(self.patches, self.conv_out, p["visual_threshold"], self.d_conv_out, self.gh, self.gw,
                                              d_thr=g["visual_threshold"], d_weight=g["conv.weight"], scratch=self.ste_scratch,
                                              stages=1 if self.defer_ste else 3)
            else:
                lib.ste_conv_backward(self.images, self.conv_out, p["visual_threshold"], self.d_conv_out, self.stride,
                                      d_thr=g["visual_threshold"], d_weight=g["conv.weight"], scratch=self.ste_scratch,
                                      stages=1 if self.defer_ste else 3)
        else:
            raise KeyError(name)

    def _forward(self) -> None:
        for name in ("front", "forward"):
            self._segment(name)

    def _local_step(self) -> None:
        for name in self.SEGMENTS:
            self._segment(name)

    def _small_update(self, first: bool, scale: float) -> None:
        ext = (self.sq_partial, *self.sq_range) if self.sq_partial is not None else None
        elsewhere = not self.grads_materialised
        if self.optimizer == "adam":
            lib.adam_step(self.flat_params, self.flat_grads, self.flat_exp_avg, self.flat_exp_avg_sq, self.adam_step_count,
                          self.lr, self.betas, self.eps, self.weight_decay, self.max_grad_norm, scale, self.grad_norm,
                          self.sgd_scratch, lr_dev=self.lr_dev, ext=ext, coef_out=self.clip_coef, ext_applied_elsewhere=elsewhere)
            return
        ste = ((self.ste_scratch, self.ste_chunks, self.fps, self.g["visual_threshold"], self.g["conv.weight"])
               if self.defer_ste else None)
        lib.sgd_step(self.flat_params, self.flat_grads, self.flat_momentum, self.lr, self.momentum, self.weight_decay,
                     self.max_grad_norm, scale, first, self.grad_norm, self.sgd_scratch, ste=ste, ext=ext,
                     coef_out=self.clip_coef, ext_applied_elsewhere=elsewhere, lr_dev=self.lr_dev)

    def _table_update(self, first: bool, scale: float, d_ft: torch.Tensor, fm, nxt=None) -> None:
        lo, hi = self.sq_range
        forward = () if nxt is None else (nxt, self.p["input.bias"], self.ft)
        if self.optimizer == "adam":
            fn = lib.ftm_backward_weight_update_adam if nxt is None else lib.ftm_backward_weight_update_forward_adam
            opt = (self.flat_exp_avg[lo:hi], self.flat_exp_avg_sq[lo:hi], self.clip_coef, self.adam_step_count, self.lr, self.betas,
                   self.eps, self.weight_decay, scale)
        else:
            fn = lib.ftm_backward_weight_update if nxt is None else lib.ftm_backward_weight_update_forward
            mom = self.flat_momentum[lo:hi] if self.flat_momentum is not None else None
            opt = (mom, self.clip_coef, self.lr, self.momentum, self.weight_decay, scale, first)
        fn(d_ft, fm, self.p["input.weight"], *opt, *forward, lr_dev=self.lr_dev)

    def _next_map(self, slot: int, nxt) -> None:
        lib.ftm_conv_binarize(self.inputs[slot][0], self.p["conv.weight"], self.p["visual_threshold"], self.stride, self.F, self.L1,
                              conv_out=self.conv_out, fm=nxt, patches=self.patches)

    def _update(self, first: bool, grad_scale: Optional[float] = None) -> None:
        scale = self.dp.grad_scale if grad_scale is None else grad_scale
        self._small_update(first, scale)
        if self.fuse_table_update:
            self._table_update(first, scale, self.d_ft, self.fm)

    def _exchange_and_update(self, first: bool, grad_scale: Optional[float] = None, alt: bool = False,
                             next_slot: Optional[int] = None) -> None:
        if self.factor_exchange:
            fx, scale = self.fx, (self.dp.grad_scale if grad_scale is None else grad_scale)
            fx.pack(self.fm_alt if alt else self.fm, self.flat_grads)
            self.dp.all_gather_chunks(fx.chunks)
            fx.unpack(self.flat_grads)
# ... 345 lines not shown
```

Measured before the change: 7.347 million images/sec.

## Precompute split-bf16 value planes of the feature table during conv-binarize for backward GEMM

Measured after the change: 7.745 million images/sec, median of 6. 5.4% higher.

```diff
diff --git a/include/nnue_hip.h b/include/nnue_hip.h
--- a/include/nnue_hip.h
+++ b/include/nnue_hip.h
@@ -143,6 +143,21 @@
                       const nnue_cls_rider* small, const float* ste_images, const float* ste_patches, const float* ste_conv_out,
                       const float* ste_thr, int H, int W, int stride, float* ste_partial, int64_t ste_partial_bytes,
                       nnue_stream_t stream);
+
+int nnue_ftm_value_planes_supported(int B, int F, int P, int L1, int H, int W, int stride);
+int64_t nnue_ftm_value_planes_bytes(int B, int F, int P, int L1);
+
+int nnue_ftm_conv_binarize_value_planes(const float* images, const float* weight, const float* thr, int B, int H, int W,
+                                        int fps, int stride, int F, const float* table, int L1, int L2, void* planes,
+                                        int64_t planes_bytes, void* val_planes, int64_t val_planes_bytes, float* conv_out,
+                                        uint8_t* bits, int32_t* n, float* sink, nnue_stream_t stream);
+
+int nnue_ftm_backward_planes(const uint8_t* bits, const float* sink, const float* d_out, const float* weight,
+                             int B, int F, int P, int L1, float* d_weight, float* d_bias, float* d_conv_out,
+                             const float* ft, const float* d_z1, int L2, float* d_w1, float* sq_partial,
+                             const nnue_cls_rider* small, const float* ste_images, const float* ste_patches, const float* ste_conv_out,
+                             const float* ste_thr, int H, int W, int stride, float* ste_partial, int64_t ste_partial_bytes,
+                             const void* val_planes, int64_t val_planes_bytes, nnue_stream_t stream);
 
 
 int64_t nnue_classifier_scratch(int B, int L1, int L2, int L3);
diff --git a/nnue-vision_amd/csrc/feature_kernels.hip b/nnue-vision_amd/csrc/feature_kernels.hip
--- a/nnue-vision_amd/csrc/feature_kernels.hip
+++ b/nnue-vision_amd/csrc/feature_kernels.hip
@@ -74,6 +74,27 @@
   const int id = (int)blockIdx.x;
   if (id >= B * slices) {
     forward_planes_write(pa, id - B * slices);
+    return;
+  }
+  ConvParamsPlain prm{w, thr};
+  conv_binarize_body<kFullUnroll, false>(img, prm, out, bits, n, sink, H, W, fps, stride, Gh, Gw, F, slices, id % B, id / B, w_lds, [] {});
+}
+
+#include "value_planes.h"
+
+template <bool kFullUnroll>
+__global__ __launch_bounds__(256) void conv_binarize_planes2_kernel(const float* __restrict__ img, const float* __restrict__ w,
+                                                                    const float* __restrict__ thr, float* __restrict__ out,
+                                                                    uint8_t* __restrict__ bits, int* __restrict__ n,
+                                                                    float* __restrict__ sink, int B, int H, int W, int fps, int stride,
+                                                                    int Gh, int Gw, int F, int slices, FwdPlaneArgs pa, int fwd_riders,
+                                                                    ValPlaneArgs va) {
+  extern __shared__ __attribute__((aligned(16))) float w_lds[];
+  const int id = (int)blockIdx.x;
+  if (id >= B * slices) {
+    const int rider = id - B * slices;
+    if (rider < fwd_riders) forward_planes_write(pa, rider);
+    else value_planes_write(va, rider - fwd_riders);
     return;
   }
   ConvParamsPlain prm{w, thr};
@@ -452,6 +473,9 @@
   int L1, L2;
   void* planes;
   int64_t planes_bytes;
+  void* val_planes = nullptr;
+  int64_t val_planes_bytes = 0;
+  bool want_val = false;
 };
 
 int conv_binarize_impl(const char* who, const float* images, const float* weight, const float* thr, int B, int H, int W, int fps, int stride, int F,
@@ -466,14 +490,29 @@
   NNUE_REQUIRE(G * fps < (1ll << 30) && (long long)B * G * fps < (1ll << 40), NNUE_E_SHAPE, "%s: map too large", who);
   NNUE_REQUIRE(!patches || 27ll * B * G * 4 < (1ll << 31), NNUE_E_SHAPE, "%s: the im2col buffer must stay below 2 GiB", who);
   const int P = (int)(G * fps);
+  const bool fwd_ride = ride.table && (ride.planes || !ride.want_val);
   if (ride.table) {
-    NNUE_REQUIRE(ride.planes, NNUE_E_ARG, "%s: null pointer", who);
-    NNUE_REQUIRE(nnue_ftm_forward_l1_planes_supported(B, F, P, ride.L1, ride.L2), NNUE_E_SHAPE,
-                 "%s: B=%d F=%d P=%d L1=%d L2=%d is not a planes-fed forward shape (nnue_ftm_forward_l1_planes_supported)", who, B, F, P, ride.L1,
-                 ride.L2);
-    NNUE_REQUIRE(nnue_aligned16(ride.table) && nnue_aligned16(ride.planes), NNUE_E_ARG, "%s: pointers must be 16-byte aligned", who);
-    NNUE_REQUIRE(ride.planes_bytes >= nnue_ftm_forward_planes_bytes(B, F, P, ride.L1), NNUE_E_SCRATCH, "%s: plane buffer of %lld bytes, needs %lld", who,
-                 (long long)ride.planes_bytes, (long long)nnue_ftm_forward_planes_bytes(B, F, P, ride.L1));
+    NNUE_REQUIRE(nnue_aligned16(ride.table), NNUE_E_ARG, "%s: pointers must be 16-byte aligned", who);
+    if (fwd_ride) {
+      NNUE_REQUIRE(ride.planes, NNUE_E_ARG, "%s: null pointer", who);
+      NNUE_REQUIRE(nnue_ftm_forward_l1_planes_supported(B, F, P, ride.L1, ride.L2), NNUE_E_SHAPE,
+                   "%s: B=%d F=%d P=%d L1=%d L2=%d is not a planes-fed forward shape (nnue_ftm_forward_l1_planes_supported)", who, B, F, P,
+                   ride.L1, ride.L2);
+      NNUE_REQUIRE(nnue_aligned16(ride.planes), NNUE_E_ARG, "%s: pointers must be 16-byte aligned", who);
+      NNUE_REQUIRE(ride.planes_bytes >= nnue_ftm_forward_planes_bytes(B, F, P, ride.L1), NNUE_E_SCRATCH,
+                   "%s: plane buffer of %lld bytes, needs %lld", who, (long long)ride.planes_bytes,
+                   (long long)nnue_ftm_forward_planes_bytes(B, F, P, ride.L1));
+    }
+    if (ride.want_val) {
+      NNUE_REQUIRE(ride.val_planes, NNUE_E_ARG, "%s: null pointer", who);
+      NNUE_REQUIRE(fps == 8 && nnue_ftm_value_planes_supported(B, F, P, ride.L1, H, W, stride), NNUE_E_SHAPE,
+                   "%s: B=%d F=%d P=%d L1=%d H=%d W=%d stride=%d is not a value-planes shape (nnue_ftm_value_planes_supported)", who, B, F, P,
+                   ride.L1, H, W, stride);
+      NNUE_REQUIRE(nnue_aligned16(ride.val_planes), NNUE_E_ARG, "%s: pointers must be 16-byte aligned", who);
+      NNUE_REQUIRE(ride.val_planes_bytes >= nnue_ftm_value_planes_bytes(B, F, P, ride.L1), NNUE_E_SCRATCH,
+                   "%s: value-plane buffer of %lld bytes, needs %lld", who, (long long)ride.val_planes_bytes,
+                   (long long)nnue_ftm_value_planes_bytes(B, F, P, ride.L1));
+    }
   }
   hipStream_t s = static_cast<hipStream_t>(stream);
   const int threads = G <= 64 ? 64 : (G <= 128 ? 128 : 256);
@@ -485,7 +524,15 @@
   if (ride.table) {
     const int direct = (F - 1 < P) ? F - 1 : P, ktiles = (direct + kBfK - 1) / kBfK, parts = 256 / threads;
     const FwdPlaneArgs pa{ride.table, static_cast<unsigned char*>(ride.planes), (unsigned)((size_t)direct * ride.L1 * 4), ride.L1, ktiles, parts};
-    const int riders = (ride.L1 / 64) * ktiles * parts;
+    const int riders = fwd_ride ? (ride.L1 / 64) * ktiles * parts : 0;
+    if (ride.want_val) {
+      const int vk = (ride.L1 + kBfK - 1) / kBfK, v_riders = (int)((G + 7) / 8) * vk * parts;
+      const ValPlaneArgs va{ride.table, static_cast<unsigned char*>(ride.val_planes), (unsigned)((size_t)F * ride.L1 * 4), ride.L1, F, (int)G, vk, parts};
+      const dim3 grid2((unsigned)(B * slices + riders + v_riders));
+      hipLaunchKernelGGL((conv_binarize_planes2_kernel<true>), grid2, dim3(threads), lds, s, images, weight, thr, conv_out, bits, n, sink, B, H, W,
+                         fps, stride, Gh, Gw, F, slices, pa, riders, va);
+      return nnue_launch_status(who);
+    }
     const dim3 grid((unsigned)(B * slices + riders));
     if (fps <= 16)
       hipLaunchKernelGGL((conv_binarize_planes_kernel<true>), grid, dim3(threads), lds, s, images, weight, thr, conv_out, bits, n, sink, B, H, W, fps,
@@ -529,6 +576,15 @@
   NNUE_REQUIRE(table && planes, NNUE_E_ARG, "nnue_ftm_conv_binarize_planes: null pointer");
   return conv_binarize_impl("nnue_ftm_conv_binarize_planes", images, weight, thr, B, H, W, fps, stride, F, conv_out, nullptr, bits, n, sink, stream,
                             PlaneRide{table, L1, L2, planes, planes_bytes});
+}
+
+extern "C" int nnue_ftm_conv_binarize_value_planes(const float* images, const float* weight, const float* thr, int B, int H, int W, int fps,
+                                                   int stride, int F, const float* table, int L1, int L2, void* planes, int64_t planes_bytes,
+                                                   void* val_planes, int64_t val_planes_bytes, float* conv_out, uint8_t* bits, int32_t* n,
+                                                   float* sink, nnue_stream_t stream) {
+  NNUE_REQUIRE(table && val_planes, NNUE_E_ARG, "nnue_ftm_conv_binarize_value_planes: null pointer");
+  return conv_binarize_impl("nnue_ftm_conv_binarize_value_planes", images, weight, thr, B, H, W, fps, stride, F, conv_out, nullptr, bits, n, sink,
+                            stream, PlaneRide{table, L1, L2, planes, planes_bytes, val_planes, val_planes_bytes, true});
 }
 
 extern "C" int nnue_binarize_features(const float* conv_out, const float* thr, int B, int fps, int Gh, int Gw, int F,
diff --git a/nnue-vision_amd/csrc/ftm_kernels.hip b/nnue-vision_amd/csrc/ftm_kernels.hip
--- a/nnue-vision_amd/csrc/ftm_kernels.hip
+++ b/nnue-vision_amd/csrc/ftm_kernels.hip
@@ -19,6 +19,7 @@
 };
 using u32x4 = __attribute__((__vector_size__(4 * sizeof(unsigned)))) unsigned;
 #include "forward_planes.h"
+#include "value_planes.h"
 
 template <bool U8>
 __device__ __forceinline__ u32x4 mat_load(__amdgpu_buffer_rsrc_t rsrc, const Mat& m, int outer, int inner) {
@@ -155,6 +156,11 @@
     return (j >> 3) * G + (hw < G ? hw : G - 1);
   }
 };
+struct ValStePlanesEpi : ValSteEpi {
+  const unsigned char* __restrict__ planes;
+  unsigned planes_bytes;
+  int ktiles;
+};
 constexpr float kFtmSteSharpness = 10.0f;
 
 template <class Epi, class = void>
@@ -212,20 +218,21 @@
       }
 }
 
-template <int BM>
+template <int BM, bool W14 = false>
 struct StePre {
-  uint8_t bit[BM / 32][2][4];
-  float cv[BM / 32][2][4], th[2];
+  static constexpr int kTM = W14 ? BM / 16 : BM / 32, kTN = W14 ? 1 : 2;
+  uint8_t bit[kTM][kTN][4];
+  float cv[kTM][kTN][4], th[kTN];
 };
-template <int BM>
-__device__ __forceinline__ void ste_prefetch(const ValSteEpi& e, StePre<BM>& p, int M, int m_base, int tile_n, int m0, int n0, int r, int q) {
-#pragma unroll
-  for (int t = 0; t < 2; ++t) {
+template <int BM, bool W14 = false>
+__device__ __forceinline__ void ste_prefetch(const ValSteEpi& e, StePre<BM, W14>& p, int M, int m_base, int tile_n, int m0, int n0, int r, int q) {
+#pragma unroll
+  for (int t = 0; t < StePre<BM, W14>::kTN; ++t) {
     const int j = n0 + 16 * t + r, c = j >> 3, hw = tile_n * 8 + (j & 7);
     const int pp = c * e.G + (hw < e.G ? hw : 0);
     p.th[t] = e.thr[c];
 #pragma unroll
-    for (int i = 0; i < BM / 32; ++i)
+    for (int i = 0; i < StePre<BM, W14>::kTM; ++i)
 #pragma unroll
       for (int ee = 0; ee < 4; ++ee) {
         const int m = min(m_base + m0 + 16 * i + 4 * q + ee, M - 1);
@@ -235,11 +242,12 @@
   }
 }
 
-template <int BM, int BN>
-__device__ __forceinline__ void ste_tile(float* __restrict__ smem, const ValSteEpi& e, const f32x4 (&acc)[BM / 32][BN / 32], const SteFrag<BM>& f,
-                                         const StePre<BM>& pre, int M, int m_base, int tile_n, int m0, int n0, int tile) {
+template <int BM, int BN, bool W14 = false>
+__device__ __forceinline__ void ste_tile(float* __restrict__ smem, const ValSteEpi& e,
+                                         const f32x4 (&acc)[StePre<BM, W14>::kTM][StePre<BM, W14>::kTN], const SteFrag<BM>& f,
+                                         const StePre<BM, W14>& pre, int M, int m_base, int tile_n, int m0, int n0, int tile) {
   static_assert(BN == 64, "a tile holds the 8 channels of 8 positions");
-  constexpr int TM = BM / 32, TN = BN / 32, LDA = 8 * BM + 4;
+  constexpr int TM = StePre<BM, W14>::kTM, TN = StePre<BM, W14>::kTN, LDA = 8 * BM + 4;
   const int tid = threadIdx.x, lane = tid & 63;
   const int wave = __builtin_amdgcn_readfirstlane(tid >> 6);
   const int r = lane & 15, q = lane >> 4;
@@ -1246,6 +1254,96 @@
   gemm_tile_bf6<BM, BN, Epi, KT, ABL>(smem, ma, mb, epi, M, N, 0, K, tiles_n, blockIdx.x, 0);
 }
 
+constexpr int kValPlanesLds = 2 * 3 * 32 * kBfK * 2;
+template <class Epi>
+__device__ __forceinline__ void gemm_tile_val_planes(unsigned char* __restrict__ smem, const Mat& ma, const Epi& epi, int M, int tiles_n, int tile) {
+  constexpr int BM = 32, KB = kBfK / 32, PA = BM * kBfK * 2, kSet = 3 * PA;
+  const __amdgpu_buffer_rsrc_t rsa = __builtin_amdgcn_make_buffer_rsrc(const_cast<void*>(ma.p), 0, ma.bytes, 0x00020000);
+  const __amdgpu_buffer_rsrc_t rsb = __builtin_amdgcn_make_buffer_rsrc(const_cast<unsigned char*>(epi.planes), 0, epi.planes_bytes, 0x00020000);
+  const int tid = threadIdx.x, lane = tid & 63;
+  const int wave = __builtin_amdgcn_readfirstlane(tid >> 6);
+  const int r = lane & 15, q = lane >> 4;
+  const int tile_n = tile % tiles_n, tile_m = tile / tiles_n;
+  const int m_base = tile_m * BM, n0 = 16 * wave;
+  const int ktiles = epi.ktiles;
+  u32x4 ra[2][2];
+  auto fetch_a = [&](int k0) {
+#pragma unroll
+    for (int i = 0; i < 2; ++i) {
+      const int g = tid + 256 * i, row = g >> 4, k = k0 + (g & 15) * 8;
+      ra[i][0] = mat_load<false>(rsa, ma, m_base + row, k);
+      ra[i][1] = mat_load<false>(rsa, ma, m_base + row, k + 4);
+    }
+  };
+  auto stage = [&](unsigned char* __restrict__ As) {
+#pragma unroll
+    for (int i = 0; i < 2; ++i) {
+      const int g = tid + 256 * i, row = g >> 4, c = g & 15;
+      u32x4 hi, mid, lo;
+      split8(ra[i][0], ra[i][1], hi, mid, lo);
+      *reinterpret_cast<u32x4*>(As + bf_img(row, c)) = hi;
+      *reinterpret_cast<u32x4*>(As + PA + bf_img(row, c)) = mid;
+      *reinterpret_cast<u32x4*>(As + 2 * PA + bf_img(row, c)) = lo;
+    }
+  };
+  u32x4 rb[KB][3];
+  auto fetch_b = [&](int kt, int kb) {
+    const int at = (tile_n * ktiles + kt) * kValPlaneBlock + val_plane_frag(wave, kb);
+    rb[kb][0] = __builtin_amdgcn_raw_buffer_load_b128(rsb, lane * 16, at, 0);
+    rb[kb][2] = __builtin_amdgcn_raw_buffer_load_b128(rsb, lane * 16, at + 2 * kValPlaneBytes, 0);
+    rb[kb][1] = __builtin_amdgcn_raw_buffer_load_b128(rsb, lane * 16, at + kValPlaneBytes, 0);
+  };
+  f32x4 acc[2][1];
+#pragma unroll
+  for (int i = 0; i < 2; ++i) acc[i][0] = (f32x4){0.f, 0.f, 0.f, 0.f};
+  auto contract_block = [&](const unsigned char* __restrict__ As, int kb) {
+    const int c = kb * 4 + q;
+    bf16x8 a[3][2];
+#pragma unroll
+    for (int pl = 0; pl < 3; ++pl)
+#pragma unroll
+      for (int i = 0; i < 2; ++i) a[pl][i] = *reinterpret_cast<const bf16x8*>(As + pl * PA + bf_img(16 * i + r, c));
+    constexpr int pa[6] = {2, 0, 1, 1, 0, 0}, pb[6] = {0, 2, 1, 0, 1, 0};
+#pragma unroll
+    for (int s6 = 0; s6 < 6; ++s6)
+#pragma unroll
+      for (int i = 0; i < 2; ++i)
+        acc[i][0] = __builtin_amdgcn_mfma_f32_16x16x32_bf16(a[pa[s6]][i], __builtin_bit_cast(bf16x8, rb[kb][pb[s6]]), acc[i][0], 0, 0, 0);
+  };
+  fetch_a(0);
+  __builtin_amdgcn_sched_barrier(0);
+#pragma unroll
+  for (int kb = 0; kb < KB; ++kb) fetch_b(0, kb);
+  __builtin_amdgcn_sched_barrier(0);
+  int kt = 0;
+  for (; kt + 1 < ktiles; ++kt) {
+    unsigned char* __restrict__ As = smem + (kt & 1) * kSet;
+    stage(As);
+    __syncthreads();
+    fetch_a((kt + 1) * kBfK);
+    __builtin_amdgcn_sched_barrier(0);
+#pragma unroll
+    for (int kb = 0; kb < KB; ++kb) {
+      contract_block(As, kb);
+      fetch_b(kt + 1, kb);
+      __builtin_amdgcn_sched_barrier(0);
+    }
+  }
+  unsigned char* __restrict__ As = smem + (kt & 1) * kSet;
+  stage(As);
+  __syncthreads();
+  SteFrag<BM> stef;
+  StePre<BM, true> stepre;
+  ste_pixels<BM>(epi, stef, M, m_base, tile_n, wave, r, q);
+  ste_prefetch<BM, true>(epi, stepre, M, m_base, tile_n, 0, n0, r, q);
+  __builtin_amdgcn_sched_barrier(0);
+#pragma unroll
+  for (int kb = 0; kb < KB; ++kb) contract_block(As, kb);
+  ste_pixels_select<BM>(stef, r);
+  __syncthreads();
+  ste_tile<BM, 64, true>(reinterpret_cast<float*>(smem), epi, acc, stef, stepre, M, m_base, tile_n, 0, n0, tile);
+}
+
 template <int BM, int BN, bool AKC, class Epi>
 __global__ __launch_bounds__(256) void ftm_gemm_bf_kernel(Mat ma, Mat mb, Epi epi, int M, int N, int K, int klen, int tiles_n, GroupArgs ga) {
   __shared__ __attribute__((aligned(16))) unsigned char smem[gemm_bf_lds_bytes<BM, BN, kBfK>()];
@@ -1499,7 +1597,10 @@
 __global__ __launch_bounds__(256) void ftm_backward_bf_kernel(Mat wa, Mat wb, BwwEpi we, int wM, int wN, int wK, int w_tiles_n, int n_w,
                                                               Mat va, Mat vb, VE ve, int vM, int vN, int vK, int v_tiles_n, int n_v,
                                                               CwArgs c, TailRows t, SmallWgrad sw) {
-  constexpr int kW = gemm_bf_lds_bytes<WM, 64, W64 ? kBf64K : kBfK>(), kV = V6 ? gemm_bf6_lds_bytes<VM, VN>() : gemm_lds_floats<VM, VN, VK, true, true>() * 4;
+  constexpr bool VP = std::is_same<VE, ValStePlanesEpi>::value;
+  static_assert(!VP || (VM == 32 && VN == 64 && VK == kBfK && !V6), "the planes-fed value tile is 32 x 64 x 128");
+  constexpr int kW = gemm_bf_lds_bytes<WM, 64, W64 ? kBf64K : kBfK>(),
+                kV = VP ? kValPlanesLds : V6 ? gemm_bf6_lds_bytes<VM, VN>() : gemm_lds_floats<VM, VN, VK, true, true>() * 4;
   constexpr int kC = gemm_lds_floats<32, 64, 128, false, false>() * 4;
   constexpr int kWV = kW > kV ? kW : kV;
   constexpr int kLds = kWV > kC ? kWV : kC;
@@ -1508,7 +1609,8 @@
   float* smem = reinterpret_cast<float*>(smem_b);
   const int blk = blockIdx.x;
   if (blk < n_v) {
-    if constexpr (V6) gemm_tile_bf6<VM, VN, VE>(smem_b, va, vb, ve, vM, vN, 0, vK, v_tiles_n, blk, 0);
+    if constexpr (VP) gemm_tile_val_planes<VE>(smem_b, va, ve, vM, v_tiles_n, blk);
+    else if constexpr (V6) gemm_tile_bf6<VM, VN, VE>(smem_b, va, vb, ve, vM, vN, 0, vK, v_tiles_n, blk, 0);
     else gemm_tile<VM, VN, VK, true, true, VE>(smem, va, vb, ve, vM, vN, 0, vK, v_tiles_n, blk, 0);
   } else if (blk < n_v + n_w) {
     if constexpr (W64) gemm_tile_bf64<WM, false, BwwEpi>(smem_b, wa, wb, we, wM, wN, 0, wK, w_tiles_n, blk - n_v, 0);
@@ -2004,6 +2106,10 @@
   float* partial;
   int64_t partial_bytes;
 };
+struct ValPlanes {
+  const void* p;
+  int64_t bytes;
+};
 
 int64_t ste_ride_tiles(int B, int F, int P, int L1, int H, int W, int stride) {
   if (!nnue_ftm_supported(F, P, L1) || !shape_ok(B, F, P, L1) || H <= 0 || W <= 0 || stride <= 0) return 0;
@@ -2018,6 +2124,29 @@
 }
 }
 
+namespace {
+int64_t val_planes_tiles(int B, int F, int P, int L1) {
+  if (env_int("NNUE_FTM_VAL_PLANES", 1) == 0) return 0;
+  if (!nnue_ftm_supported(F, P, L1) || !shape_ok(B, F, P, L1) || P % 8 != 0 || L1 % 8 != 0) return 0;
+  bool big = false;
+  if (!merged_backward_shape(B, F, P, L1, &big) || merged_bf_wm() != 64 || !merged_w64()) return 0;
+  if (big || plan(B, P, L1, true, false).cfg != 0) return 0;
+  const int64_t tiles = (int64_t)((B + 31) / 32) * ((P / 8 + 7) / 8);
+  if (tiles < env_int("NNUE_FTM_VAL_PLANES_MIN_TILES", 256)) return 0;
+  return (int64_t)((P / 8 + 7) / 8) * ((L1 + kBfK - 1) / kBfK) * kValPlaneBlock < (1ll << 31) ? tiles : 0;
+}
+}
+
+extern "C" int nnue_ftm_value_planes_supported(int B, int F, int P, int L1, int H, int W, int stride) {
+  const int64_t tiles = val_planes_tiles(B, F, P, L1);
+  return tiles > 0 && ste_ride_tiles(B, F, P, L1, H, W, stride) == tiles;
+}
+
+extern "C" int64_t nnue_ftm_value_planes_bytes(int B, int F, int P, int L1) {
+  if (B <= 0 || F <= 1 || P <= 0 || L1 <= 0 || P % 8 != 0 || L1 % 8 != 0) return 0;
+  return (int64_t)((P / 8 + 7) / 8) * ((L1 + kBfK - 1) / kBfK) * kValPlaneBlock;
+}
+
 extern "C" int64_t nnue_ftm_backward_ste_chunks(int B, int F, int P, int L1, int H, int W, int stride) {
   return ste_ride_tiles(B, F, P, L1, H, W, stride);
 }
@@ -2050,7 +2179,7 @@
 int ftm_backward_impl(const uint8_t* bits, const float* sink, const float* d_out, const float* weight, int B, int F, int P, int L1,
                       float* d_weight, float* d_bias, float* d_conv_out, const float* ft, const float* d_z1, int L2, float* d_w1,
                       float* sq_partial, int K, const int32_t* seg, int grouped_rows, const nnue_cls_rider* small, const SteArgs* ste,
-                      nnue_stream_t stream);
+                      nnue_stream_t stream, const ValPlanes* vp = nullptr);
 }
 extern "C" int nnue_ftm_backward(const uint8_t* bits, const float* sink, const float* d_out, const float* weight, int B, int F, int P,
                                  int L1, float* d_weight, float* d_bias, float* d_conv_out, const float* ft, const float* d_z1, int L2,
@@ -2059,6 +2188,17 @@
   const SteArgs sa{ste_images, ste_patches, ste_conv_out, ste_thr, H, W, stride, ste_partial, ste_partial_bytes};
   return ftm_backward_impl(bits, sink, d_out, weight, B, F, P, L1, d_weight, d_bias, d_conv_out, ft, d_z1, L2, d_w1, sq_partial, 1, nullptr, 0,
                            small, ste_partial ? &sa : nullptr, stream);
+}
+extern "C" int nnue_ftm_backward_planes(const uint8_t* bits, const float* sink, const float* d_out, const float* weight, int B, int F, int P,
+                                        int L1, float* d_weight, float* d_bias, float* d_conv_out, const float* ft, const float* d_z1, int L2,
+                                        float* d_w1, float* sq_partial, const nnue_cls_rider* small, const float* ste_images,
+                                        const float* ste_patches, const float* ste_conv_out, const float* ste_thr, int H, int W, int stride,
+                                        float* ste_partial, int64_t ste_partial_bytes, const void* val_planes, int64_t val_planes_bytes,
+                                        nnue_stream_t stream) {
+  const SteArgs sa{ste_images, ste_patches, ste_conv_out, ste_thr, H, W, stride, ste_partial, ste_partial_bytes};
+  const ValPlanes vp{val_planes, val_planes_bytes};
+  return ftm_backward_impl(bits, sink, d_out, weight, B, F, P, L1, d_weight, d_bias, d_conv_out, ft, d_z1, L2, d_w1, sq_partial, 1, nullptr, 0,
+                           small, ste_partial ? &sa : nullptr, stream, &vp);
 }
 extern "C" int nnue_ftm_backward_bucketed(const uint8_t* bits, const float* sink, const float* d_out, const float* weight, int B, int F,
                                           int P, int L1, float* d_weight, float* d_bias, float* d_conv_out, const float* ft_grouped,
@@ -2077,7 +2217,7 @@
 int ftm_backward_impl(const uint8_t* bits, const float* sink, const float* d_out, const float* weight, int B, int F, int P, int L1,
                       float* d_weight, float* d_bias, float* d_conv_out, const float* ft, const float* d_z1, int L2, float* d_w1,
                       float* sq_partial, int K, const int32_t* seg, int grouped_rows, const nnue_cls_rider* small, const SteArgs* ste,
-                      nnue_stream_t stream) {
+                      nnue_stream_t stream, const ValPlanes* vp) {
   NNUE_REQUIRE(bits && sink && d_out && weight && d_weight && d_bias && (d_conv_out || ste), NNUE_E_ARG, "nnue_ftm_backward: null pointer");
   const int64_t ste_tiles = ste ? ste_ride_tiles(B, F, P, L1, ste->H, ste->W, ste->stride) : 0;
   NNUE_REQUIRE(!ste || ((ste->img || ste->patches) && ste->conv_out && ste->thr && ste->partial), NNUE_E_ARG,
@@ -2093,6 +2233,14 @@
   NNUE_REQUIRE(nnue_ftm_supported(F, P, L1), NNUE_E_SHAPE, "nnue_ftm_backward: P=%d and L1=%d must be multiples of 4", P, L1);
   NNUE_REQUIRE(nnue_aligned16(bits) && nnue_aligned16(d_out) && nnue_aligned16(weight), NNUE_E_ARG,
                "nnue_ftm_backward: pointers must be 16-byte aligned");
+  const bool planes_fed = vp && ste && nnue_ftm_value_planes_supported(B, F, P, L1, ste->H, ste->W, ste->stride);
+  if (vp) {
+    NNUE_REQUIRE(vp->p, NNUE_E_ARG, "nnue_ftm_backward_planes: null pointer");
+    NNUE_REQUIRE(nnue_aligned16(vp->p), NNUE_E_ARG, "nnue_ftm_backward_planes: pointers must be 16-byte aligned");
+    NNUE_REQUIRE(!planes_fed || vp->bytes >= nnue_ftm_value_planes_bytes(B, F, P, L1), NNUE_E_SCRATCH,
+                 "nnue_ftm_backward_planes: value-plane buffer of %lld bytes, needs %lld", (long long)vp->bytes,
+                 (long long)nnue_ftm_value_planes_bytes(B, F, P, L1));
+  }
   hipStream_t st = static_cast<hipStream_t>(stream);
   const int direct = (F - 1 < P) ? F - 1 : P;
   const Shape sw = plan(direct > 0 ? direct : 1, L1, B, false, false), sv = plan(B, P, L1, true, false);
@@ -2158,7 +2306,16 @@
   const bool v6 = merged_values_bf6(B, F, P, L1);
   const bool w64 = merged_w64();
   if (ste) {
-    if (v_small)
+    if (planes_fed) {
+      const int ktiles = (L1 + kBfK - 1) / kBfK;
+      ValStePlanesEpi vps{};
+      static_cast<ValSteEpi&>(vps) = vs;
+      vps.planes = static_cast<const unsigned char*>(vp->p);
+      vps.planes_bytes = (unsigned)nnue_ftm_value_planes_bytes(B, F, P, L1);
+      vps.ktiles = ktiles;
+      hipLaunchKernelGGL((ftm_backward_bf_kernel<64, 32, 64, 128, false, true, ValStePlanesEpi>), grid, dim3(256), 0, st, wa, wb, we, direct, L1, B,
+                         swr.tiles_n, n_w, va, vb, vps, B, P, L1, v_tiles_n, n_v, cw, t, sgw);
+    } else if (v_small)
       hipLaunchKernelGGL((ftm_backward_bf_kernel<64, 32, 64, 128, false, true, ValSteEpi>), grid, dim3(256), 0, st, wa, wb, we, direct, L1, B,
                          swr.tiles_n, n_w, va, vb, vs, B, P, L1, v_tiles_n, n_v, cw, t, sgw);
     else if (v6)
@@ -2529,6 +2686,6 @@
   if (which == 1) return plan(direct, L1, B, false, false, true).cfg >= 6;
   if (which == 2) { bool big = false; return merged_backward_shape(B, F, P, L1, &big) ? merged_bf_wm() != 0 : plan(direct, L1, B, false, false, true).cfg >= 6; }
   if (which == 4) return values_bf6(B, P, L1);
-  if (which == 5) return merged_values_bf6(B, F, P, L1);
+  if (which == 5) return merged_values_bf6(B, F, P, L1) || val_planes_tiles(B, F, P, L1) > 0;
   return 1;
 }
diff --git a/nnue-vision_amd/csrc/value_planes.h b/nnue-vision_amd/csrc/value_planes.h
--- /dev/null
+++ b/nnue-vision_amd/csrc/value_planes.h
@@ -0,0 +1,46 @@
+#pragma once
+
+constexpr int kValPlaneBytes = 64 * kBfK * 2;
+constexpr int kValPlaneBlock = 3 * kValPlaneBytes;
+
+__device__ __forceinline__ int val_plane_frag(int w, int kb) { return (w * (kBfK / 32) + kb) * 1024; }
+
+__device__ __forceinline__ int val_plane_row(int tile_n, int n, int G, int F) {
+  const int hw = tile_n * 8 + (n & 7);
+  const int p = (n >> 3) * G + (hw < G ? hw : G - 1);
+  return p < F - 1 ? p : F - 1;
+}
+
+struct ValPlaneArgs {
+  const float* __restrict__ weight;
+  unsigned char* __restrict__ planes;
+  unsigned w_bytes;
+  int L1, F, G, ktiles, parts;
+};
+
+__device__ __forceinline__ void value_planes_write(const ValPlaneArgs& a, int rider) {
+  const int block = rider / a.parts, part = rider - block * a.parts;
+  const int tile_n = block / a.ktiles, kt = block - tile_n * a.ktiles;
+  const int vt = part * (int)blockDim.x + (int)threadIdx.x;
+  const __amdgpu_buffer_rsrc_t rs = __builtin_amdgcn_make_buffer_rsrc(const_cast<float*>(a.weight), 0, a.w_bytes, 0x00020000);
+  u32x4 raw[4][2];
+#pragma unroll
+  for (int i = 0; i < 4; ++i) {
+    const int ci = vt + 256 * i, lane = ci & 63, g = ci >> 6;
+    const int n = (g >> 2) * 16 + (lane & 15), j = kt * kBfK + (g & 3) * 32 + (lane >> 4) * 8;
+    const bool in = j < a.L1;
+    const int off = (val_plane_row(tile_n, n, a.G, a.F) * a.L1 + j) * 4;
+    raw[i][0] = __builtin_amdgcn_raw_buffer_load_b128(rs, in ? off : 0x7ffffff0, 0, 0);
+    raw[i][1] = __builtin_amdgcn_raw_buffer_load_b128(rs, in ? off + 16 : 0x7ffffff0, 0, 0);
+  }
+  unsigned char* __restrict__ dst = a.planes + (size_t)block * kValPlaneBlock;
+#pragma unroll
+  for (int i = 0; i < 4; ++i) {
+    u32x4 hi, mid, lo;
+    split8(raw[i][0], raw[i][1], hi, mid, lo);
+    const int at = (vt + 256 * i) * 16;
+    *reinterpret_cast<u32x4*>(dst + at) = hi;
+    *reinterpret_cast<u32x4*>(dst + kValPlaneBytes + at) = mid;
+    *reinterpret_cast<u32x4*>(dst + 2 * kValPlaneBytes + at) = lo;
+  }
+}
diff --git a/nnue-vision_amd/nnue_hip/lib.py b/nnue-vision_amd/nnue_hip/lib.py
--- a/nnue-vision_amd/nnue_hip/lib.py
+++ b/nnue-vision_amd/nnue_hip/lib.py
@@ -85,6 +85,13 @@
     "nnue_ftm_backward": (_c_int, [_c_p, _c_p, _c_p, _c_p, _c_int, _c_int, _c_int, _c_int, _c_p, _c_p, _c_p,
                                    _c_p, _c_p, _c_int, _c_p, _c_p, _c_rider, _c_p, _c_p, _c_p, _c_p, _c_int, _c_int, _c_int,
                                    _c_p, _c_i64, _c_p]),
+    "nnue_ftm_value_planes_supported": (_c_int, [_c_int, _c_int, _c_int, _c_int, _c_int, _c_int, _c_int]),
+    "nnue_ftm_value_planes_bytes": (_c_i64, [_c_int, _c_int, _c_int, _c_int]),
+    "nnue_ftm_conv_binarize_value_planes": (_c_int, [_c_p, _c_p, _c_p, _c_int, _c_int, _c_int, _c_int, _c_int, _c_int, _c_p, _c_int, _c_int, _c_p,
+                                                     _c_i64, _c_p, _c_i64, _c_p, _c_p, _c_p, _c_p, _c_p]),
+    "nnue_ftm_backward_planes": (_c_int, [_c_p, _c_p, _c_p, _c_p, _c_int, _c_int, _c_int, _c_int, _c_p, _c_p, _c_p,
+                                          _c_p, _c_p, _c_int, _c_p, _c_p, _c_rider, _c_p, _c_p, _c_p, _c_p, _c_int, _c_int, _c_int,
+                                          _c_p, _c_i64, _c_p, _c_i64, _c_p]),
     "nnue_ftm_backward_bucketed": (_c_int, [_c_p, _c_p, _c_p, _c_p, _c_int, _c_int, _c_int, _c_int, _c_p, _c_p, _c_p,
                                             _c_p, _c_p, _c_int, _c_p, _c_p, _c_int, _c_p, _c_int, _c_rider, _c_p, _c_p, _c_p,
                                             _c_p, _c_int, _c_int, _c_int, _c_p, _c_i64, _c_p]),
@@ -246,7 +253,8 @@
         return False
 
 
-_TIMED_AS = {"nnue_ftm_conv_binarize_planes": "nnue_ftm_conv_binarize", "nnue_ftm_forward_l1_planes": "nnue_ftm_forward_l1"}
+_TIMED_AS = {"nnue_ftm_conv_binarize_planes": "nnue_ftm_conv_binarize", "nnue_ftm_forward_l1_planes": "nnue_ftm_forward_l1",
+             "nnue_ftm_conv_binarize_value_planes": "nnue_ftm_conv_binarize", "nnue_ftm_backward_planes": "nnue_ftm_backward"}
 
 
 def _call(name: str, *args) -> None:
@@ -769,7 +777,8 @@
 
 
 def ftm_conv_binarize_planes(images: torch.Tensor, weight: torch.Tensor, thr: torch.Tensor, stride: int, table: torch.Tensor, l2: int,
-                             planes: torch.Tensor, conv_out: Optional[torch.Tensor] = None, fm: Optional[FeatureMatrix] = None):
+                             planes: torch.Tensor, conv_out: Optional[torch.Tensor] = None, fm: Optional[FeatureMatrix] = None,
+                             val_planes: Optional[torch.Tensor] = None):
     images = _need(images, torch.float32, "images")
     if images.dim() != 4 or images.shape[1] != 3:
         raise ValueError(f"images: expected [B,3,H,W], got {tuple(images.shape)}")
@@ -781,7 +790,8 @@
     thr = _need(thr.reshape(-1), torch.float32, "threshold", (fps,))
     table = _need(table, torch.float32, "input.weight")
     f, l1 = table.shape
-    planes = _need(planes, torch.uint8, "planes")
+    if planes is not None or val_planes is None:
+        planes = _need(planes, torch.uint8, "planes")
     gh, gw = conv_out_hw(h, w, stride)
     if conv_out is None:
         conv_out = torch.empty((b, fps, gh, gw), dtype=torch.float32, device=images.device)
@@ -791,6 +801,12 @@
         fm = FeatureMatrix.empty(b, fps * gh * gw, f, l1, images.device)
     elif fm.batch != b or fm.positions != fps * gh * gw or fm.num_rows != f:
         raise ValueError("ftm_conv_binarize_planes: buffers do not match the map")
+    if val_planes is not None:
+        val_planes = _need(val_planes, torch.uint8, "val_planes")
+        _call("nnue_ftm_conv_binarize_value_planes", images.data_ptr(), weight.data_ptr(), thr.data_ptr(), b, h, w, fps, int(stride), f,
+              table.data_ptr(), l1, int(l2), _ptr(planes), planes.numel() if planes is not None else 0, val_planes.data_ptr(), val_planes.numel(),
+              conv_out.data_ptr(), fm.bits.data_ptr(), fm.n.data_ptr(), fm.sink.data_ptr(), _stream(images))
+        return conv_out, fm
     _call("nnue_ftm_conv_binarize_planes", images.data_ptr(), weight.data_ptr(), thr.data_ptr(), b, h, w, fps, int(stride), f,
           table.data_ptr(), l1, int(l2), planes.data_ptr(), planes.numel(), conv_out.data_ptr(), fm.bits.data_ptr(), fm.n.data_ptr(),
           fm.sink.data_ptr(), _stream(images))
@@ -855,6 +871,14 @@
     return bool(load().nnue_ftm_backward_cw_supported(b, f, p, l1, l2))
 
 
+def ftm_value_planes_supported(b: int, f: int, p: int, l1: int, h: int, w: int, stride: int) -> bool:
+    return bool(load().nnue_ftm_value_planes_supported(int(b), int(f), int(p), int(l1), int(h), int(w), int(stride)))
+
+
+def ftm_value_planes_bytes(b: int, f: int, p: int, l1: int) -> int:
+    return int(load().nnue_ftm_value_planes_bytes(int(b), int(f), int(p), int(l1)))
+
+
 def ftm_backward_ste_chunks(b: int, f: int, p: int, l1: int, h: int, w: int, stride: int) -> int:
     return int(load().nnue_ftm_backward_ste_chunks(b, f, p, l1, h, w, stride))
 
@@ -862,7 +886,8 @@
 def ftm_backward(d_out: torch.Tensor, weight: torch.Tensor, fm: FeatureMatrix, d_weight: Optional[torch.Tensor] = None,
                  d_bias: Optional[torch.Tensor] = None, dst: Optional[torch.Tensor] = None, ft: Optional[torch.Tensor] = None,
                  d_z1: Optional[torch.Tensor] = None, d_w1: Optional[torch.Tensor] = None,
-                 sq_partial: Optional[torch.Tensor] = None, buckets=None, small: Optional["NnueClsRider"] = None, ste=None):
+                 sq_partial: Optional[torch.Tensor] = None, buckets=None, small: Optional["NnueClsRider"] = None, ste=None,
+                 val_planes: Optional[torch.Tensor] = None):
     d_out = _need(d_out, torch.float32, "d_out")
     weight = _need(weight, torch.float32, "input.weight")
     b, l1 = d_out.shape
@@ -904,7 +929,12 @@
             fm.positions, l1, d_weight.data_ptr(), d_bias.data_ptr(), _ptr(dst),
             _ptr(ft if d_w1 is not None else None), _ptr(d_z1 if d_w1 is not None else None), l2, _ptr(d_w1), _ptr(sq_partial))
     rider = ctypes.pointer(small) if small is not None else None
-    if buckets is None:
+    if val_planes is not None:
+        if buckets is not None:
+            raise ValueError("ftm_backward: the value planes have no bucketed form")
+        val_planes = _need(val_planes, torch.uint8, "val_planes")
+        _call("nnue_ftm_backward_planes", *args, rider, *ste_args, val_planes.data_ptr(), val_planes.numel(), _stream(d_out))
+    elif buckets is None:
         _call("nnue_ftm_backward", *args, rider, *ste_args, _stream(d_out))
     else:
         _call("nnue_ftm_backward_bucketed", *args, buckets.K, buckets.seg.data_ptr(), rows, rider, *ste_args, _stream(d_out))
diff --git a/nnue-vision_amd/nnue_hip/trainer.py b/nnue-vision_amd/nnue_hip/trainer.py
--- a/nnue-vision_amd/nnue_hip/trainer.py
+++ b/nnue-vision_amd/nnue_hip/trainer.py
@@ -261,6 +261,10 @@
             need = self.fps * 28 * ste_chunks * 4
             if self.ste_scratch.numel() < need:
                 self.ste_scratch = torch.empty((need,), **u8)
+        self.val_planes = None
+        if (self.ride_ste and not self.use_patches and self.bucket_plan is None
+                and lib.ftm_value_planes_supported(B, self.F, self.P, self.L1, self.H, self.W, self.stride)):
+            self.val_planes = torch.empty((lib.ftm_value_planes_bytes(B, self.F, self.P, self.L1),), **u8)
         self.fuse_next_forward = ((self.fuse_table_update or self.factor_exchange) and not self.fuse_l1 and self.K == 1
                                   and os.environ.get("NNUE_FUSE_NEXT_FORWARD", "1") != "0"
                                   and lib.ftm_update_forward_supported(gb if self.factor_exchange else B, self.F, self.P, self.L1, B))
@@ -331,9 +335,9 @@
     def _segment(self, name: str) -> None:
         p, g = self.p, self.g
         if name == "front":
-            if self.fwd_planes:
+            if self.fwd_planes or self.val_planes is not None:
                 lib.ftm_conv_binarize_planes(self.images, p["conv.weight"], p["visual_threshold"], self.stride, p["input.weight"], self.L2,
-                                             self.planes, conv_out=self.conv_out, fm=self.fm)
+                                             self.planes, conv_out=self.conv_out, fm=self.fm, val_planes=self.val_planes)
                 return
             if self.use_mfma:
                 lib.ftm_conv_binarize(self.images, p["conv.weight"], p["visual_threshold"], self.stride, self.F, self.L1,
@@ -378,7 +382,7 @@
                                  d_w1=g["classifier.classifier.0.weight"] if self.ride_dw1 else None, sq_partial=self.sq_partial,
                                  buckets=self.bucket_plan, small=self._rider(self.loss) if self.ride_small else None,
                                  ste=((self.images, self.conv_out, p["visual_threshold"], self.stride, self.ste_scratch, self.patches)
-                                      if self.ride_ste else None))
+                                      if self.ride_ste else None), val_planes=self.val_planes)
             elif self.use_mfma:
                 lib.ftm_backward_weight(self.d_ft, self.fm, d_weight=g["input.weight"], d_bias=g["input.bias"])
             elif self.use_bits:
```
